# themattinthehatt/behavenet

Hardware: AMD Instinct MI355X
Metric: AE training frames/sec (128x128x1, batch 256) (higher is better)
Workload: dtype f32; 1 GPU; configs[1]: conv AE default arch, 1x128x128 f32 frames resident in HBM, 12 latents, batch 256 (chunks 200+56), fwd+bwd+Adam(amsgrad)

## Files before the change

### behavenet_amd/_hip.py

```python

import ctypes
import os

import numpy as np
import torch

_LIB_NAME = 'libbehavenet_hip.so'
_LIB_PATH = os.environ.get('BN_HIP_LIB') or os.path.join(
    os.path.dirname(os.path.abspath(__file__)), _LIB_NAME)
_lib = None

ACT_NONE, ACT_LRELU, ACT_SIGMOID = 0, 1, 2

PROF_NONE, PROF_CONV_FWD, PROF_CONV_BWD_D, PROF_CONV_BWD_W = 0, 1, 2, 3
PROF_CONVT_FWD, PROF_CONVT_BWD_D, PROF_CONVT_BWD_W, PROF_ADAM = 4, 5, 6, 7
PROF_LINEAR_FWD, PROF_LINEAR_BWD = 8, 9

_c_int, _c_float, _c_size_t, _c_void_p = ctypes.c_int, ctypes.c_float, ctypes.c_size_t, ctypes.c_void_p

_CONV_GEOM = [_c_int] * 12
_ACT_WS = [_c_int, _c_float, _c_void_p, _c_size_t, _c_void_p]

OP_CONV_FWD, OP_CONV_BWD_D, OP_CONV_BWD_W = 1, 2, 3
OP_CONVT_FWD, OP_CONVT_BWD_D, OP_CONVT_BWD_W = 4, 5, 6

SIGNATURES = {
    'bn_version': (_c_int, []),
    'bn_build_arch': (ctypes.c_char_p, []),
    'bn_error_string': (ctypes.c_char_p, [_c_int]),
    'bn_set_force_generic': (_c_int, [_c_int]),
    'bn_set_bigk1_block_bytes': (_c_size_t, [_c_size_t]),
    'bn_conv_ws_bytes': (_c_size_t, [_c_int] + _CONV_GEOM),
    'bn_conv_taps_bytes': (_c_size_t, [_c_int] + _CONV_GEOM),
    'bn_conv_taps_pad': (_c_int, [_c_int, _c_void_p, _c_void_p, _c_void_p, _c_void_p]),
    'bn_conv2d_fwd': (_c_int, [_c_void_p] * 5 + _CONV_GEOM + _ACT_WS),
    'bn_conv2d_fwd_u8_ws_bytes': (_c_size_t, _CONV_GEOM + [_c_int]),
    'bn_conv2d_fwd_u8': (_c_int, [_c_void_p] * 4 + _CONV_GEOM + _ACT_WS),
    'bn_conv2d_bwd_data': (_c_int, [_c_void_p] * 5 + _CONV_GEOM + _ACT_WS),
    'bn_conv2d_bwd_weight': (
        _c_int, [_c_void_p] * 4 + _CONV_GEOM + [_c_int, _c_void_p, _c_size_t, _c_void_p]),
    'bn_convT2d_fwd': (_c_int, [_c_void_p] * 5 + _CONV_GEOM + _ACT_WS),
    'bn_convT2d_bwd_data': (_c_int, [_c_void_p] * 5 + _CONV_GEOM + _ACT_WS),
    'bn_convT2d_bwd_weight': (
        _c_int, [_c_void_p] * 4 + _CONV_GEOM + [_c_int, _c_void_p, _c_size_t, _c_void_p]),
    'bn_batchnorm_ws_bytes': (_c_size_t, [_c_int, _c_int]),
    'bn_batchnorm_stats': (_c_int, [_c_void_p] * 3 + [_c_int] * 3 + [_c_void_p, _c_size_t, _c_void_p]),
    'bn_batchnorm_finalize': (_c_int, [_c_void_p] * 5 + [_c_int] + [_c_float] * 3 + [_c_void_p]),
    'bn_batchnorm_act_fwd': (_c_int, [_c_void_p] * 6 + [_c_int] * 4 + [_c_float, _c_void_p]),
    'bn_batchnorm_train_fwd_chunks': (
        _c_int, [_c_void_p] * 11 + [_c_int] * 3 + [_c_float, _c_int, _c_float, _c_void_p, _c_size_t,
                                                  _c_void_p]),
    'bn_batchnorm_act_bwd_chunks': (
        _c_int, [_c_void_p] * 10 + [_c_int, _c_void_p] + [_c_int] * 4 + [_c_float, _c_void_p, _c_size_t,
                                                                        _c_void_p]),
    'bn_batchnorm_act_bwd': (
        _c_int, [_c_void_p] * 9 + [_c_int] * 6 + [_c_float, _c_void_p, _c_size_t, _c_void_p]),
    'bn_batchnorm_moment': (_c_int, [_c_void_p] * 3 + [_c_int] * 3 + [_c_void_p, _c_size_t, _c_void_p]),
    'bn_batchnorm_bwd_reduce': (
        _c_int, [_c_void_p] * 7 + [_c_int] * 4 + [_c_float, _c_void_p, _c_size_t, _c_void_p]),
    'bn_batchnorm_bwd_apply': (
        _c_int, [_c_void_p] * 9 + [_c_int] * 3 + [_c_float, _c_int, _c_float, _c_void_p]),
    'bn_maxpool2d_fwd': (_c_int, [_c_void_p] * 3 + [_c_int] * 9 + [_c_void_p]),
    'bn_maxpool2d_bwd': (_c_int, [_c_void_p] * 3 + [_c_int] * 9 + [_c_void_p]),
    'bn_maxpool2d_act_fwd': (_c_int, [_c_void_p] * 3 + [_c_int] * 4 + [ctypes.c_float, _c_void_p]),
    'bn_conv2d_pool2_act_fwd': (_c_int, [_c_void_p] * 5 + _CONV_GEOM + [_c_int, _c_float, _c_void_p]),
    'bn_conv2d_pool2_act_ok': (_c_int, _CONV_GEOM),
    'bn_conv2d_pool2_bwd_weight_ws_bytes': (_c_size_t, _CONV_GEOM),
    'bn_conv2d_pool2_bwd_weight': (
        _c_int, [_c_void_p] * 6 + _CONV_GEOM + [_c_int, _c_float, _c_int, _c_void_p, _c_size_t, _c_void_p]),
    'bn_maxpool2d_act_bwd': (_c_int, [_c_void_p] * 4 + [_c_int] * 4 + [ctypes.c_float, _c_void_p]),
    'bn_maxunpool2d_fwd': (_c_int, [_c_void_p] * 3 + [_c_int] * 3 + [_c_void_p]),
    'bn_maxunpool2d_fwd_k2': (_c_int, [_c_void_p] * 3 + [_c_int] * 3 + [_c_void_p]),
    'bn_maxunpool2d_bwd': (_c_int, [_c_void_p] * 3 + [_c_int] * 3 + [_c_void_p]),
    'bn_act_fwd': (_c_int, [_c_void_p] * 2 + [_c_size_t, _c_int, _c_float, _c_void_p]),
    'bn_act_bwd': (_c_int, [_c_void_p] * 3 + [_c_size_t, _c_int, _c_float, _c_void_p]),
    'bn_linear_ws_bytes': (_c_size_t, [_c_int] * 3),
    'bn_linear_fwd': (_c_int, [_c_void_p] * 4 + [_c_int] * 3 + [_c_void_p, _c_size_t, _c_void_p]),
    'bn_linear_bwd': (
        _c_int, [_c_void_p] * 5 + [_c_int, _c_float, _c_void_p, _c_void_p, _c_int] +
        [_c_int] * 3 + [_c_void_p, _c_size_t, _c_void_p]),
    'bn_sqerr_frame_sums': (_c_int, [_c_void_p] * 4 + [_c_int, _c_size_t, _c_void_p]),
    'bn_sqerr_bwd': (_c_int, [_c_void_p] * 4 + [_c_size_t, _c_float, _c_void_p, _c_void_p]),
    'bn_convT2d_fwd_sqerr_parts': (_c_int, _CONV_GEOM),
    'bn_convT2d_fwd_sqerr_ws_bytes': (_c_size_t, _CONV_GEOM + [_c_int]),
    'bn_convT2d_fwd_sqerr': (
        _c_int, [_c_void_p] * 8 + _CONV_GEOM + [_c_int, _c_float, _c_void_p, _c_size_t, _c_void_p]),
    'bn_scale_frames': (_c_int, [_c_void_p] * 4 + [_c_int, _c_size_t, _c_void_p]),
    'bn_reduce_sum': (_c_int, [_c_void_p] * 2 + [_c_size_t, _c_float, _c_void_p]),
    'bn_reparam_fwd': (_c_int, [_c_void_p] * 4 + [_c_size_t, _c_void_p]),
    'bn_kl_rows': (_c_int, [_c_void_p] * 3 + [_c_int, _c_int, _c_void_p]),
    'bn_reparam_bwd': (_c_int, [_c_void_p] * 4 + [_c_size_t, _c_void_p]),
    'bn_kl_bwd': (_c_int, [_c_void_p] * 4 + [_c_size_t, _c_float, _c_void_p, _c_void_p]),
    'bn_decomposed_kl_fwd': (_c_int, [_c_void_p] * 7 + [_c_int, _c_int, _c_void_p]),
    'bn_decomposed_kl_bwd': (_c_int, [_c_void_p] * 9 + [_c_int, _c_int, _c_void_p]),
    'bn_psvae_head_fwd': (_c_int, [_c_void_p] * 14 + [_c_int] * 3 + [_c_void_p]),
    'bn_psvae_head_combine': (
        _c_int, [_c_void_p] * 4 + [_c_int] + [_c_float] * 3 + [_c_int] + [_c_void_p] * 3),
    'bn_psvae_head_bwd': (
        _c_int, [_c_void_p] * 3 + [_c_int] + [_c_void_p] * 10 + [_c_float] + [_c_void_p] * 5 +
        [_c_int] * 4 + [_c_void_p]),
    'bn_adam_amsgrad_step': (
        _c_int, [_c_void_p] * 5 + [_c_size_t] + [_c_float] * 5 + [_c_int, _c_void_p]),
    'bn_conv2d_first_bf16_ok': (_c_int, _CONV_GEOM),
    'bn_conv2d_bf16_ok': (_c_int, _CONV_GEOM),
    'bn_conv_pack_w_bf16_bytes': (_c_size_t, [_c_int] * 4),
    'bn_conv_pack_w_bf16': (_c_int, [_c_void_p] * 2 + [_c_int] * 4 + [_c_void_p]),
    'bn_conv2d_first_bf16': (
        _c_int, [_c_void_p, _c_int] + [_c_void_p] * 3 + _CONV_GEOM + [_c_int, _c_float, _c_void_p]),
    'bn_conv2d_fwd_bf16': (
        _c_int, [_c_void_p] * 4 + [_c_int] + _CONV_GEOM + [_c_int, _c_float, _c_void_p]),
    'bn_convT2d_bf16_ok': (_c_int, _CONV_GEOM),
    'bn_convT2d_last_bf16_ok': (_c_int, _CONV_GEOM),
    'bn_convT_pack_w_bf16_bytes': (_c_size_t, [_c_int] * 4),
    'bn_convT_pack_w_bf16': (_c_int, [_c_void_p] * 2 + [_c_int] * 4 + [_c_void_p]),
    'bn_to_nhwc_bf16': (_c_int, [_c_void_p] * 2 + [_c_int] * 4 + [_c_void_p]),
    'bn_convT2d_fwd_bf16': (
        _c_int, [_c_void_p] * 4 + [_c_int] + _CONV_GEOM + [_c_int, _c_float, _c_void_p]),
    'bn_convT2d_last_bf16': (
        _c_int, [_c_void_p] * 4 + _CONV_GEOM + [_c_int, _c_float, _c_void_p]),
    'bn_convT2d_last_bf16_sqerr_ws_bytes': (_c_size_t, _CONV_GEOM),
    'bn_convT2d_last_bf16_sqerr': (
        _c_int, [_c_void_p] * 4 + [_c_int] + [_c_void_p] * 2 + _CONV_GEOM +
        [_c_int, _c_float, _c_float, _c_void_p, _c_size_t, _c_void_p]),
    'bn_convT2d_last_bf16_u8': (
        _c_int, [_c_void_p] * 4 + _CONV_GEOM + [_c_int, _c_float, _c_void_p]),
    'bn_frame_sq_err_ws_bytes': (_c_size_t, [_c_int, _c_size_t]),
    'bn_frame_sq_err': (
        _c_int, [_c_void_p] * 2 + [_c_int] + [_c_void_p] * 2 + [_c_int, _c_size_t, _c_float, _c_void_p, _c_size_t,
                                                                 _c_void_p]),
    'bn_pixel_stats_ws_bytes': (_c_size_t, [_c_int, _c_size_t]),
    'bn_pixel_stats_accum': (
        _c_int, [_c_void_p] * 2 + [_c_int, _c_void_p, _c_int, _c_void_p, _c_int, _c_size_t, _c_void_p, _c_size_t,
                                   _c_void_p]),
    'bn_u8_to_unit_float': (_c_int, [_c_void_p] * 2 + [_c_size_t, _c_void_p]),
    'bn_unit_float_to_u8': (_c_int, [_c_void_p] * 2 + [_c_size_t, _c_void_p]),
    'bn_cond_encoder_input': (_c_int, [_c_void_p, _c_int, _c_void_p] + [_c_int] * 6 + [_c_void_p, _c_void_p]),
    'bn_frame_mosaic_u8': (_c_int, [_c_void_p] + [_c_int] * 10 + [_c_void_p] + [_c_int] * 3 + [_c_void_p, _c_void_p]),
    'bn_recon_panels_u8': (_c_int, [_c_void_p, _c_int, _c_void_p, _c_int, _c_void_p] + [_c_int] * 6
                           + [_c_void_p, _c_size_t, _c_void_p]),
    'bn_column_select_ws_bytes': (_c_size_t, [_c_int] * 3),
    'bn_column_count': (_c_int, [_c_void_p] + [_c_int] * 3 + [_c_void_p, _c_void_p, _c_size_t, _c_void_p]),
    'bn_column_select': (_c_int, [_c_void_p] + [_c_int] * 3 + [_c_void_p, _c_int, _c_void_p, _c_void_p, _c_size_t,
                                                                _c_void_p]),
    'bn_segment_label_sums_ws_bytes': (_c_size_t, [_c_int] * 3),
    'bn_segment_label_sums': (_c_int, [_c_void_p, _c_int] * 3 + [_c_void_p] + [_c_int] * 3
                              + [_c_void_p, _c_void_p, _c_size_t, _c_void_p]),
    'bn_prof_select': (_c_int, [_c_int] * 3),
    'bn_prof_select_nth': (_c_int, [_c_int] * 4),
    'bn_prof_read': (_c_int, [ctypes.POINTER(ctypes.c_double), ctypes.POINTER(ctypes.c_long)]),
    'bn_prof_read_main': (_c_int, [ctypes.POINTER(ctypes.c_double), ctypes.POINTER(ctypes.c_long)]),
    'bn_prof_set_bracket': (_c_int, [_c_int]),
    'bn_prof_kernel_name': (ctypes.c_char_p, []),
    'bn_prof_dispatch_overhead_us': (ctypes.c_double, [_c_int, _c_void_p]),
}


class HipLibraryError(RuntimeError):
    pass


def lib_path():
    return _LIB_PATH


def load(required=True):
    global _lib
    if _lib is not None:
        return _lib
    if not os.path.exists(_LIB_PATH):
        if required:
            raise HipLibraryError(
                '%s not found next to the package (%s). Build it with '
                '`python -c "import __graft_entry__ as g; g.build()"` or '
                '`make -C behavenet_amd/csrc`. There is no CPU fallback.' % (_LIB_NAME, _LIB_PATH))
        return None
    lib = ctypes.CDLL(_LIB_PATH)
    for name, (restype, argtypes) in SIGNATURES.items():
        fn = getattr(lib, name)
        fn.restype = restype
        fn.argtypes = argtypes
    _lib = lib
    return _lib


def _check(rc, what):
    if rc != 0:
        msg = load().bn_error_string(int(rc))
        raise HipLibraryError('%s failed: %s (code %d)' % (what, msg.decode() if msg else '?', rc))


def _ptr(t, name, dtype=torch.float32, allow_none=False):
    if t is None:
        if allow_none:
            return None
        raise HipLibraryError('%s: tensor is None' % name)
    if not t.is_cuda:
        raise HipLibraryError(
            '%s: expected a tensor on the GPU, got device %s (the HIP path has no CPU fallback)'
            % (name, t.device))
    if t.dtype != dtype:
        raise HipLibraryError('%s: expected dtype %s, got %s' % (name, dtype, t.dtype))
    if not t.is_contiguous():
        raise HipLibraryError('%s: tensor must be contiguous' % name)
    return t.data_ptr()


def _stream():
    return torch.cuda.current_stream().cuda_stream


_ws_cache = {}


def _arena(device, nbytes, tag=None):
    if torch.cuda.is_current_stream_capturing():
        return torch.empty(int(nbytes), dtype=torch.uint8, device=device).data_ptr()
    key = (device, torch.cuda.current_stream(device).cuda_stream) + ((tag,) if tag else ())
    buf = _ws_cache.get(key)
    if buf is None or buf.numel() < nbytes:
        with torch.cuda.stream(torch.cuda.current_stream(device)):
            buf = torch.empty(int(nbytes), dtype=torch.uint8, device=device)
        _ws_cache[key] = buf
    return buf.data_ptr()


def _workspace(op, geom, device):
    if torch.device(device).type != 'cuda':
        raise HipLibraryError(
            'expected tensors on the GPU, got device %s (the HIP path has no CPU fallback)' % device)
    nbytes = load().bn_conv_ws_bytes(op, *geom)
    if nbytes == 0:
        return None, 0
    return _arena(device, nbytes), nbytes


_taps_bytes = {}
_generic_epoch = 0


def conv_taps_bytes(op, geom):
    key = (_generic_epoch, op) + tuple(geom)
    v = _taps_bytes.get(key)
    if v is None:
        v = _taps_bytes[key] = int(load().bn_conv_taps_bytes(op, *geom))
    return v


def conv_taps_pad(jobs, device):
    n = len(jobs)
    if n == 0:
        return []
    sizes = [(conv_taps_bytes(op, geom) // 4 + 63) // 64 * 64 for op, geom, _ in jobs]
    if min(sizes) == 0:
        raise HipLibraryError('conv_taps_pad: a layer whose op does not pad its taps')
    buf = torch.empty(sum(sizes), dtype=torch.float32, device=device)
    out, o = [], 0
    for sz in sizes:
        out.append(buf[o:o + sz])
        o += sz
    wp = (ctypes.c_void_p * n)(*[_ptr(w, 'w') for _, _, w in jobs])
    w5p = (ctypes.c_void_p * n)(*[t.data_ptr() for t in out])
    flat = []
    for op, geom, _ in jobs:
        flat.append(op)
        flat.extend(int(v) for v in geom)
    geoms = (ctypes.c_int * (13 * n))(*flat)
    _check(load().bn_conv_taps_pad(n, wp, w5p, geoms, _stream()), 'bn_conv_taps_pad')
    return out


def conv2d_fwd(x, w, b, geom, act, slope, w5=None):
    N, C, H, W, K, R, S, st, pt, pl, P, Q = geom
    y = torch.empty((N, K, P, Q), dtype=torch.float32, device=x.device)
    ws, nb = _workspace(OP_CONV_FWD, geom, x.device)
    _check(load().bn_conv2d_fwd(
        _ptr(x, 'x'), _ptr(w, 'w'), _ptr(w5, 'w5', allow_none=True), _ptr(b, 'b', allow_none=True), _ptr(y, 'y'),
        *geom, act, slope, ws, nb, _stream()), 'bn_conv2d_fwd')
    return y


def conv2d_fwd_u8(x_u8, w, b, geom, act, slope):
    N, C, H, W, K, R, S, st, pt, pl, P, Q = geom
    y = torch.empty((N, K, P, Q), dtype=torch.float32, device=x_u8.device)
    lib = load()
    nbytes = lib.bn_conv2d_fwd_u8_ws_bytes(*geom, act)
    ws = None
    if nbytes:
        ws = _arena(x_u8.device, nbytes, 'fwd_u8')
    _check(lib.bn_conv2d_fwd_u8(
        _ptr(x_u8, 'x', dtype=torch.uint8), _ptr(w, 'w'), _ptr(b, 'b', allow_none=True),
        _ptr(y, 'y'), *geom, act, slope, ws, nbytes, _stream()), 'bn_conv2d_fwd_u8')
    return y


def conv2d_bwd_data(dy, w, geom, dact_src, dact, slope, w5=None):
    N, C, H, W = geom[:4]
    dx = torch.empty((N, C, H, W), dtype=torch.float32, device=dy.device)
    ws, nb = _workspace(OP_CONV_BWD_D, geom, dy.device)
    _check(load().bn_conv2d_bwd_data(
        _ptr(dy, 'dy'), _ptr(w, 'w'), _ptr(w5, 'w5', allow_none=True), _ptr(dx, 'dx'),
        _ptr(dact_src, 'dact_src', allow_none=True), *geom, dact, slope, ws, nb, _stream()), 'bn_conv2d_bwd_data')
    return dx


def conv2d_bwd_weight(x, dy, dw, db, geom, accumulate):
    ws, nb = _workspace(OP_CONV_BWD_W, geom, x.device)
    _check(load().bn_conv2d_bwd_weight(
        _ptr(x, 'x'), _ptr(dy, 'dy'), _ptr(dw, 'dw'), _ptr(db, 'db', allow_none=True), *geom,
# ... 361 lines not shown


def batchnorm_sync_train_fwd(x, gamma, beta, running_mean, running_var, momentum, eps, act, slope,
                             all_reduce):
    n, c = x.shape[0], x.shape[1]
    hw = x.numel() // max(n * c, 1) if n else int(x.shape[2] * x.shape[3])
    dev = x.device
    s1 = torch.zeros((c + 1,), dtype=torch.float32, device=dev)
    if n:
        ws, nb = _bn_ws(n, c, dev)
        _check(load().bn_batchnorm_moment(_ptr(x, 'x'), None, _ptr(s1, 'sums'), n, c, hw, ws, nb,
                                          _stream()), 'bn_batchnorm_moment')
        s1[c] = float(n)
    all_reduce(s1)
    count = s1[c] * hw
    mean = (s1[:c] / count).contiguous()
    s2 = torch.zeros((c,), dtype=torch.float32, device=dev)
    if n:
        _check(load().bn_batchnorm_moment(_ptr(x, 'x'), _ptr(mean, 'mean'), _ptr(s2, 'sums'), n, c,
                                          hw, ws, nb, _stream()), 'bn_batchnorm_moment')
    all_reduce(s2)
    var = (s2 / count).contiguous()
    cnt = float(count.item())
    unbias = cnt / (cnt - 1.0) if cnt > 1 else 1.0
    invstd = torch.empty_like(mean)
    _check(load().bn_batchnorm_finalize(
        _ptr(mean, 'mean'), _ptr(var, 'var'), _ptr(invstd, 'invstd'),
        _ptr(running_mean, 'running_mean', allow_none=True),
        _ptr(running_var, 'running_var', allow_none=True), c, eps, momentum, unbias, _stream()),
        'bn_batchnorm_finalize')
    y = torch.empty_like(x)
    if n:
        _check(load().bn_batchnorm_act_fwd(
            _ptr(x, 'x'), _ptr(mean, 'mean'), _ptr(invstd, 'invstd'),
            _ptr(gamma, 'gamma', allow_none=True), _ptr(beta, 'beta', allow_none=True),
            _ptr(y, 'y'), n, c, hw, act, slope, _stream()), 'bn_batchnorm_act_fwd')
    return y, mean, invstd, cnt


def batchnorm_sync_bwd(x, y, dy, mean, invstd, gamma, count, act, slope, all_reduce):
    n, c = x.shape[0], x.shape[1]
    hw = x.numel() // max(n * c, 1) if n else 1
    local = torch.zeros((2, c), dtype=torch.float32, device=x.device)
    if n:
        ws, nb = _bn_ws(n, c, x.device)
        _check(load().bn_batchnorm_bwd_reduce(
            _ptr(x, 'x'), _ptr(y, 'y'), _ptr(dy, 'dy'), _ptr(mean, 'mean'),
            _ptr(invstd, 'invstd'), _ptr(local[0], 'sum_dz'), _ptr(local[1], 'sum_dzx'), n, c, hw,
            act, slope, ws, nb, _stream()), 'bn_batchnorm_bwd_reduce')
    total = all_reduce(local.clone())
    dx = torch.empty_like(x)
    if n:
        _check(load().bn_batchnorm_bwd_apply(
            _ptr(x, 'x'), _ptr(y, 'y'), _ptr(dy, 'dy'), _ptr(mean, 'mean'),
            _ptr(invstd, 'invstd'), _ptr(gamma, 'gamma', allow_none=True),
            _ptr(total[0], 'sum_dz'), _ptr(total[1], 'sum_dzx'), _ptr(dx, 'dx'), n, c, hw,
            1.0 / float(count), act, slope, _stream()), 'bn_batchnorm_bwd_apply')
    return dx, local[0], local[1]


def act_fwd(x, act, slope):
    y = torch.empty_like(x)
    _check(load().bn_act_fwd(_ptr(x, 'x'), _ptr(y, 'y'), x.numel(), act, slope, _stream()),
           'bn_act_fwd')
    return y


def act_bwd(dy, y, act, slope, out=None):
    if out is None:
        out = torch.empty_like(dy)
    _check(load().bn_act_bwd(
        _ptr(dy, 'dy'), _ptr(y, 'y'), _ptr(out, 'dpre'), dy.numel(), act, slope, _stream()),
        'bn_act_bwd')
    return out


def _linear_ws(M, K, N, device):
    nbytes = load().bn_linear_ws_bytes(M, K, N)
    if nbytes == 0:
        return None, 0
    return _arena(device, nbytes, 'linear'), nbytes


def linear_fwd(x, w, b):
    M, K = x.shape
    N = w.shape[0]
    y = torch.empty((M, N), dtype=torch.float32, device=x.device)
    ws, nb = _linear_ws(M, K, N, x.device)
    _check(load().bn_linear_fwd(
        _ptr(x, 'x'), _ptr(w, 'w'), _ptr(b, 'b', allow_none=True), _ptr(y, 'y'), M, K, N,
        ws, nb, _stream()), 'bn_linear_fwd')
    return y


def linear_bwd(x, w, dy, need_dx, dact_src, dact, slope, dw, db, accumulate):
    M, N = dy.shape
    K = w.shape[1]
    dx = torch.empty((M, K), dtype=torch.float32, device=dy.device) if need_dx else None
    ws, nb = _linear_ws(M, K, N, dy.device) if need_dx else (None, 0)
    _check(load().bn_linear_bwd(
        _ptr(x, 'x', allow_none=True), _ptr(w, 'w'), _ptr(dy, 'dy'),
        _ptr(dx, 'dx', allow_none=True), _ptr(dact_src, 'dact_src', allow_none=True), dact, slope,
        _ptr(dw, 'dw', allow_none=True), _ptr(db, 'db', allow_none=True), int(accumulate),
        M, K, N, ws, nb, _stream()), 'bn_linear_bwd')
    return dx


def sqerr_frame_sums(pred, target, mask):
    N = pred.shape[0]
    D = pred.numel() // N
    out = torch.empty((N,), dtype=torch.float32, device=pred.device)
    _check(load().bn_sqerr_frame_sums(
        _ptr(pred, 'pred'), _ptr(target, 'target'), _ptr(mask, 'mask', allow_none=True),
        _ptr(out, 'frame_sums'), N, D, _stream()), 'bn_sqerr_frame_sums')
    return out


def sqerr_bwd(pred, target, mask, scale, gscale, out=None):
    dpred = torch.empty_like(pred) if out is None else out
    _check(load().bn_sqerr_bwd(
        _ptr(pred, 'pred'), _ptr(target, 'target'), _ptr(mask, 'mask', allow_none=True),
        _ptr(dpred, 'dpred'), pred.numel(), float(scale), _ptr(gscale, 'gscale', allow_none=True),
        _stream()), 'bn_sqerr_bwd')
    return dpred


def convT2d_fwd_sqerr(x, w, b, target, mask, geom, act, slope, want_xhat):
    N, Ci, Hi, Wi, Co, R, S, st, ct, cl, Ho, Wo = geom
    lib = load()
    P = lib.bn_convT2d_fwd_sqerr_parts(*geom)
    if P <= 0:
        raise HipLibraryError('bn_convT2d_fwd_sqerr_parts: bad geometry %s' % (geom,))
    xhat = torch.empty((N, Co, Ho, Wo), dtype=torch.float32, device=x.device) if want_xhat \
        else None
    dpre = torch.empty((N, Co, Ho, Wo), dtype=torch.float32, device=x.device)
    part = torch.empty((N, P), dtype=torch.float32, device=x.device)
    nbytes = lib.bn_convT2d_fwd_sqerr_ws_bytes(*geom, int(want_xhat))
    ws = None
    if nbytes:
        ws = _arena(x.device, nbytes, 'fwd_sqerr')
    _check(lib.bn_convT2d_fwd_sqerr(
        _ptr(x, 'x'), _ptr(w, 'w'), _ptr(b, 'b', allow_none=True), _ptr(target, 'target'),
        _ptr(mask, 'mask', allow_none=True), _ptr(xhat, 'xhat', allow_none=True),
        _ptr(dpre, 'dpre'), _ptr(part, 'part'), *geom, act, slope, ws, nbytes, _stream()),
        'bn_convT2d_fwd_sqerr')
    return xhat, dpre, part


def scale_frames(t, frame_scale, group_scale=None, group_of_frame=None):
    N = t.shape[0]
    _check(load().bn_scale_frames(
        _ptr(t, 't'), _ptr(frame_scale, 'frame_scale'),
        _ptr(group_scale, 'group_scale', allow_none=True),
        _ptr(group_of_frame, 'group_of_frame', dtype=torch.int32, allow_none=True),
        N, t.numel() // N, _stream()), 'bn_scale_frames')
    return t


def reduce_sum(t, scale=1.0, out=None):
    if out is None:
        out = torch.empty((), dtype=torch.float32, device=t.device)
    _check(load().bn_reduce_sum(_ptr(t, 'in'), _ptr(out, 'out'), t.numel(), float(scale),
                                _stream()), 'bn_reduce_sum')
    return out


def reparam_fwd(mu, logvar, eps):
    z = torch.empty_like(mu)
    _check(load().bn_reparam_fwd(
        _ptr(mu, 'mu'), _ptr(logvar, 'logvar'), _ptr(eps, 'eps'), _ptr(z, 'z'), mu.numel(),
        _stream()), 'bn_reparam_fwd')
    return z


def kl_rows(mu, logvar):
    N, D = mu.shape
    out = torch.empty((N,), dtype=torch.float32, device=mu.device)
    _check(load().bn_kl_rows(_ptr(mu, 'mu'), _ptr(logvar, 'logvar'), _ptr(out, 'kl_rows'), N, D,
                             _stream()), 'bn_kl_rows')
    return out


DECOMPOSED_KL_MAX_D = 64


def _check_dkl_width(D):
    if D > DECOMPOSED_KL_MAX_D:
        raise ValueError('decomposed KL: %d latent dimensions, the kernels serve at most %d'
                         % (D, DECOMPOSED_KL_MAX_D))


def decomposed_kl_fwd(z, mu, logvar, out3=None):
    N, D = z.shape
    _check_dkl_width(D)
    if out3 is None:
        out3 = torch.empty((3,), dtype=torch.float32, device=z.device)
    log_qz = torch.empty((N,), dtype=torch.float32, device=z.device)
    lse = torch.empty((N, D), dtype=torch.float32, device=z.device)
    terms = torch.empty((3 * N,), dtype=torch.float32, device=z.device)
    _check(load().bn_decomposed_kl_fwd(
        _ptr(z, 'z'), _ptr(mu, 'mu'), _ptr(logvar, 'logvar'), _ptr(out3, 'out3'),
        _ptr(log_qz, 'log_qz'), _ptr(lse, 'lse'), _ptr(terms, 'terms'), N, D, _stream()),
        'bn_decomposed_kl_fwd')
    return out3, log_qz, lse


def decomposed_kl_bwd(z, mu, logvar, log_qz, lse, g3, out=None):
    N, D = z.shape
    _check_dkl_width(D)
    dz, dmu, dlogvar = out if out is not None else (
        torch.empty_like(z), torch.empty_like(z), torch.empty_like(z))
    _check(load().bn_decomposed_kl_bwd(
        _ptr(z, 'z'), _ptr(mu, 'mu'), _ptr(logvar, 'logvar'), _ptr(log_qz, 'log_qz'),
        _ptr(lse, 'lse'), _ptr(g3, 'g3'), _ptr(dz, 'dz'), _ptr(dmu, 'dmu'),
        _ptr(dlogvar, 'dlogvar'), N, D, _stream()), 'bn_decomposed_kl_bwd')
    return dz, dmu, dlogvar


def psvae_head_fwd(y, w, logvar, eps, Dw, Db, labels, lmask):
    N, L = y.shape
    U = logvar.shape[1] - L
    dev = y.device
    z = torch.empty((N, L + U), dtype=torch.float32, device=dev)
    z_u = torch.empty((N, U), dtype=torch.float32, device=dev)
    lv_u = torch.empty((N, U), dtype=torch.float32, device=dev)
    yhat = torch.empty((N, L), dtype=torch.float32, device=dev)
    rows = torch.empty((2, N), dtype=torch.float32, device=dev)
    _check(load().bn_psvae_head_fwd(
        _ptr(y, 'y'), _ptr(w, 'w', allow_none=True), _ptr(logvar, 'logvar'), _ptr(eps, 'eps'),
        _ptr(Dw, 'Dw'), _ptr(Db, 'Db', allow_none=True), _ptr(labels, 'labels'),
        _ptr(lmask, 'lmask', allow_none=True), _ptr(z, 'z'), _ptr(z_u, 'z_u'), _ptr(lv_u, 'lv_u'),
        _ptr(yhat, 'yhat'), _ptr(rows[0], 'row_sq'), _ptr(rows[1], 'row_kl'), N, L, U, _stream()),
        'bn_psvae_head_fwd')
    return z, z_u, lv_u, yhat, rows[0], rows[1]


def psvae_head_combine(row_sq, row_kl, dkl3, bounds_dev, n_chunks, alpha, kl, beta, L):
    T = torch.empty((n_chunks,), dtype=torch.float32, device=row_sq.device)
    cols5 = torch.empty((n_chunks, 5), dtype=torch.float32, device=row_sq.device)
    _check(load().bn_psvae_head_combine(
        _ptr(row_sq, 'row_sq'), _ptr(row_kl, 'row_kl'), _ptr(dkl3, 'dkl3'),
        _ptr(bounds_dev, 'bounds', dtype=torch.int32), int(n_chunks), float(alpha), float(kl),
        float(beta), int(L), _ptr(T, 'T'), _ptr(cols5, 'cols5'), _stream()), 'bn_psvae_head_combine')
    return T, cols5


# ... 411 lines not shown
```

### behavenet_amd/csrc/bn_launch.h

```cpp
#pragma once
#include "bn_common.h"

struct GemmArgs {
    const float* A; long sai, sak;
    const float* B; long sbk, sbj;
    float* C; long sci, scj;
    int M, N, K;
    const float* bias_j;
    const float* dact_src;
    int dact; float slope;
    int accumulate;
    float* part;
    int kslice;
};

int bn_launch_down_generic(const float* big, const float* w, const float* bias, float* out,
                           const float* dact_src, const BnGeom& g, int act, int dact, float slope,
                           hipStream_t st);
int bn_launch_up_generic(const float* small, const float* w, const float* bias, float* out,
                         const float* dact_src, const BnGeom& g, int act, int dact, float slope,
                         hipStream_t st);
int bn_launch_wgrad_generic(const float* small, const float* big, float* dw, const BnGeom& g,
                            int accumulate, hipStream_t st);
size_t bn_channel_sum_ws_bytes(int N, int C, int npix);
int bn_launch_channel_sum(const float* t, float* db, int N, int C, int npix, int accumulate,
                          void* ws, size_t ws_bytes, hipStream_t st);

int bn_launch_gemm(const GemmArgs& a, hipStream_t st, void* ws = nullptr, size_t ws_bytes = 0);
size_t bn_gemm_ws_bytes(int M, int N, int K);
int bn_launch_col_sum(const float* dy, float* db, int M, int N, int accumulate, hipStream_t st);
int bn_launch_linear_jobs(const GemmArgs* g0, const GemmArgs* g1, const float* dy, float* db, int M,
                          int N, int accumulate, void* ws, size_t ws_bytes, hipStream_t st);
size_t bn_linear_jobs_ws_bytes(int M, int N, int K);

int bn_launch_act_fwd(const float* x, float* y, size_t n, int act, float slope, hipStream_t st);
int bn_launch_act_bwd(const float* dy, const float* y, float* dpre, size_t n, int act, float slope,
                      hipStream_t st);
int bn_launch_sqerr_frame_sums(const float* pred, const float* target, const float* mask,
                               float* frame_sums, int N, size_t D, hipStream_t st);
int bn_launch_sqerr_bwd(const float* pred, const float* target, const float* mask, float* dpred,
                        size_t n, float scale, const float* gscale, hipStream_t st);
int bn_launch_scale_frames(float* t, const float* frame_scale, const float* group_scale,
                           const int* group_of_frame, int N, size_t D, hipStream_t st);
int bn_launch_reduce_sum(const float* in, float* out, size_t n, float scale, hipStream_t st);
int bn_launch_reparam_fwd(const float* mu, const float* logvar, const float* eps, float* z,
                          size_t n, hipStream_t st);
int bn_launch_kl_rows(const float* mu, const float* logvar, float* kl_rows, int N, int D,
                      hipStream_t st);
int bn_launch_reparam_bwd(const float* dz, const float* z, const float* mu, float* dlogvar,
                          size_t n, hipStream_t st);
int bn_launch_kl_bwd(const float* mu, const float* logvar, float* dmu, float* dlogvar, size_t n,
                     float scale, const float* gscale, hipStream_t st);
int bn_launch_adam(float* p, const float* g, float* m, float* v, float* vmax, size_t n, float lr,
                   float b1, float b2, float eps, float wd, int step, hipStream_t st);
int bn_launch_u8_to_unit_float(const unsigned char* in, float* out, size_t n, hipStream_t st);

bool bn_frame_sq_err_ok(int N, size_t D);
size_t bn_frame_sq_err_ws_bytes_impl(int N, size_t D);
int bn_launch_frame_sq_err(const float* xhat, const void* target, int target_is_u8, const float* mask, float* out,
                           int N, size_t D, float scale, void* ws, hipStream_t st);
int bn_launch_frame_err_finish(const float* part, float* out, int N, unsigned P, float scale, hipStream_t st);

bool bn_unit_float_to_u8_ok(size_t n);
int bn_launch_unit_float_to_u8(const float* in, unsigned char* out, size_t n, hipStream_t st);

bool bn_pixel_stats_ok(int N, size_t D);
size_t bn_pixel_stats_ws_bytes_impl(int N, size_t D);
int bn_launch_pixel_stats(const float* xhat, const void* target, int target_is_u8, const float* mask, int mask_frames,
                          double* acc, int N, size_t D, void* ws, hipStream_t st);

bool bn_cond_input_ok(int N, int C, int H, int W, int L);
int bn_launch_cond_input(const void* frames, int frames_is_u8, const float* coords, int ld, int N, int C, int H, int W,
                         int L, float* out, hipStream_t st);

bool bn_frame_mosaic_ok(int P, int C, int H, int W, int ch, int y_min, int x_min, int Hc, int Wc, int T, int R, int Cc);
int bn_launch_frame_mosaic(const void* frames, int frames_u8, int P, int C, int H, int W, int ch, int y_min, int x_min,
                           int Hc, int Wc, const int* src, int T, int R, int Cc, unsigned char* out, hipStream_t st);

bool bn_recon_panels_ok(int N, int C, int H, int W, size_t out_frame_stride);
int bn_launch_recon_panels(const void* orig, int orig_u8, const void* recon, int recon_u8, const float* mask,
                           int mask_per_frame, int N, int C, int H, int W, int show_orig, unsigned char* out,
                           size_t out_frame_stride, hipStream_t st);

bool bn_column_select_ok(int n, int d, int ld, int r);
size_t bn_column_count_ws_bytes_impl(int n, int d);
size_t bn_column_select_ws_bytes_impl(int n, int d, int r);
int bn_launch_column_count(const float* x, int n, int d, int ld, long long* n_valid, void* ws, hipStream_t st);
int bn_launch_column_select(const float* x, int n, int d, int ld, const long long* ranks, int r, float* out, void* ws,
                            hipStream_t st);

bool bn_segment_label_sums_ok(int n, int S, int L);
size_t bn_segment_label_sums_ws_bytes_impl(int n, int S, int L);
int bn_launch_segment_label_sums(const float* pred, int ld_pred, const float* truth, int ld_truth, const float* mask,
                                 int ld_mask, const long long* offsets, int S, int L, int n, double* out, void* ws,
                                 hipStream_t st);

size_t bn_batchnorm_ws_bytes_impl(int N, int C);
int bn_launch_bn_stats(const float* x, float* mean, float* var, int N, int C, int HW, void* ws,
                       hipStream_t st);
int bn_launch_bn_finalize(const float* mean, const float* var, float* invstd, float* running_mean,
                          float* running_var, int C, float eps, float momentum, float unbias,
                          hipStream_t st);
int bn_launch_bn_act_fwd(const float* x, const float* mean, const float* invstd,
                         const float* gamma, const float* beta, float* y, int N, int C, int HW,
                         int act, float slope, hipStream_t st);
int bn_launch_bn_act_bwd(const float* x, const float* y, const float* dy, const float* mean,
                         const float* invstd, const float* gamma, float* dx, float* dgamma,
                         float* dbeta, int accumulate, int batch_stats, int N, int C, int HW,
                         int act, float slope, void* ws, hipStream_t st);

int bn_launch_bn_moment(const float* x, const float* center, float* sums, int N, int C, int HW,
                        void* ws, hipStream_t st);
int bn_launch_bn_bwd_reduce(const float* x, const float* y, const float* dy, const float* mean,
                            const float* invstd, float* sum_dz, float* sum_dzx, int N, int C,
                            int HW, int act, float slope, void* ws, hipStream_t st);
int bn_launch_bn_train_fwd_chunks(const float* x, const float* gamma, const float* beta,
                                  float* running_mean, float* running_var, long long* num_batches,
                                  float* y, float* mean, float* invstd, const int* bounds,
                                  const float* factors, int n_chunks, int C, int HW, float eps, int act,
                                  float slope, void* ws, hipStream_t st);
int bn_launch_bn_act_bwd_chunks(const float* x, const float* y, const float* dy, const float* mean,
                                const float* invstd, const float* gamma, const float* beta, float* dx,
                                float* dgamma, float* dbeta, int accumulate, const int* bounds,
                                int n_chunks, int C, int HW, int act, float slope, void* ws,
                                hipStream_t st);
int bn_launch_bn_bwd_apply(const float* x, const float* y, const float* dy, const float* mean,
                           const float* invstd, const float* gamma, const float* sum_dz,
// ... 85 lines not shown
```

### behavenet_amd/csrc/bn_reduce.h

```cpp
#pragma once
#include "bn_common.h"

__global__ __launch_bounds__(1024) void k_sum_partials(const float* __restrict__ part,
                                                       float* __restrict__ out, int total,
                                                       int splits, int accumulate, int ab_elems,
                                                       int ntap, int row_len, int row_stride);

__global__ __launch_bounds__(256) void k_sum_partials_pair(
    const float* __restrict__ part_a, float* __restrict__ out_a, int total_a, int ab_elems, int ntap,
    const float* __restrict__ part_b, float* __restrict__ out_b, int total_b, int splits,
    int accumulate, int blocks_a);

static inline int bn_launch_sum_partials_pair(const float* part_a, float* out_a, int total_a,
                                              int ab_elems, int ntap, const float* part_b,
                                              float* out_b, int total_b, int splits, int accumulate,
                                              hipStream_t st) {
    const int blocks_a = (total_a + 63) / 64, blocks_b = (total_b + 63) / 64;
    hipLaunchKernelGGL(k_sum_partials_pair, dim3(blocks_a + blocks_b), dim3(256), 0, st, part_a, out_a,
                       total_a, ab_elems, ntap, part_b, out_b, total_b, splits, accumulate, blocks_a);
    hipError_t e = hipGetLastError();
    return e == hipSuccess ? 0 : (int)e;
}

static inline int bn_launch_sum_partials(const float* part, float* out, int total, int splits,
                                         int accumulate, int ab_elems, int ntap, hipStream_t st,
                                         int row_len = 0, int row_stride = 0) {
    const int threads = (splits >= 128 && total <= 16384) ? 1024 : 256;
    hipLaunchKernelGGL(k_sum_partials, dim3((total + 63) / 64), dim3(threads), 0, st, part, out, total,
                       splits, accumulate, ab_elems, ntap, row_len, row_stride);
    hipError_t e = hipGetLastError();
    return e == hipSuccess ? 0 : (int)e;
}
```

### behavenet_amd/csrc/capi.hip

```cpp
#include <math.h>
#include <stdio.h>
#include <stdlib.h>
#include <string.h>
#include <hip/hip_ext.h>
#include "bn_common.h"
#include "bn_launch.h"
#include "bn_fast.h"

namespace {
struct ProfState {
    int family = BN_PROF_NONE;
    int C = 0, K = 0;
    static const int kMaxSlots = 2048;
    hipEvent_t ev[4 * kMaxSlots];
    bool taken[kMaxSlots], bracketed[kMaxSlots];
    int created = 0;
    int used = 0;
    double total_ms = 0.0, main_ms = 0.0;
    long launches = 0, main_launches = 0;
    bool bracket = true;
    int nth = -1, seen = 0;
    char kernel_name[96] = "";
} g_prof;

// ... 1342 lines not shown
        if (bi[1] <= 0 || bounds[2 * i] < 0) return BN_E_BADARG;
        if (!ws || ws_bytes < bn_batchnorm_ws_bytes_impl(bi[1], C)) return BN_E_WORKSPACE;
        const size_t o = (size_t)bounds[2 * i] * C * HW;
        const float fi = factors ? factors[i] : 0.f;
        const int rc = bn_launch_bn_train_fwd_chunks(x + o, gamma, beta, running_mean, running_var,
                                                     num_batches_tracked, y + o, mean + (size_t)i * C,
                                                     invstd + (size_t)i * C, bi, &fi, 1, C, HW, eps, act,
                                                     slope, ws, st);
        if (rc) return rc;
    }
    return 0;
}

extern "C" int bn_batchnorm_act_bwd_chunks(const float* x, const float* y, const float* dy,
                                           const float* mean, const float* invstd,
                                           const float* gamma, const float* beta, float* dx,
                                           float* dgamma, float* dbeta, int accumulate,
                                           const int* bounds, int n_chunks, int C, int HW, int act,
                                           float slope, void* ws, size_t ws_bytes, bn_stream_t stream) {
    if (!x || !dy || !mean || !invstd || !dx || !bounds || n_chunks <= 0 || C <= 0 || HW <= 0)
        return BN_E_BADARG;
    if (!y && act != BN_ACT_NONE && act != BN_ACT_LRELU) return BN_E_BADARG;
    hipStream_t st = (hipStream_t)stream;
    {
        int nmax = 0;
        for (int i = 0; i < n_chunks; ++i) nmax = bounds[2 * i + 1] - bounds[2 * i] > nmax ? bounds[2 * i + 1] - bounds[2 * i] : nmax;
        if (nmax > 0 && ws && ws_bytes >= bn_batchnorm_ws_bytes_impl(nmax, C)) {
            const int rc = bn_launch_bn_act_bwd_chunks(x, y, dy, mean, invstd, gamma, beta, dx, dgamma, dbeta,
                                                       accumulate, bounds, n_chunks, C, HW, act, slope, ws, st);
            if (rc != BN_E_SHAPE) return rc;
        }
    }
    for (int i = 0; i < n_chunks; ++i) {
        const int bi[2] = {0, bounds[2 * i + 1] - bounds[2 * i]};
        if (bi[1] <= 0 || bounds[2 * i] < 0) return BN_E_BADARG;
        if (!ws || ws_bytes < bn_batchnorm_ws_bytes_impl(bi[1], C)) return BN_E_WORKSPACE;
        const size_t o = (size_t)bounds[2 * i] * C * HW;
        const int rc = bn_launch_bn_act_bwd_chunks(x + o, y ? y + o : nullptr, dy + o, mean + (size_t)i * C,
                                                   invstd + (size_t)i * C, gamma, beta, dx + o, dgamma, dbeta,
                                                   (accumulate || i > 0) ? 1 : 0, bi, 1, C, HW, act, slope, ws,
                                                   st);
        if (rc) return rc;
    }
    return 0;
}

extern "C" int bn_batchnorm_moment(const float* x, const float* center, float* sums, int N, int C,
                                   int HW, void* ws, size_t ws_bytes, bn_stream_t stream) {
    if (!x || !sums || N <= 0 || C <= 0 || HW <= 0) return BN_E_BADARG;
    if (!ws || ws_bytes < bn_batchnorm_ws_bytes_impl(N, C)) return BN_E_WORKSPACE;
    return bn_launch_bn_moment(x, center, sums, N, C, HW, ws, (hipStream_t)stream);
}

extern "C" int bn_batchnorm_bwd_reduce(const float* x, const float* y, const float* dy,
                                       const float* mean, const float* invstd, float* sum_dz,
                                       float* sum_dzx, int N, int C, int HW, int act, float slope,
                                       void* ws, size_t ws_bytes, bn_stream_t stream) {
    if (!x || !y || !dy || !mean || !invstd || !sum_dz || !sum_dzx || N <= 0 || C <= 0 || HW <= 0)
        return BN_E_BADARG;
    if (!ws || ws_bytes < bn_batchnorm_ws_bytes_impl(N, C)) return BN_E_WORKSPACE;
    return bn_launch_bn_bwd_reduce(x, y, dy, mean, invstd, sum_dz, sum_dzx, N, C, HW, act, slope, ws,
                                   (hipStream_t)stream);
}

extern "C" int bn_batchnorm_bwd_apply(const float* x, const float* y, const float* dy,
                                      const float* mean, const float* invstd, const float* gamma,
                                      const float* sum_dz, const float* sum_dzx, float* dx, int N,
                                      int C, int HW, float inv_count, int act, float slope,
                                      bn_stream_t stream) {
    if (!x || !y || !dy || !mean || !invstd || !sum_dz || !sum_dzx || !dx || N <= 0 || C <= 0 ||
        HW <= 0)
        return BN_E_BADARG;
    return bn_launch_bn_bwd_apply(x, y, dy, mean, invstd, gamma, sum_dz, sum_dzx, dx, N, C, HW,
                                  inv_count, act, slope, (hipStream_t)stream);
}

extern "C" size_t bn_linear_ws_bytes(int M, int K, int N) {
    if (M <= 0 || K <= 0 || N <= 0) return 0;
    const size_t f = bn_gemm_ws_bytes(M, N, K), d = bn_gemm_ws_bytes(M, K, N);
    return f > d ? f : d;
}

extern "C" int bn_linear_fwd(const float* x, const float* w, const float* b, float* y, int M,
                             int K, int N, void* ws, size_t ws_bytes, bn_stream_t stream) {
    if (!x || !w || !y || M <= 0 || K <= 0 || N <= 0) return BN_E_BADARG;
    GemmArgs a;
    a.A = x; a.sai = K; a.sak = 1;
    a.B = w; a.sbk = 1; a.sbj = K;
    a.C = y; a.sci = N; a.scj = 1;
    a.M = M; a.N = N; a.K = K;
    a.bias_j = b; a.dact_src = nullptr; a.dact = BN_ACT_NONE; a.slope = 0.f; a.accumulate = 0;
    BnProfScope prof(BN_PROF_LINEAR_FWD, K, N, "k_linear_jobs", (hipStream_t)stream);
    return bn_launch_linear_jobs(&a, nullptr, nullptr, nullptr, 0, 0, 0, ws, ws_bytes, (hipStream_t)stream);
}

extern "C" int bn_linear_bwd(const float* x, const float* w, const float* dy, float* dx,
                             const float* dact_src, int dact, float slope, float* dw, float* db,
                             int accumulate, int M, int K, int N, void* ws, size_t ws_bytes,
                             bn_stream_t stream) {
    if (!dy || M <= 0 || K <= 0 || N <= 0) return BN_E_BADARG;
    hipStream_t st = (hipStream_t)stream;
    BnProfScope prof(BN_PROF_LINEAR_BWD, K, N, "k_linear_jobs (dx, dW, db)", st);
    GemmArgs gx, gw;
    if (dx) {
        if (!w) return BN_E_BADARG;
        GemmArgs& a = gx;
        a.A = dy; a.sai = N; a.sak = 1;
        a.B = w; a.sbk = K; a.sbj = 1;
        a.C = dx; a.sci = K; a.scj = 1;
        a.M = M; a.N = K; a.K = N;
        a.bias_j = nullptr; a.dact_src = dact_src; a.dact = dact; a.slope = slope;
        a.accumulate = 0; a.part = nullptr; a.kslice = 0;
    }
    if (dw) {
        if (!x) return BN_E_BADARG;
        GemmArgs& a = gw;
        a.A = dy; a.sai = 1; a.sak = N;
        a.B = x; a.sbk = K; a.sbj = 1;
        a.C = dw; a.sci = K; a.scj = 1;
        a.M = N; a.N = K; a.K = M;
        a.bias_j = nullptr; a.dact_src = nullptr; a.dact = BN_ACT_NONE; a.slope = 0.f;
        a.accumulate = accumulate; a.part = nullptr; a.kslice = 0;
    }
    return bn_launch_linear_jobs(dx ? &gx : nullptr, dw ? &gw : nullptr, dy, db, M, N, accumulate, ws,
                                 ws_bytes, st);
}

extern "C" int bn_sqerr_frame_sums(const float* pred, const float* target, const float* mask,
                                   float* frame_sums, int N, size_t D, bn_stream_t stream) {
    if (!pred || !target || !frame_sums || N <= 0 || D == 0) return BN_E_BADARG;
    return bn_launch_sqerr_frame_sums(pred, target, mask, frame_sums, N, D, (hipStream_t)stream);
}

extern "C" int bn_sqerr_bwd(const float* pred, const float* target, const float* mask,
                            float* dpred, size_t n, float scale, const float* gscale,
                            bn_stream_t stream) {
    if (!pred || !target || !dpred) return BN_E_BADARG;
    if (n == 0) return 0;
    return bn_launch_sqerr_bwd(pred, target, mask, dpred, n, scale, gscale, (hipStream_t)stream);
}

static bool fused_sqerr_fast(const BnGeom& g) {
    return !force_generic() && !bn_qgemm_supported(g) && !bn_s5win_supported(g) && !bn_s5_up_plan(g).supported &&
           bn_edge_up_plan(g).supported;
}

extern "C" int bn_convT2d_fwd_sqerr_parts(int N, int Ci, int Hi, int Wi, int Co, int R, int S,
                                          int stride, int crop_t, int crop_l, int Ho, int Wo) {
    const BnGeom g = convT_geom(N, Ci, Hi, Wi, Co, R, S, stride, crop_t, crop_l, Ho, Wo);
    if (!bn_geom_ok(g)) return 0;
    return fused_sqerr_fast(g) ? bn_edge_up_parts_per_frame(g) : 1;
}

extern "C" size_t bn_convT2d_fwd_sqerr_ws_bytes(int N, int Ci, int Hi, int Wi, int Co, int R,
                                                int S, int stride, int crop_t, int crop_l, int Ho,
                                                int Wo, int with_xhat) {
    const BnGeom g = convT_geom(N, Ci, Hi, Wi, Co, R, S, stride, crop_t, crop_l, Ho, Wo);
    if (!bn_geom_ok(g) || fused_sqerr_fast(g)) return 0;
    size_t conv = bn_conv_ws_bytes(BN_OP_CONVT_FWD, N, Ci, Hi, Wi, Co, R, S, stride, crop_t, crop_l,
                                   Ho, Wo);
    conv = (conv + 255) & ~(size_t)255;
    return conv + (with_xhat ? 0 : (size_t)N * Co * Ho * Wo * sizeof(float));
}

extern "C" int bn_convT2d_fwd_sqerr(const float* x, const float* w, const float* b,
                                    const float* target, const float* mask, float* xhat,
                                    float* dpre, float* part, int N, int Ci, int Hi, int Wi,
                                    int Co, int R, int S, int stride, int crop_t, int crop_l,
                                    int Ho, int Wo, int act, float slope, void* ws,
                                    size_t ws_bytes, bn_stream_t stream) {
    if (!x || !w || !target || !dpre || !part) return BN_E_BADARG;
    const BnGeom g = convT_geom(N, Ci, Hi, Wi, Co, R, S, stride, crop_t, crop_l, Ho, Wo);
    if (!bn_geom_ok(g)) return BN_E_BADARG;
    hipStream_t st = (hipStream_t)stream;
    if (fused_sqerr_fast(g)) {
        BnProfScope prof(BN_PROF_CONVT_FWD, g.Cs, g.Cb, bn_edge_up_kernel_name(g, true), st);
        return bn_launch_edge_up(x, w, b, xhat, g, act, slope, st, target, mask, dpre, part);
    }
    const size_t need = bn_convT2d_fwd_sqerr_ws_bytes(N, Ci, Hi, Wi, Co, R, S, stride, crop_t,
                                                      crop_l, Ho, Wo, xhat != nullptr);
    if (need && (!ws || ws_bytes < need)) return BN_E_WORKSPACE;
    const size_t n_out = (size_t)N * Co * Ho * Wo;
    const size_t conv_ws = need - (xhat ? 0 : n_out * sizeof(float));
    float* xh = xhat ? xhat : (float*)((char*)ws + conv_ws);
    int rc = run_up(BN_PROF_CONVT_FWD, x, w, nullptr, b, xh, nullptr, g, act, BN_ACT_NONE, slope, ws,
                    conv_ws, st);
    if (rc) return rc;
    rc = bn_launch_sqerr_frame_sums(xh, target, mask, part, N, (size_t)Co * Ho * Wo, st);
    if (rc) return rc;
    rc = bn_launch_sqerr_bwd(xh, target, mask, dpre, n_out, 1.f, nullptr, st);
    if (rc) return rc;
    if (act != BN_ACT_NONE) rc = bn_launch_act_bwd(dpre, xh, dpre, n_out, act, slope, st);
    return rc;
}

extern "C" int bn_scale_frames(float* t, const float* frame_scale, const float* group_scale,
                               const int* group_of_frame, int N, size_t D, bn_stream_t stream) {
    if (!t || !frame_scale || N <= 0 || D == 0) return BN_E_BADARG;
    if ((group_scale == nullptr) != (group_of_frame == nullptr)) return BN_E_BADARG;
    return bn_launch_scale_frames(t, frame_scale, group_scale, group_of_frame, N, D,
                                  (hipStream_t)stream);
}

extern "C" int bn_reduce_sum(const float* in, float* out, size_t n, float scale,
                             bn_stream_t stream) {
    if (!in || !out) return BN_E_BADARG;
    return bn_launch_reduce_sum(in, out, n, scale, (hipStream_t)stream);
}

extern "C" int bn_reparam_fwd(const float* mu, const float* logvar, const float* eps, float* z,
                              size_t n, bn_stream_t stream) {
    if (!mu || !logvar || !eps || !z) return BN_E_BADARG;
    if (n == 0) return 0;
    return bn_launch_reparam_fwd(mu, logvar, eps, z, n, (hipStream_t)stream);
}

extern "C" int bn_kl_rows(const float* mu, const float* logvar, float* kl_rows, int N, int D,
                          bn_stream_t stream) {
    if (!mu || !logvar || !kl_rows || N <= 0 || D <= 0) return BN_E_BADARG;
    return bn_launch_kl_rows(mu, logvar, kl_rows, N, D, (hipStream_t)stream);
}

extern "C" int bn_reparam_bwd(const float* dz, const float* z, const float* mu, float* dlogvar,
                              size_t n, bn_stream_t stream) {
    if (!dz || !z || !mu || !dlogvar) return BN_E_BADARG;
    if (n == 0) return 0;
    return bn_launch_reparam_bwd(dz, z, mu, dlogvar, n, (hipStream_t)stream);
}

extern "C" int bn_kl_bwd(const float* mu, const float* logvar, float* dmu, float* dlogvar,
                         size_t n, float scale, const float* gscale, bn_stream_t stream) {
    if (!mu || !logvar || !dmu || !dlogvar) return BN_E_BADARG;
    if (n == 0) return 0;
    return bn_launch_kl_bwd(mu, logvar, dmu, dlogvar, n, scale, gscale, (hipStream_t)stream);
}

extern "C" int bn_decomposed_kl_fwd(const float* z, const float* mu, const float* logvar,
                                    float* out3, float* log_qz, float* lse, float* terms, int N,
                                    int D, bn_stream_t stream) {
    if (!z || !mu || !logvar || !out3 || !log_qz || !lse || !terms || N <= 0 || D <= 0)
        return BN_E_BADARG;
    return bn_launch_dkl_fwd(z, mu, logvar, out3, log_qz, lse, terms, N, D, (hipStream_t)stream);
}

extern "C" int bn_decomposed_kl_bwd(const float* z, const float* mu, const float* logvar,
                                    const float* log_qz, const float* lse, const float* g3,
                                    float* dz, float* dmu, float* dlogvar, int N, int D,
                                    bn_stream_t stream) {
    if (!z || !mu || !logvar || !log_qz || !lse || !g3 || !dz || !dmu || !dlogvar || N <= 0 ||
        D <= 0)
        return BN_E_BADARG;
    return bn_launch_dkl_bwd(z, mu, logvar, log_qz, lse, g3, dz, dmu, dlogvar, N, D,
                             (hipStream_t)stream);
}

extern "C" int bn_adam_amsgrad_step(float* p, const float* g, float* m, float* v, float* vmax,
                                    size_t n, float lr, float beta1, float beta2, float eps,
                                    float weight_decay, int step, bn_stream_t stream) {
    if (!p || !g || !m || !v || !vmax || step < 1) return BN_E_BADARG;
    if (n == 0) return 0;
    BnProfScope prof(BN_PROF_ADAM, 0, 0, "k_adam_amsgrad", (hipStream_t)stream);
    return bn_launch_adam(p, g, m, v, vmax, n, lr, beta1, beta2, eps, weight_decay, step,
                          (hipStream_t)stream);
}

extern "C" int bn_u8_to_unit_float(const unsigned char* in, float* out, size_t n,
                                   bn_stream_t stream) {
    if (!in || !out) return BN_E_BADARG;
    if (n == 0) return 0;
    return bn_launch_u8_to_unit_float(in, out, n, (hipStream_t)stream);
}

static BnBf16Geom bf16_geom(int N, int C, int H, int W, int K, int R, int S, int stride, int pad_t, int pad_l, int P,
                            int Q) {
    return BnBf16Geom{N, C, H, W, K, R, S, stride, pad_t, pad_l, P, Q};
}
static bool bf16_geom_valid(const BnBf16Geom& g) {
    if (!(g.N > 0 && g.C > 0 && g.H > 0 && g.W > 0 && g.K > 0 && g.R > 0 && g.S > 0 && g.stride > 0 && g.pt >= 0 &&
          g.pl >= 0 && g.P > 0 && g.Q > 0))
        return false;
    return (long)(g.P - 1) * g.stride - g.pt < g.H && (long)(g.Q - 1) * g.stride - g.pl < g.W;
}
static bool aligned16(const void* p) { return ((uintptr_t)p & 15) == 0; }

extern "C" int bn_conv2d_bf16_ok(int N, int C, int H, int W, int K, int R, int S, int stride, int pad_t, int pad_l,
                                 int P, int Q) {
    const BnBf16Geom g = bf16_geom(N, C, H, W, K, R, S, stride, pad_t, pad_l, P, Q);
    return (bf16_geom_valid(g) && bn_bf16_conv_ok(g)) ? 1 : 0;
}
extern "C" int bn_conv2d_first_bf16_ok(int N, int C, int H, int W, int K, int R, int S, int stride, int pad_t,
                                       int pad_l, int P, int Q) {
    const BnBf16Geom g = bf16_geom(N, C, H, W, K, R, S, stride, pad_t, pad_l, P, Q);
// ... 228 lines not shown
```

### behavenet_amd/csrc/conv_edge.hip

```cpp
#include <hip/hip_ext.h>
#include <stdlib.h>
#include "bn_common.h"
#include "bn_fast.h"
#include "bn_reduce.h"

typedef float floatx16 __attribute__((ext_vector_type(16)));

#define ED_THREADS 256
#define ED_OOB 0x7fffffff

__device__ __forceinline__ float ed_ld(__amdgpu_buffer_rsrc_t r, int byte_off) {
    return __builtin_bit_cast(float, __builtin_amdgcn_raw_buffer_load_b32(r, byte_off, 0, 0));
}

#define WC_ROWS 4
#define WC_W 64
#define WC_TPX (WC_ROWS * WC_W)
#define WC_SP (WC_TPX + 2)
#define WC_IH (2 * WC_ROWS + 3)
#define WC_RW (2 * WC_W + 4)
#define WC_KS (32 * WC_TPX / ED_THREADS)

#define WC_DECODE_GRID()                                                                    \
    int bch, bx, G;                                                                         \
// ... 436 lines not shown
        p.variant = 1;
        p.d = wgrad_c1_grid(g);
        p.ws_bytes = ((size_t)g.Cb * p.d * g.Cs * 25 + (size_t)p.d * 32) * sizeof(float);
        p.kernel_name = wgrad_c1e_ok(g) ? "k_wgrad_c1e" : "k_wgrad_c1<1>";
        return p;
    }
    if (g.Cs > 32) return p;
    if (g.Ws != WC_W || (g.Hs % WC_ROWS) != 0 || g.Hb != 2 * g.Hs || g.Wb != 2 * g.Ws) {
        if (g.pt > 4 || g.pl > 4 || (g.CsS > 0 && g.CsS != g.Cs)) return p;
        p.supported = true;
        p.variant = 1;
        p.d = wgrad_c1_grid(g);
        p.ws_bytes = ((size_t)g.Cb * p.d * g.Cs * 25 + (size_t)p.d * 32) * sizeof(float);
        p.kernel_name = "k_wgrad_c1<2>";
        return p;
    }
    p.supported = true;
    p.d = wgrad_c1_grid(g);
    p.ws_bytes = ((size_t)g.Cb * p.d * g.Cs * 25 + (size_t)p.d * 32) * sizeof(float);
    p.kernel_name = (g.pt == 1 && g.pl == 1) ? "k_wgrad_c1d" : "k_wgrad_c1<2>";
    return p;
}

int bn_launch_edge_wgrad(const BnFastPlan& plan, const float* small, const float* big, float* dw,
                         const BnGeom& g, int accumulate, void* ws, hipStream_t st, float* db,
                         int bias_side, bool* bias_done) {
    const int spf = wgrad_c1_rblocks(g) * wgrad_c1_cblocks(g), n_stages = g.N * spf;
    float* bias_part = (db && bias_side == 1)
        ? (float*)ws + (size_t)g.Cb * plan.d * g.Cs * 25 : nullptr;
    if (g.CsS > 0 && g.CsS != g.Cs && !(g.pt == 1 && g.pl == 1)) return BN_E_SHAPE;
    const bool vec = (g.Ws & 3) == 0 && (((uintptr_t)small) & 15u) == 0 && g.CsS == 0;
    const int pair = (g.Cb > 1 && (plan.d & 7) == 0) ? 1 : 0;
    const dim3 wgrid = pair ? dim3(plan.d * g.Cb) : dim3(plan.d, g.Cb);
    if (g.stride == 1 && wgrad_c1e_ok(g) && vec) {
        static bool attr_set = false;
        if (!attr_set) {
            const void* fns[4] = {(const void*)k_wgrad_c1e<true, false>, (const void*)k_wgrad_c1e<false, false>,
                                  (const void*)k_wgrad_c1e<true, true>, (const void*)k_wgrad_c1e<false, true>};
            for (const void* fn : fns) {
                hipError_t e1 = hipFuncSetAttribute(fn, hipFuncAttributeMaxDynamicSharedMemorySize, WE_LDS);
                if (e1 != hipSuccess) return (int)e1;
            }
            attr_set = true;
        }
#define WE_LAUNCH(B, M)                                                                                     \
        BN_LAUNCH_MAIN((k_wgrad_c1e<B, M>), wgrid, dim3(ED_THREADS), WE_LDS, st, small, big, (float*)ws,   \
                           bias_part, g, n_stages, spf, wgrad_c1_cblocks(g), pair)
        if (g.Cs <= 16) { if (bias_part) WE_LAUNCH(true, true); else WE_LAUNCH(false, true); }
        else { if (bias_part) WE_LAUNCH(true, false); else WE_LAUNCH(false, false); }
#undef WE_LAUNCH
    } else if (g.stride == 1) {
        if (vec)
            BN_LAUNCH_MAIN((k_wgrad_c1<1, true>), wgrid, dim3(ED_THREADS), 0, st, small, big,
                               (float*)ws, bias_part, g, n_stages, spf, wgrad_c1_cblocks(g), pair);
        else
            BN_LAUNCH_MAIN((k_wgrad_c1<1, false>), wgrid, dim3(ED_THREADS), 0, st, small, big,
                               (float*)ws, bias_part, g, n_stages, spf, wgrad_c1_cblocks(g), pair);
    } else if (g.pt == 1 && g.pl == 1 && plan.variant != 1) {
        static bool attr_set = false;
        if (!attr_set) {
            hipError_t e1 = hipFuncSetAttribute((const void*)k_wgrad_c1d<true>,
                                                hipFuncAttributeMaxDynamicSharedMemorySize, WD_LDS);
            hipError_t e2 = hipFuncSetAttribute((const void*)k_wgrad_c1d<false>,
                                                hipFuncAttributeMaxDynamicSharedMemorySize, WD_LDS);
            if (e1 != hipSuccess) return (int)e1;
            if (e2 != hipSuccess) return (int)e2;
            attr_set = true;
        }
        if (bias_part)
            BN_LAUNCH_MAIN(k_wgrad_c1d<true>, wgrid, dim3(ED_THREADS), WD_LDS, st, small,
                               big, (float*)ws, bias_part, g, n_stages, g.Hs / WC_ROWS, pair);
        else
            BN_LAUNCH_MAIN(k_wgrad_c1d<false>, wgrid, dim3(ED_THREADS), WD_LDS, st, small,
                               big, (float*)ws, bias_part, g, n_stages, g.Hs / WC_ROWS, pair);
    } else if (vec) {
        BN_LAUNCH_MAIN((k_wgrad_c1<2, true>), wgrid, dim3(ED_THREADS), 0, st, small, big,
                           (float*)ws, bias_part, g, n_stages, spf, wgrad_c1_cblocks(g), pair);
    } else {
        BN_LAUNCH_MAIN((k_wgrad_c1<2, false>), wgrid, dim3(ED_THREADS), 0, st, small, big,
                           (float*)ws, bias_part, g, n_stages, spf, wgrad_c1_cblocks(g), pair);
    }
    BN_LAUNCH_CHECK();
    if (bias_part) {
        const int rc = bn_launch_sum_partials(bias_part, db, g.Cs, plan.d, accumulate, 0, 0, st);
        if (rc) return rc;
        if (bias_done) *bias_done = true;
    }
    for (int b = 0; b < g.Cb; ++b) {
        const int rc = bn_launch_sum_partials(
            (const float*)ws + (size_t)b * plan.d * g.Cs * 25, dw + b * 25, g.Cs * 25, plan.d,
            accumulate, 0, 0, st, 25, g.Cb * 25);
        if (rc) return rc;
    }
    return 0;
}

#define DC_W 64
#define DC_ROWS 2
#define DC_IH (2 * DC_ROWS + 3)
#define DC_X0 4
#define DC_RW (2 * DC_W + 8)
#define DC_C4 (DC_RW / 4)
#define DC_NLD ((DC_IH * DC_C4 + 63) / 64)
#define DC_TS (DC_W + 4)
#define DC_SLAB (32 * DC_TS)
#ifndef DC_HALF
#define DC_HALF 1
#endif
#if DC_HALF
#define DC_MAX_WAVES_PER_CU 16
#define DC_WPE 4
#else
#define DC_MAX_WAVES_PER_CU 12
#define DC_WPE 3
#endif
#define DC_HTS 36

#ifndef DC_ST_AUX
#define DC_ST_AUX 16
#endif

typedef float floatx2p __attribute__((ext_vector_type(2)));
__device__ __forceinline__ void ed_lrelu4(float (&v)[4], float slope) {
    const floatx2p s2 = {slope, slope};
    floatx2p lo = {v[0], v[1]}, hi = {v[2], v[3]}, mlo, mhi;
    asm("v_pk_mul_f32 %0, %1, %2" : "=v"(mlo) : "v"(lo), "v"(s2));
    asm("v_pk_mul_f32 %0, %1, %2" : "=v"(mhi) : "v"(hi), "v"(s2));
    asm("v_max_f32 %0, %1, %2" : "=v"(v[0]) : "v"(lo.x), "v"(mlo.x));
    asm("v_max_f32 %0, %1, %2" : "=v"(v[1]) : "v"(lo.y), "v"(mlo.y));
    asm("v_max_f32 %0, %1, %2" : "=v"(v[2]) : "v"(hi.x), "v"(mhi.x));
    asm("v_max_f32 %0, %1, %2" : "=v"(v[3]) : "v"(hi.y), "v"(mhi.y));
}

#ifdef E0_SMALLOUT
#define E0_OUT_OFFSET(o) ((o) & 0xffff0)
#else
#define E0_OUT_OFFSET(o) (o)
#endif

typedef int intx4 __attribute__((ext_vector_type(4)));
typedef float floatx4e __attribute__((ext_vector_type(4)));
typedef unsigned int uintx4e __attribute__((ext_vector_type(4)));

template <int ACT, bool MASK, bool GENW = false>
__global__ __launch_bounds__(64) __attribute__((amdgpu_waves_per_eu(DC_WPE, DC_WPE))) void k_down_c1(
    const float* __restrict__ big, const float* __restrict__ w, const float* __restrict__ bias,
    float* __restrict__ out, const float* __restrict__ dact_src, BnGeom g, float slope,
    int units) {
    __shared__ __attribute__((aligned(16))) float bl[DC_IH * DC_RW];
    __shared__ __attribute__((aligned(16))) float tw[DC_HALF ? 32 * DC_HTS : DC_SLAB];
    const int lane = threadIdx.x;
    const int li = lane & 31, kk = lane >> 5;
    const int ncb = GENW ? (g.Ws + DC_W - 1) / DC_W : 1;
    const int rpf = GENW ? (g.Hs + DC_ROWS - 1) / DC_ROWS : g.Hs / DC_ROWS;
    const int upf = rpf * ncb;
    const int HWb = g.Hb * g.Wb, PQ = g.Hs * g.Ws;
#ifdef E0_TRACE
    unsigned long long* trc = e0_trace + (size_t)blockIdx.x * 8;
#define E0_MARK(slot) do { if (threadIdx.x == 0) trc[slot] = __builtin_amdgcn_s_memrealtime(); } while (0)
    E0_MARK(0);
    if (threadIdx.x == 0) trc[7] = __builtin_amdgcn_s_getreg((4 << 0) | (0 << 6) | (31 << 11));
#else
#define E0_MARK(slot)
#endif

    const __amdgpu_buffer_rsrc_t rb = __builtin_amdgcn_make_buffer_rsrc(
        (void*)big, 0, (int)((size_t)g.N * HWb * 4), 0x00020000);

    int ld_y[DC_NLD], ld_off[DC_NLD];
#pragma unroll
    for (int k = 0; k < DC_NLD; ++k) {
// ... 1774 lines not shown
```

### behavenet_amd/csrc/conv_generic.hip

```cpp
#include "bn_common.h"
#include "bn_launch.h"

#define GEN_THREADS 256
#define GEN_MT 8
#define GEN_MAXS 16

__global__ __launch_bounds__(GEN_THREADS) void k_down_generic(
    const float* __restrict__ big, const float* __restrict__ w, const float* __restrict__ bias,
    float* __restrict__ out, const float* __restrict__ dact_src, BnGeom g, int act, int dact,
    float slope) {
    const int pix = blockIdx.x * GEN_THREADS + threadIdx.x;
    const int npix = g.Hs * g.Ws;
    const int m0 = blockIdx.y * GEN_MT;
    const int n = blockIdx.z;
    if (pix >= npix) return;
    const int p = pix / g.Ws, q = pix - p * g.Ws;
    const int RS = g.R * g.S;
    float acc[GEN_MT];
#pragma unroll
    for (int j = 0; j < GEN_MT; ++j) acc[j] = 0.f;

    const int h0 = p * g.stride - g.pt, w0 = q * g.stride - g.pl;
    for (int c = 0; c < g.Cb; ++c) {
        const float* bp = big + ((size_t)n * g.Cb + c) * g.Hb * g.Wb;
// ... 167 lines not shown
int bn_launch_wgrad_generic(const float* small, const float* big, float* dw, const BnGeom& g,
                            int accumulate, hipStream_t st) {
    if (g.R > GEN_MAXS || g.S > GEN_MAXS) return BN_E_SHAPE;
    dim3 grid(g.Cb, g.Cs, g.R);
    hipLaunchKernelGGL(k_wgrad_generic, grid, dim3(GEN_THREADS), 0, st, small, big, dw, g,
                       accumulate);
    BN_LAUNCH_CHECK();
    return 0;
}

__global__ __launch_bounds__(GEN_THREADS) void k_channel_sum_part(
    const float* __restrict__ t, float* __restrict__ part, int N, int C, int npix, int S) {
    __shared__ float red[4];
    const int c = blockIdx.x, sp = blockIdx.y;
    const int n_beg = (int)((long)sp * N / S), n_end = (int)((long)(sp + 1) * N / S);
    float acc = 0.f;
    const bool vec = (npix & 3) == 0 && ((((uintptr_t)t) & 15u) == 0);
    const int per = npix >> 2;
    if (vec && per < GEN_THREADS && (GEN_THREADS % per) == 0) {
        const int fpp = GEN_THREADS / per, q = threadIdx.x % per;
        for (int n = n_beg + threadIdx.x / per; n < n_end; n += fpp) {
            const float4 v = reinterpret_cast<const float4*>(t + ((size_t)n * C + c) * npix)[q];
            acc += (v.x + v.y) + (v.z + v.w);
        }
    } else
    for (int n = n_beg; n < n_end; ++n) {
        const float* tp = t + ((size_t)n * C + c) * npix;
        if (vec) {
            const float4* t4 = reinterpret_cast<const float4*>(tp);
            for (int i = threadIdx.x; i < (npix >> 2); i += GEN_THREADS) {
                const float4 v = t4[i];
                acc += (v.x + v.y) + (v.z + v.w);
            }
        } else {
            for (int i = threadIdx.x; i < npix; i += GEN_THREADS) acc += tp[i];
        }
    }
    const float s = bn_block_reduce_256(acc, red);
    if (threadIdx.x == 0) part[(size_t)c * S + sp] = s;
}

__global__ __launch_bounds__(64) void k_channel_sum_final(const float* __restrict__ part, float* __restrict__ db,
                                                          int C, int S, int accumulate) {
    const int c = blockIdx.x;
    float v = 0.f;
    for (int s = threadIdx.x; s < S; s += 64) v += part[(size_t)c * S + s];
#pragma unroll
    for (int off = 32; off > 0; off >>= 1) v += __shfl_xor(v, off, 64);
    if (threadIdx.x == 0) db[c] = accumulate ? db[c] + v : v;
}

static int channel_sum_splits(int N, int C, int npix) {
    if ((long)N * npix < 8192) return 1;
    int s = 1024 / C;
    if (s > 256) s = 256;
    if (s > N) s = N;
    return s < 1 ? 1 : s;
}

size_t bn_channel_sum_ws_bytes(int N, int C, int npix) {
    const int s = channel_sum_splits(N, C, npix);
    return s > 1 ? (size_t)C * s * sizeof(float) : 0;
}

int bn_launch_channel_sum(const float* t, float* db, int N, int C, int npix, int accumulate,
                          void* ws, size_t ws_bytes, hipStream_t st) {
    const int S = channel_sum_splits(N, C, npix);
    if (S > 1 && ws && ws_bytes >= (size_t)C * S * sizeof(float)) {
        hipLaunchKernelGGL(k_channel_sum_part, dim3(C, S), dim3(GEN_THREADS), 0, st, t, (float*)ws,
                           N, C, npix, S);
        BN_LAUNCH_CHECK();
        hipLaunchKernelGGL(k_channel_sum_final, dim3(C), dim3(64), 0, st,
                           (const float*)ws, db, C, S, accumulate);
        BN_LAUNCH_CHECK();
        return 0;
    }
    hipLaunchKernelGGL(k_channel_sum, dim3(C), dim3(GEN_THREADS), 0, st, t, db, N, C, npix,
                       accumulate);
    BN_LAUNCH_CHECK();
    return 0;
}

#include "bn_reduce.h"
__global__ __launch_bounds__(1024) void k_sum_partials(const float* __restrict__ part,
                                                       float* __restrict__ out, int total,
                                                       int splits, int accumulate, int ab_elems,
                                                       int ntap, int row_len, int row_stride) {
    __shared__ float red[16][64];
    const int il = threadIdx.x & 63, zl = threadIdx.x >> 6;
    const int nz = blockDim.x >> 6;
    const int i = blockIdx.x * 64 + il;
    float s0 = 0.f, s1 = 0.f, s2 = 0.f, s3 = 0.f;
    if (i < total) {
        int z = zl;
        for (; z + 3 * nz < splits; z += 4 * nz) {
            s0 += part[(size_t)z * total + i];
            s1 += part[(size_t)(z + nz) * total + i];
            s2 += part[(size_t)(z + 2 * nz) * total + i];
            s3 += part[(size_t)(z + 3 * nz) * total + i];
        }
        for (; z < splits; z += nz) s0 += part[(size_t)z * total + i];
    }
    red[zl][il] = (s0 + s1) + (s2 + s3);
    __syncthreads();
    if (nz == 16 && zl < 4)
        red[zl][il] = (red[zl][il] + red[zl + 4][il]) + (red[zl + 8][il] + red[zl + 12][il]);
    if (nz == 16) __syncthreads();
    if (zl == 0 && i < total) {
        const float v = (red[0][il] + red[1][il]) + (red[2][il] + red[3][il]);
        size_t o = i;
        if (ab_elems > 0) {
            const int tap = i / ab_elems;
            o = (size_t)(i - tap * ab_elems) * ntap + tap;
        } else if (row_len > 0) {
            const int row = i / row_len;
            o = (size_t)row * row_stride + (i - row * row_len);
        }
        out[o] = accumulate ? out[o] + v : v;
    }
}

__global__ __launch_bounds__(256) void k_sum_partials_pair(
    const float* __restrict__ part_a, float* __restrict__ out_a, int total_a, int ab_elems, int ntap,
    const float* __restrict__ part_b, float* __restrict__ out_b, int total_b, int splits,
    int accumulate, int blocks_a) {
    __shared__ float red[4][64];
    const bool job_b = (int)blockIdx.x >= blocks_a;
    const float* part = job_b ? part_b : part_a;
    float* out = job_b ? out_b : out_a;
    const int total = job_b ? total_b : total_a;
    const int il = threadIdx.x & 63, zl = threadIdx.x >> 6;
    const int i = (job_b ? (int)blockIdx.x - blocks_a : (int)blockIdx.x) * 64 + il;
    float s0 = 0.f, s1 = 0.f, s2 = 0.f, s3 = 0.f;
    if (i < total) {
        int z = zl;
        for (; z + 12 < splits; z += 16) {
            s0 += part[(size_t)z * total + i];
            s1 += part[(size_t)(z + 4) * total + i];
            s2 += part[(size_t)(z + 8) * total + i];
            s3 += part[(size_t)(z + 12) * total + i];
        }
        for (; z < splits; z += 4) s0 += part[(size_t)z * total + i];
    }
    red[zl][il] = (s0 + s1) + (s2 + s3);
    __syncthreads();
    if (zl == 0 && i < total) {
        const float v = (red[0][il] + red[1][il]) + (red[2][il] + red[3][il]);
        size_t o = i;
        if (!job_b && ab_elems > 0) {
            const int tap = i / ab_elems;
            o = (size_t)(i - tap * ab_elems) * ntap + tap;
        }
        out[o] = accumulate ? out[o] + v : v;
    }
}
```

### behavenet_amd/csrc/elementwise.hip

```cpp
#include "bn_common.h"
#include "bn_launch.h"

#define EW_THREADS 256
#define EW_MAX_BLOCKS 2048

static inline int ew_blocks(size_t nvec) {
    size_t b = (nvec + EW_THREADS - 1) / EW_THREADS;
    if (b < 1) b = 1;
    if (b > EW_MAX_BLOCKS) b = EW_MAX_BLOCKS;
    return (int)b;
}

static inline bool aligned16(const void* p) { return (((uintptr_t)p) & 15u) == 0; }

__global__ __launch_bounds__(EW_THREADS) void k_act_bwd(
    const float* __restrict__ dy, const float* __restrict__ y, float* __restrict__ dpre, size_t n,
    int vec, int act, float slope) {
    const size_t tid = (size_t)blockIdx.x * EW_THREADS + threadIdx.x;
    const size_t nthreads = (size_t)gridDim.x * EW_THREADS;
    if (vec) {
        const size_t n4 = n >> 2;
        const float4* dy4 = reinterpret_cast<const float4*>(dy);
        const float4* y4 = reinterpret_cast<const float4*>(y);
        float4* o4 = reinterpret_cast<float4*>(dpre);
// ... 1 lines not shown
            const float4 a = dy4[i], b = y4[i];
            float4 o;
            o.x = a.x * bn_act_grad_from_output(b.x, act, slope);
            o.y = a.y * bn_act_grad_from_output(b.y, act, slope);
            o.z = a.z * bn_act_grad_from_output(b.z, act, slope);
            o.w = a.w * bn_act_grad_from_output(b.w, act, slope);
            o4[i] = o;
        }
        for (size_t i = (n4 << 2) + tid; i < n; i += nthreads)
            dpre[i] = dy[i] * bn_act_grad_from_output(y[i], act, slope);
    } else {
        for (size_t i = tid; i < n; i += nthreads)
            dpre[i] = dy[i] * bn_act_grad_from_output(y[i], act, slope);
    }
}

__global__ __launch_bounds__(EW_THREADS) void k_sqerr_frame_sums(
    const float* __restrict__ pred, const float* __restrict__ target,
    const float* __restrict__ mask, float* __restrict__ frame_sums, size_t D, int vec) {
    __shared__ float red[EW_THREADS / BN_WAVE];
    const size_t base = (size_t)blockIdx.x * D;
    const float* p = pred + base;
    const float* t = target + base;
    const float* m = mask ? mask + base : nullptr;
    float acc = 0.f;
    if (vec) {
        const size_t D4 = D >> 2;
        const float4* p4 = reinterpret_cast<const float4*>(p);
        const float4* t4 = reinterpret_cast<const float4*>(t);
        const float4* m4 = reinterpret_cast<const float4*>(m);
        for (size_t i = threadIdx.x; i < D4; i += EW_THREADS) {
            const float4 a = p4[i], b = t4[i];
            float dx = a.x - b.x, dy = a.y - b.y, dz = a.z - b.z, dw = a.w - b.w;
            dx *= dx; dy *= dy; dz *= dz; dw *= dw;
            if (m) { const float4 k = m4[i]; dx *= k.x; dy *= k.y; dz *= k.z; dw *= k.w; }
            acc += (dx + dy) + (dz + dw);
        }
        for (size_t i = (D4 << 2) + threadIdx.x; i < D; i += EW_THREADS) {
            float d = p[i] - t[i]; d *= d; if (m) d *= m[i]; acc += d;
        }
    } else {
        for (size_t i = threadIdx.x; i < D; i += EW_THREADS) {
            float d = p[i] - t[i]; d *= d; if (m) d *= m[i]; acc += d;
        }
    }
#pragma unroll
    for (int off = 32; off > 0; off >>= 1) acc += __shfl_down(acc, off, 64);
    if ((threadIdx.x & 63) == 0) red[threadIdx.x >> 6] = acc;
    __syncthreads();
    if (threadIdx.x == 0) frame_sums[blockIdx.x] = (red[0] + red[1]) + (red[2] + red[3]);
}

__global__ __launch_bounds__(EW_THREADS) void k_sqerr_bwd(
    const float* __restrict__ pred, const float* __restrict__ target,
    const float* __restrict__ mask, float* __restrict__ dpred, size_t n, float scale,
    const float* __restrict__ gscale, int vec) {
    const float sc = 2.f * scale * (gscale ? gscale[0] : 1.f);
    const size_t tid = (size_t)blockIdx.x * EW_THREADS + threadIdx.x;
    const size_t nthreads = (size_t)gridDim.x * EW_THREADS;
    if (vec) {
        const size_t n4 = n >> 2;
        const float4* p4 = reinterpret_cast<const float4*>(pred);
        const float4* t4 = reinterpret_cast<const float4*>(target);
        const float4* m4 = reinterpret_cast<const float4*>(mask);
        float4* o4 = reinterpret_cast<float4*>(dpred);
        for (size_t i = tid; i < n4; i += nthreads) {
            const float4 a = p4[i], b = t4[i];
            float4 o;
            o.x = sc * (a.x - b.x); o.y = sc * (a.y - b.y);
            o.z = sc * (a.z - b.z); o.w = sc * (a.w - b.w);
            if (mask) { const float4 k = m4[i]; o.x *= k.x; o.y *= k.y; o.z *= k.z; o.w *= k.w; }
            o4[i] = o;
        }
        for (size_t i = (n4 << 2) + tid; i < n; i += nthreads) {
            float o = sc * (pred[i] - target[i]); if (mask) o *= mask[i]; dpred[i] = o;
        }
    } else {
        for (size_t i = tid; i < n; i += nthreads) {
            float o = sc * (pred[i] - target[i]); if (mask) o *= mask[i]; dpred[i] = o;
        }
    }
}

__global__ __launch_bounds__(EW_THREADS) void k_reduce_sum(
    const float* __restrict__ in, float* __restrict__ out, size_t n, float scale) {
    __shared__ float red[EW_THREADS / BN_WAVE];
    float acc = 0.f;
    for (size_t i = threadIdx.x; i < n; i += EW_THREADS) acc += in[i];
#pragma unroll
    for (int off = 32; off > 0; off >>= 1) acc += __shfl_down(acc, off, 64);
    if ((threadIdx.x & 63) == 0) red[threadIdx.x >> 6] = acc;
    __syncthreads();
    if (threadIdx.x == 0) out[0] = ((red[0] + red[1]) + (red[2] + red[3])) * scale;
}

__global__ __launch_bounds__(EW_THREADS) void k_reparam_fwd(
    const float* __restrict__ mu, const float* __restrict__ logvar, const float* __restrict__ eps,
    float* __restrict__ z, size_t n) {
    const size_t nthreads = (size_t)gridDim.x * EW_THREADS;
    for (size_t i = (size_t)blockIdx.x * EW_THREADS + threadIdx.x; i < n; i += nthreads)
        z[i] = fmaf(eps[i], expf(logvar[i]), mu[i]);
}

__global__ __launch_bounds__(EW_THREADS) void k_kl_rows(
    const float* __restrict__ mu, const float* __restrict__ logvar, float* __restrict__ kl_rows,
    int N, int D) {
    const int row = blockIdx.x * (EW_THREADS / BN_WAVE) + (threadIdx.x >> 6);
    if (row >= N) return;
    const int lane = threadIdx.x & 63;
    float acc = 0.f;
    for (int d = lane; d < D; d += BN_WAVE) {
        const float lv = logvar[(size_t)row * D + d], m = mu[(size_t)row * D + d];
        acc += expf(lv) - lv + m * m - 1.f;
    }
#pragma unroll
    for (int off = 32; off > 0; off >>= 1) acc += __shfl_down(acc, off, 64);
    if (lane == 0) kl_rows[row] = 0.5f * acc;
}

__global__ __launch_bounds__(EW_THREADS) void k_reparam_bwd(
    const float* __restrict__ dz, const float* __restrict__ z, const float* __restrict__ mu,
    float* __restrict__ dlogvar, size_t n) {
    const size_t nthreads = (size_t)gridDim.x * EW_THREADS;
    for (size_t i = (size_t)blockIdx.x * EW_THREADS + threadIdx.x; i < n; i += nthreads)
        dlogvar[i] = dz[i] * (z[i] - mu[i]);
}

__global__ __launch_bounds__(EW_THREADS) void k_kl_bwd(
    const float* __restrict__ mu, const float* __restrict__ logvar, float* __restrict__ dmu,
    float* __restrict__ dlogvar, size_t n, float scale, const float* __restrict__ gscale) {
    const float s = scale * (gscale ? gscale[0] : 1.f);
    const size_t nthreads = (size_t)gridDim.x * EW_THREADS;
    for (size_t i = (size_t)blockIdx.x * EW_THREADS + threadIdx.x; i < n; i += nthreads) {
        dmu[i] = s * mu[i];
        dlogvar[i] = s * 0.5f * (expf(logvar[i]) - 1.f);
    }
}

typedef unsigned int adam_u4 __attribute__((ext_vector_type(4)));
__global__ __launch_bounds__(EW_THREADS) void k_adam_amsgrad(
    float* __restrict__ p, const float* __restrict__ g, float* __restrict__ m,
    float* __restrict__ v, float* __restrict__ vmax, size_t n, float step_size, float b1,
    float b2, float bc2_sqrt, float eps, float wd, int vec) {
    const size_t tid = (size_t)blockIdx.x * EW_THREADS + threadIdx.x;
    const size_t nthreads = (size_t)gridDim.x * EW_THREADS;
    const float omb1 = 1.f - b1, omb2 = 1.f - b2;
#define ADAM_ONE(P, G, M, V, X)                                  \
    {                                                            \
        float gg = (G);                                          \
        if (wd != 0.f) gg = fmaf(wd, (P), gg);                   \
        (M) = (M) + omb1 * (gg - (M));                           \
        (V) = fmaf(omb2 * gg, gg, (V) * b2);                     \
        (X) = fmaxf((X), (V));                                   \
        const float denom = sqrtf(X) / bc2_sqrt + eps;           \
        (P) = (P) - step_size * ((M) / denom);                   \
    }
#define ADAM_ST(VAL, PTR)                                                                       \
    __builtin_amdgcn_raw_buffer_store_b128(                                                     \
        __builtin_bit_cast(adam_u4, VAL),                                                       \
        __builtin_amdgcn_make_buffer_rsrc((void*)(PTR), 0, (int)(n * 4), 0x00020000), o, 0, 16);
    if (vec) {
        const size_t n4 = n >> 2;
        float4* p4 = reinterpret_cast<float4*>(p);
        const float4* g4 = reinterpret_cast<const float4*>(g);
        float4* m4 = reinterpret_cast<float4*>(m);
        float4* v4 = reinterpret_cast<float4*>(v);
        float4* x4 = reinterpret_cast<float4*>(vmax);
        for (size_t i = tid; i < n4; i += nthreads) {
            float4 P = p4[i], M = m4[i], V = v4[i], X = x4[i];
            const float4 G = g4[i];
            ADAM_ONE(P.x, G.x, M.x, V.x, X.x)
            ADAM_ONE(P.y, G.y, M.y, V.y, X.y)
            ADAM_ONE(P.z, G.z, M.z, V.z, X.z)
            ADAM_ONE(P.w, G.w, M.w, V.w, X.w)
            if (vec == 2) {
                const int o = (int)(i << 4);
// ... 26 lines not shown
        for (size_t i = (n4 << 2) + tid; i < n; i += nthreads) out[i] = in[i] / 255.f;
    } else {
        for (size_t i = tid; i < n; i += nthreads) out[i] = in[i] / 255.f;
    }
}

int bn_launch_act_bwd(const float* dy, const float* y, float* dpre, size_t n, int act, float slope,
                      hipStream_t st) {
    const int vec = aligned16(dy) && aligned16(y) && aligned16(dpre);
    hipLaunchKernelGGL(k_act_bwd, dim3(ew_blocks(vec ? n / 4 + 1 : n)), dim3(EW_THREADS), 0, st, dy,
                       y, dpre, n, vec, act, slope);
    BN_LAUNCH_CHECK();
    return 0;
}

__global__ __launch_bounds__(EW_THREADS) void k_act_fwd(const float* __restrict__ x,
                                                        float* __restrict__ y, size_t n, int act,
                                                        float slope) {
    const size_t nthreads = (size_t)gridDim.x * EW_THREADS;
    for (size_t i = (size_t)blockIdx.x * EW_THREADS + threadIdx.x; i < n; i += nthreads)
        y[i] = bn_apply_act(x[i], act, slope);
}

int bn_launch_act_fwd(const float* x, float* y, size_t n, int act, float slope, hipStream_t st) {
    hipLaunchKernelGGL(k_act_fwd, dim3(ew_blocks(n)), dim3(EW_THREADS), 0, st, x, y, n, act, slope);
    BN_LAUNCH_CHECK();
    return 0;
}

int bn_launch_sqerr_frame_sums(const float* pred, const float* target, const float* mask,
                               float* frame_sums, int N, size_t D, hipStream_t st) {
    const int vec = aligned16(pred) && aligned16(target) && (!mask || aligned16(mask)) &&
                    (D % 4 == 0);
    hipLaunchKernelGGL(k_sqerr_frame_sums, dim3(N), dim3(EW_THREADS), 0, st, pred, target, mask,
                       frame_sums, D, vec);
    BN_LAUNCH_CHECK();
    return 0;
}

int bn_launch_sqerr_bwd(const float* pred, const float* target, const float* mask, float* dpred,
                        size_t n, float scale, const float* gscale, hipStream_t st) {
    const int vec = aligned16(pred) && aligned16(target) && aligned16(dpred) &&
                    (!mask || aligned16(mask));
    hipLaunchKernelGGL(k_sqerr_bwd, dim3(ew_blocks(vec ? n / 4 + 1 : n)), dim3(EW_THREADS), 0, st,
                       pred, target, mask, dpred, n, scale, gscale, vec);
    BN_LAUNCH_CHECK();
    return 0;
}

__global__ __launch_bounds__(EW_THREADS) void k_scale_frames(
    float* __restrict__ t, const float* __restrict__ frame_scale,
    const float* __restrict__ group_scale, const int* __restrict__ group_of_frame, size_t D,
    int vec) {
    const int n = blockIdx.y;
    float sc = frame_scale[n];
    if (group_scale) sc *= group_scale[group_of_frame[n]];
    float* row = t + (size_t)n * D;
    const size_t tid = (size_t)blockIdx.x * EW_THREADS + threadIdx.x;
    const size_t nthreads = (size_t)gridDim.x * EW_THREADS;
    if (vec) {
        float4* r4 = reinterpret_cast<float4*>(row);
        for (size_t i = tid; i < (D >> 2); i += nthreads) {
            float4 v = r4[i];
            v.x *= sc; v.y *= sc; v.z *= sc; v.w *= sc;
            r4[i] = v;
        }
    } else {
        for (size_t i = tid; i < D; i += nthreads) row[i] *= sc;
    }
}

int bn_launch_scale_frames(float* t, const float* frame_scale, const float* group_scale,
                           const int* group_of_frame, int N, size_t D, hipStream_t st) {
    const int vec = aligned16(t) && (D % 4 == 0);
    const size_t per = vec ? D / 4 : D;
    int bx = (int)((per + EW_THREADS - 1) / EW_THREADS);
    if (bx > 64) bx = 64;
    hipLaunchKernelGGL(k_scale_frames, dim3(bx, N), dim3(EW_THREADS), 0, st, t, frame_scale,
                       group_scale, group_of_frame, D, vec);
    BN_LAUNCH_CHECK();
    return 0;
}

int bn_launch_reduce_sum(const float* in, float* out, size_t n, float scale, hipStream_t st) {
    hipLaunchKernelGGL(k_reduce_sum, dim3(1), dim3(EW_THREADS), 0, st, in, out, n, scale);
    BN_LAUNCH_CHECK();
    return 0;
}

int bn_launch_reparam_fwd(const float* mu, const float* logvar, const float* eps, float* z,
                          size_t n, hipStream_t st) {
    hipLaunchKernelGGL(k_reparam_fwd, dim3(ew_blocks(n)), dim3(EW_THREADS), 0, st, mu, logvar, eps,
                       z, n);
    BN_LAUNCH_CHECK();
    return 0;
}

int bn_launch_kl_rows(const float* mu, const float* logvar, float* kl_rows, int N, int D,
                      hipStream_t st) {
    const int rows_per_block = EW_THREADS / BN_WAVE;
    hipLaunchKernelGGL(k_kl_rows, dim3((N + rows_per_block - 1) / rows_per_block),
                       dim3(EW_THREADS), 0, st, mu, logvar, kl_rows, N, D);
    BN_LAUNCH_CHECK();
    return 0;
}

int bn_launch_reparam_bwd(const float* dz, const float* z, const float* mu, float* dlogvar,
                          size_t n, hipStream_t st) {
    hipLaunchKernelGGL(k_reparam_bwd, dim3(ew_blocks(n)), dim3(EW_THREADS), 0, st, dz, z, mu,
                       dlogvar, n);
    BN_LAUNCH_CHECK();
    return 0;
}

int bn_launch_kl_bwd(const float* mu, const float* logvar, float* dmu, float* dlogvar, size_t n,
                     float scale, const float* gscale, hipStream_t st) {
    hipLaunchKernelGGL(k_kl_bwd, dim3(ew_blocks(n)), dim3(EW_THREADS), 0, st, mu, logvar, dmu,
                       dlogvar, n, scale, gscale);
    BN_LAUNCH_CHECK();
    return 0;
}

int bn_launch_adam(float* p, const float* g, float* m, float* v, float* vmax, size_t n, float lr,
                   float b1, float b2, float eps, float wd, int step, hipStream_t st) {
    const double bc1 = 1.0 - pow((double)b1, (double)step);
    const double bc2 = 1.0 - pow((double)b2, (double)step);
    const float step_size = (float)((double)lr / bc1);
    const float bc2_sqrt = (float)sqrt(bc2);
    int vec = aligned16(p) && aligned16(g) && aligned16(m) && aligned16(v) && aligned16(vmax);
    if (vec && n * 4 < 0x7fffffffull) vec = 2;
    BN_LAUNCH_MAIN(k_adam_amsgrad, dim3(ew_blocks(vec ? n / 4 + 1 : n)), dim3(EW_THREADS), 0,
                       st, p, g, m, v, vmax, n, step_size, b1, b2, bc2_sqrt, eps, wd, vec);
    BN_LAUNCH_CHECK();
    return 0;
}

int bn_launch_u8_to_unit_float(const unsigned char* in, float* out, size_t n, hipStream_t st) {
    const int vec = ((((uintptr_t)in) & 3u) == 0) && aligned16(out);
    hipLaunchKernelGGL(k_u8_to_unit_float, dim3(ew_blocks(vec ? n / 4 + 1 : n)), dim3(EW_THREADS),
                       0, st, in, out, n, vec);
    BN_LAUNCH_CHECK();
    return 0;
}
```

### behavenet_amd/csrc/gemm.hip

```cpp
#include <string.h>
#include "bn_common.h"
#include "bn_launch.h"

typedef float floatx16 __attribute__((ext_vector_type(16)));


__device__ __forceinline__ void gemm_tile(const GemmArgs& a, const int bx, const int by, const int bz,
                                          const int nw, const int ws, float* red,
                                          const bool live = true) {
    const int lane = threadIdx.x & 63;
    const int i0 = by * 32, j0 = bx * 32;
    const int li = lane & 31, lk = lane >> 5;

    const int zbeg = bz * a.kslice;
    const int zend = min(a.K, zbeg + a.kslice);
    int kper = (zend - zbeg + nw - 1) / nw;
    kper = (kper + 7) & ~7;
    const int kbeg = zbeg + ws * kper;
    const int kend = min(zend, kbeg + kper);

    const int ia = i0 + li, jb = j0 + li;
    const bool a_ok = ia < a.M, b_ok = jb < a.N;
    const float* ap = a.A + (long)(a_ok ? ia : 0) * a.sai;
    const float* bp = a.B + (long)(b_ok ? jb : 0) * a.sbj;

    floatx16 acc;
#pragma unroll
    for (int t = 0; t < 16; ++t) acc[t] = 0.f;

    const bool vec = (a.sak == 1) && (a.sbk == 1) && ((kbeg & 7) == 0) && ((kend & 3) == 0) && kend - kbeg >= 4 &&
                     ((a.sai & 3) == 0) && ((a.sbj & 3) == 0) &&
                     ((((uintptr_t)a.A) | ((uintptr_t)a.B)) & 15u) == 0;
    if (vec) {
        for (int k0 = kbeg; k0 < kend; k0 += 32) {
            float4 av4[4], bv4[4];
#pragma unroll
            for (int h = 0; h < 4; ++h) {
                const int k = min(k0 + 8 * h + 4 * lk, kend - 4);
                av4[h] = *reinterpret_cast<const float4*>(ap + k);
                bv4[h] = *reinterpret_cast<const float4*>(bp + k);
            }
#pragma unroll
            for (int h = 0; h < 4; ++h) {
                const bool ok = (k0 + 8 * h + 4 * lk) < kend;
                if (k0 + 8 * h >= kend) break;
                const float ax[4] = {av4[h].x, av4[h].y, av4[h].z, av4[h].w};
                const float bx4[4] = {bv4[h].x, bv4[h].y, bv4[h].z, bv4[h].w};
#pragma unroll
                for (int u = 0; u < 4; ++u)
                    acc = __builtin_amdgcn_mfma_f32_32x32x2f32((a_ok && ok) ? ax[u] : 0.f,
                                                               (b_ok && ok) ? bx4[u] : 0.f, acc, 0,
                                                               0, 0);
            }
        }
    }
    const bool veca = !vec && (a.sak == 1) && ((kbeg & 7) == 0) && ((kend & 3) == 0) && kend - kbeg >= 4 &&
                      ((a.sai & 3) == 0) && (((uintptr_t)a.A) & 15u) == 0;
    if (veca) {
        for (int k0 = kbeg; k0 < kend; k0 += 32) {
            float4 av4[4];
            float bs[4][4];
#pragma unroll
            for (int h = 0; h < 4; ++h) {
                const int k = min(k0 + 8 * h + 4 * lk, kend - 4);
                av4[h] = *reinterpret_cast<const float4*>(ap + k);
#pragma unroll
                for (int u = 0; u < 4; ++u) bs[h][u] = bp[(long)(k + u) * a.sbk];
            }
#pragma unroll
            for (int h = 0; h < 4; ++h) {
                const bool ok = (k0 + 8 * h + 4 * lk) < kend;
                if (k0 + 8 * h >= kend) break;
                const float ax[4] = {av4[h].x, av4[h].y, av4[h].z, av4[h].w};
#pragma unroll
                for (int u = 0; u < 4; ++u)
                    acc = __builtin_amdgcn_mfma_f32_32x32x2f32((a_ok && ok) ? ax[u] : 0.f,
                                                               (b_ok && ok) ? bs[h][u] : 0.f, acc, 0,
                                                               0, 0);
            }
        }
    }
    const int klast = max(kend - 1, kbeg);
    for (int k0 = kbeg + lk; k0 < ((vec || veca) ? 0 : kend + lk); k0 += 32) {
        float av[16], bv[16];
#pragma unroll
        for (int u = 0; u < 16; ++u) {
            const int k = min(k0 + 2 * u, klast);
            av[u] = ap[(long)k * a.sak];
            bv[u] = bp[(long)k * a.sbk];
        }
#pragma unroll
        for (int u = 0; u < 16; ++u) {
            const bool ok = (k0 + 2 * u) < kend;
            acc = __builtin_amdgcn_mfma_f32_32x32x2f32((a_ok && ok) ? av[u] : 0.f,
                                                       (b_ok && ok) ? bv[u] : 0.f, acc, 0, 0, 0);
        }
    }

    if (nw > 1) {
#pragma unroll
        for (int t = 0; t < 16; ++t) red[(ws * 16 + t) * 64 + lane] = acc[t];
        __syncthreads();
        if (ws != 0) return;
#pragma unroll
        for (int t = 0; t < 16; ++t) {
            float s = red[t * 64 + lane];
            for (int w2 = 1; w2 < nw; ++w2) s += red[(w2 * 16 + t) * 64 + lane];
            acc[t] = s;
        }
    }

    const int j = j0 + (lane & 31);
    if (j >= a.N || !live) return;
    if (a.part) {
#pragma unroll
        for (int t = 0; t < 16; ++t) {
            const int i = i0 + (t & 3) + 8 * (t >> 2) + 4 * (lane >> 5);
            if (i < a.M) a.part[((size_t)bz * a.M + i) * a.N + j] = acc[t];
        }
        return;
    }
    const float bj = a.bias_j ? a.bias_j[j] : 0.f;
#pragma unroll
    for (int t = 0; t < 16; ++t) {
        const int i = i0 + (t & 3) + 8 * (t >> 2) + 4 * (lane >> 5);
        if (i >= a.M) continue;
        const long off = (long)i * a.sci + (long)j * a.scj;
        float v = acc[t] + bj;
        if (a.dact_src) v *= bn_act_grad_from_output(a.dact_src[off], a.dact, a.slope);
        a.C[off] = a.accumulate ? a.C[off] + v : v;
    }
}

template <int SPLITK>
__global__ __launch_bounds__(64 * SPLITK) void k_gemm_mfma(GemmArgs a) {
    __shared__ float red[SPLITK > 1 ? SPLITK * 16 * 64 : 1];
    gemm_tile(a, blockIdx.x, blockIdx.y, blockIdx.z, SPLITK, threadIdx.x >> 6, red);
}

__global__ void k_gemm_combine(GemmArgs a, int slices);
#define GJ_WAVES 4
struct GemmJob { GemmArgs a; int tiles_x, tiles, slices, nw, blocks; };
struct LinearJobs {
    GemmJob g[2];
    const float* dy; float* db; int M, N, accumulate, db_blocks;
};

__global__ __launch_bounds__(64 * GJ_WAVES) void k_linear_jobs(LinearJobs p) {
    __shared__ float red[GJ_WAVES * 16 * 64];
    int b = blockIdx.x;
    const int wave = threadIdx.x >> 6;
#pragma unroll
    for (int q = 0; q < 2; ++q) {
        const GemmJob& job = p.g[q];
        if (b < job.blocks) {
            const int upb = GJ_WAVES / job.nw;
            const int units = job.tiles * job.slices;
            const int unit_w = b * upb + wave / job.nw;
            const bool live = unit_w < units;
            const int unit = live ? unit_w : units - 1;
            const int tile = unit / job.slices, slice = unit - tile * job.slices;
            gemm_tile(job.a, tile % job.tiles_x, tile / job.tiles_x, slice, job.nw, wave % job.nw,
                      red + (wave / job.nw) * job.nw * 1024, live);
            return;
        }
        b -= job.blocks;
    }
    const int col = b * 64 + (threadIdx.x & 63);
    float acc = 0.f;
    if (col < p.N) {
        for (int m0 = wave; m0 < p.M; m0 += 16 * GJ_WAVES) {
            float v[16];
#pragma unroll
            for (int u = 0; u < 16; ++u) {
                const int m = m0 + u * GJ_WAVES;
                v[u] = p.dy[(size_t)(m < p.M ? m : wave) * p.N + col];
            }
#pragma unroll
            for (int u = 0; u < 16; ++u)
                if (m0 + u * GJ_WAVES < p.M) acc += v[u];
        }
    }
    red[threadIdx.x] = acc;
    __syncthreads();
    if (wave == 0 && col < p.N) {
        float v = red[threadIdx.x];
        for (int w2 = 1; w2 < GJ_WAVES; ++w2) v += red[w2 * 64 + threadIdx.x];
        p.db[col] = p.accumulate ? p.db[col] + v : v;
    }
}

static int gemm_slices(int M, int N, int K) {
    const int tiles = ((N + 31) / 32) * ((M + 31) / 32);
    if (K < 1024 || tiles > 32) return 1;
    int s = K / 128;
    int cap = 16;
    while (cap < 128 && tiles * cap < 512 && K / (2 * cap) >= 256) cap *= 2;
    if (s > cap) s = cap;
    return s < 1 ? 1 : s;
}

static void gemm_job(GemmJob* j, const GemmArgs& a, float* part) {
    j->a = a;
    j->tiles_x = (a.N + 31) / 32;
    j->tiles = j->tiles_x * ((a.M + 31) / 32);
    j->slices = part ? gemm_slices(a.M, a.N, a.K) : 1;
    j->a.part = j->slices > 1 ? part : nullptr;
    j->a.kslice = ((a.K + j->slices - 1) / j->slices + 15) & ~15;
    const int kw = j->a.kslice / 32;
    j->nw = kw >= 4 ? 4 : kw >= 2 ? 2 : 1;
    const int upb = GJ_WAVES / j->nw, units = j->tiles * j->slices;
    j->blocks = (units + upb - 1) / upb;
}

size_t bn_linear_jobs_ws_bytes(int M, int N, int K) {
    const int s = gemm_slices(M, N, K);
    return s > 1 ? (size_t)s * M * N * sizeof(float) : 0;
}

int bn_launch_linear_jobs(const GemmArgs* g0, const GemmArgs* g1, const float* dy, float* db, int M,
                          int N, int accumulate, void* ws, size_t ws_bytes, hipStream_t st) {
    LinearJobs p;
    memset(&p, 0, sizeof(p));
    int blocks = 0;
    const GemmArgs* gs[2] = {g0, g1};
    char* wp = (char*)ws;
    for (int q = 0; q < 2; ++q)
        if (gs[q]) {
            const size_t need = bn_linear_jobs_ws_bytes(gs[q]->M, gs[q]->N, gs[q]->K);
            float* part = nullptr;
            if (need && wp && ws_bytes >= need) { part = (float*)wp; wp += need; ws_bytes -= need; }
            gemm_job(&p.g[q], *gs[q], part);
            blocks += p.g[q].blocks;
        }
    if (db) {
        p.dy = dy; p.db = db; p.M = M; p.N = N; p.accumulate = accumulate;
        p.db_blocks = (N + 63) / 64;
        blocks += p.db_blocks;
    }
    if (blocks == 0) return 0;
    BN_LAUNCH_MAIN(k_linear_jobs, dim3(blocks), dim3(64 * GJ_WAVES), 0, st, p);
    for (int q = 0; q < 2; ++q)
        if (gs[q] && p.g[q].slices > 1)
            hipLaunchKernelGGL(k_gemm_combine, dim3((gs[q]->M * gs[q]->N + 255) / 256), dim3(256), 0, st,
                               p.g[q].a, p.g[q].slices);
    BN_LAUNCH_CHECK();
    return 0;
}

#define GT_M 64
#define GT_N 128
#define GT_K 32
#define GT_LD 33
template <int TA, int TB>
__global__ __launch_bounds__(256) void k_gemm_tiled(GemmArgs a) {
    __shared__ float As[GT_M * GT_LD];
    __shared__ float Bs[GT_N * GT_LD];
    const int tid = threadIdx.x, lane = tid & 63;
    const int wv = __builtin_amdgcn_readfirstlane(tid >> 6);
    const int li = lane & 31, lk = lane >> 5;
    const int i0 = blockIdx.y * GT_M, j0 = blockIdx.x * GT_N;
    const int kbeg = blockIdx.z * a.kslice;
    const int kend = min(a.K, kbeg + a.kslice);

    const int ar = TA ? (tid & 7) * 8 : tid >> 2, ak = TA ? tid >> 3 : (tid & 3) * 8;
    const int br = TB ? (tid & 7) * 8 : tid >> 2, bk = TB ? tid >> 3 : (tid & 3) * 8;
    float ra[8], rb[2][8];
    auto fetch = [&](const int k0) __attribute__((always_inline)) {
        {
            const int i = i0 + ar, k = k0 + ak;
            const bool ok = TA ? (k < kend && i < a.M) : (i < a.M && k < kend);
            float4 v0 = make_float4(0.f, 0.f, 0.f, 0.f), v1 = v0;
            if (ok) {
                const float* p = a.A + (long)i * a.sai + (long)k * a.sak;
                v0 = *reinterpret_cast<const float4*>(p);
                v1 = *reinterpret_cast<const float4*>(p + 4);
            }
            ra[0] = v0.x; ra[1] = v0.y; ra[2] = v0.z; ra[3] = v0.w;
            ra[4] = v1.x; ra[5] = v1.y; ra[6] = v1.z; ra[7] = v1.w;
        }
#pragma unroll
        for (int h = 0; h < 2; ++h) {
            const int j = j0 + 64 * h + br, k = k0 + bk;
            const bool ok = j < a.N && k < kend;
            float4 v0 = make_float4(0.f, 0.f, 0.f, 0.f), v1 = v0;
            if (ok) {
                const float* p = a.B + (long)k * a.sbk + (long)j * a.sbj;
                v0 = *reinterpret_cast<const float4*>(p);
                v1 = *reinterpret_cast<const float4*>(p + 4);
            }
            rb[h][0] = v0.x; rb[h][1] = v0.y; rb[h][2] = v0.z; rb[h][3] = v0.w;
            rb[h][4] = v1.x; rb[h][5] = v1.y; rb[h][6] = v1.z; rb[h][7] = v1.w;
        }
    };

    floatx16 acc[2];
#pragma unroll
    for (int h = 0; h < 2; ++h)
#pragma unroll
        for (int t = 0; t < 16; ++t) acc[h][t] = 0.f;
    const float* ap = As + ((wv >> 1) * 32 + li) * GT_LD + lk;
    const float* bp = Bs + ((wv & 1) * 32 + li) * GT_LD + lk;

    if (kbeg < kend) fetch(kbeg);
    for (int k0 = kbeg; k0 < kend; k0 += GT_K) {
        __syncthreads();
#pragma unroll
        for (int e = 0; e < 8; ++e) {
            if (TA) As[(ar + e) * GT_LD + ak] = ra[e];
            else    As[ar * GT_LD + ak + e] = ra[e];
        }
#pragma unroll
        for (int h = 0; h < 2; ++h)
#pragma unroll
            for (int e = 0; e < 8; ++e) {
                if (TB) Bs[(64 * h + br + e) * GT_LD + bk] = rb[h][e];
                else    Bs[(64 * h + br) * GT_LD + bk + e] = rb[h][e];
            }
        __syncthreads();
#pragma unroll
        for (int t = 0; t < GT_K / 2; ++t) {
            const float av = ap[2 * t];
#pragma unroll
            for (int h = 0; h < 2; ++h)
                acc[h] = __builtin_amdgcn_mfma_f32_32x32x2f32(av, bp[64 * h * GT_LD + 2 * t], acc[h], 0, 0, 0);
            if (t == 1) {
                __builtin_amdgcn_sched_barrier(0);
                if (k0 + GT_K < kend) fetch(k0 + GT_K);
                __builtin_amdgcn_sched_barrier(0);
            }
        }
    }

#pragma unroll
    for (int h = 0; h < 2; ++h) {
        const int j = j0 + 64 * h + (wv & 1) * 32 + li;
        if (j >= a.N) continue;
        const float bj = (a.bias_j && !a.part) ? a.bias_j[j] : 0.f;
#pragma unroll
        for (int t = 0; t < 16; ++t) {
            const int i = i0 + (wv >> 1) * 32 + (t & 3) + 8 * (t >> 2) + 4 * lk;
            if (i >= a.M) continue;
            if (a.part) {
                a.part[((size_t)blockIdx.z * a.M + i) * a.N + j] = acc[h][t];
                continue;
            }
            const long off = (long)i * a.sci + (long)j * a.scj;
            float v = acc[h][t] + bj;
            if (a.dact_src) v *= bn_act_grad_from_output(a.dact_src[off], a.dact, a.slope);
            a.C[off] = a.accumulate ? a.C[off] + v : v;
        }
    }
}

__global__ __launch_bounds__(256) void k_gemm_combine(GemmArgs a, int slices) {
    const int idx = blockIdx.x * 256 + threadIdx.x;
    if (idx >= a.M * a.N) return;
    const int i = idx / a.N, j = idx - i * a.N;
    float v = 0.f;
    const size_t zs = (size_t)a.M * a.N;
    const float* p0 = a.part + (size_t)i * a.N + j;
    for (int z0 = 0; z0 < slices; z0 += 16) {
        float t[16];
#pragma unroll
        for (int u = 0; u < 16; ++u) t[u] = p0[(size_t)(z0 + u < slices ? z0 + u : z0) * zs];
#pragma unroll
        for (int u = 0; u < 16; ++u)
            if (z0 + u < slices) v += t[u];
    }
    if (a.bias_j) v += a.bias_j[j];
    const long off = (long)i * a.sci + (long)j * a.scj;
    if (a.dact_src) v *= bn_act_grad_from_output(a.dact_src[off], a.dact, a.slope);
    a.C[off] = a.accumulate ? a.C[off] + v : v;
}

__global__ __launch_bounds__(64) void k_col_sum(const float* __restrict__ dy,
                                                float* __restrict__ db, int M, int N,
                                                int accumulate) {
    const int n = blockIdx.x;
    float acc = 0.f;
    for (int m = threadIdx.x; m < M; m += 64) acc += dy[(size_t)m * N + n];
#pragma unroll
    for (int off = 32; off > 0; off >>= 1) acc += __shfl_down(acc, off, 64);
    if (threadIdx.x == 0) db[n] = accumulate ? db[n] + acc : acc;
}

static int gemm_tiled_slices(int M, int N, int K) {
    const int tiles = ((N + GT_N - 1) / GT_N) * ((M + GT_M - 1) / GT_M);
    if (tiles >= 256 || K < 512) return 1;
    int s = 512 / tiles;
    if (s > K / 128) s = K / 128;
    if (s > 64) s = 64;
    return s < 1 ? 1 : s;
}

size_t bn_gemm_ws_bytes(int M, int N, int K) {
    const int s = gemm_slices(M, N, K);
    size_t need = s > 1 ? (size_t)s * M * N * sizeof(float) : 0;
    if (M >= 64 && N >= 64 && K >= 64) {
        const size_t t = (size_t)gemm_tiled_slices(M, N, K) * M * N * sizeof(float);
        if (gemm_tiled_slices(M, N, K) > 1 && t > need) need = t;
    }
    return need;
}

static bool gemm_tiled_ok(const GemmArgs& a, int* ta, int* tb) {
    if (a.M < 64 || a.N < 64 || a.K < 64 || (size_t)a.M * a.N < 64 * 1024) return false;
    if ((((uintptr_t)a.A) | ((uintptr_t)a.B)) & 15u) return false;
    if (a.sak == 1) { *ta = 0; if ((a.K & 7) || (a.sai & 3)) return false; }
    else if (a.sai == 1) { *ta = 1; if ((a.M & 7) || (a.sak & 3)) return false; }
    else return false;
    if (a.sbk == 1) { *tb = 0; if ((a.K & 7) || (a.sbj & 3)) return false; }
    else if (a.sbj == 1) { *tb = 1; if ((a.N & 7) || (a.sbk & 3)) return false; }
    else return false;
    return true;
}
int bn_launch_gemm(const GemmArgs& a0, hipStream_t st, void* ws, size_t ws_bytes) {
    GemmArgs a = a0;
    int ta = 0, tb = 0;
    if (gemm_tiled_ok(a, &ta, &tb)) {
        int slices = gemm_tiled_slices(a.M, a.N, a.K);
        if (slices > 1 && (!ws || ws_bytes < (size_t)slices * a.M * a.N * sizeof(float))) slices = 1;
        a.kslice = ((a.K + slices - 1) / slices + GT_K - 1) / GT_K * GT_K;
        a.part = slices > 1 ? (float*)ws : nullptr;
        dim3 grid((a.N + GT_N - 1) / GT_N, (a.M + GT_M - 1) / GT_M, slices);
        if (grid.y < 65536) {
            if (ta == 0 && tb == 0) hipLaunchKernelGGL((k_gemm_tiled<0, 0>), grid, dim3(256), 0, st, a);
            else if (ta == 0) hipLaunchKernelGGL((k_gemm_tiled<0, 1>), grid, dim3(256), 0, st, a);
            else if (tb == 0) hipLaunchKernelGGL((k_gemm_tiled<1, 0>), grid, dim3(256), 0, st, a);
            else hipLaunchKernelGGL((k_gemm_tiled<1, 1>), grid, dim3(256), 0, st, a);
            if (slices > 1)
                hipLaunchKernelGGL(k_gemm_combine, dim3((a.M * a.N + 255) / 256), dim3(256), 0, st, a, slices);
            BN_LAUNCH_CHECK();
            return 0;
        }
    }
    a = a0;
    int slices = gemm_slices(a.M, a.N, a.K);
    if (slices > 1 && (!ws || ws_bytes < (size_t)slices * a.M * a.N * sizeof(float))) slices = 1;
    a.kslice = ((a.K + slices - 1) / slices + 15) & ~15;
    a.part = slices > 1 ? (float*)ws : nullptr;
    dim3 grid((a.N + 31) / 32, (a.M + 31) / 32, slices);
    if (a.K >= 512) {
        hipLaunchKernelGGL(k_gemm_mfma<8>, grid, dim3(512), 0, st, a);
    } else if (a.K >= 128) {
        hipLaunchKernelGGL(k_gemm_mfma<4>, grid, dim3(256), 0, st, a);
    } else {
        hipLaunchKernelGGL(k_gemm_mfma<1>, grid, dim3(64), 0, st, a);
    }
    if (slices > 1)
        hipLaunchKernelGGL(k_gemm_combine, dim3((a.M * a.N + 255) / 256), dim3(256), 0, st, a,
                           slices);
    BN_LAUNCH_CHECK();
    return 0;
}

int bn_launch_col_sum(const float* dy, float* db, int M, int N, int accumulate, hipStream_t st) {
    hipLaunchKernelGGL(k_col_sum, dim3(N), dim3(64), 0, st, dy, db, M, N, accumulate);
    BN_LAUNCH_CHECK();
    return 0;
}
```

### behavenet_amd/hip_functions.py

```python

import collections.abc
import contextlib
import os
import threading
import warnings

import torch

from behavenet_amd import _hip

LRELU_SLOPE = 0.05

_direct_grads = False


class accumulate_into_param_grads(object):

    def __enter__(self):
        global _direct_grads
        self._prev = _direct_grads
        _direct_grads = True

    def __exit__(self, *exc):
        global _direct_grads
# ... 302 lines not shown

def _fwd(layer, x, w, b, w5=None):
    g = layer.geom(x.shape[0])
    if layer.kind == 'conv':
        if x.dtype == torch.uint8:
            return _hip.conv2d_fwd_u8(x, w, b, g, layer.act, LRELU_SLOPE)
        return _hip.conv2d_fwd(x, w, b, g, layer.act, LRELU_SLOPE, w5=w5)
    return _hip.convT2d_fwd(x, w, b, g, layer.act, LRELU_SLOPE, w5=w5)


_FWD_OP = {'conv': _hip.OP_CONV_FWD, 'convT': _hip.OP_CONVT_FWD}
_BWD_OP = {'conv': _hip.OP_CONV_BWD_D, 'convT': _hip.OP_CONVT_BWD_D}


def _stack_taps(plan, n, params, first=0):
    jobs, idx = [], []
    for i in range(first, len(plan)):
        layer = plan[i]
        g = layer.geom(n)
        for op in (_FWD_OP[layer.kind], _BWD_OP[layer.kind]):
            if _hip.conv_taps_bytes(op, g):
                jobs.append((op, g, params[2 * i].detach()))
                idx.append(i)
                break
    if not jobs:
        return None
    taps = [None] * len(plan)
    for i, w5 in zip(idx, _hip.conv_taps_pad(jobs, params[0].device)):
        taps[i] = w5
    return taps


def first_layer_forward(plan, x, params):
    return _fwd(plan[0], x.contiguous(), params[0].detach(), params[1].detach())


_sign_tap = None


def _note_signs(plan, i, h):
    if _sign_tap is not None and plan[i].act == _hip.ACT_LRELU:
        _sign_tap.setdefault(id(plan), [[] for _ in plan])[i].append((h.detach() > 0).cpu())


class ConvStackFn(torch.autograd.Function):

    @staticmethod
    def forward(ctx, plan, x, h1, *params):
        if x.shape[1:] != (plan[0].cin, plan[0].hin, plan[0].win):
            raise ValueError('conv stack expects input (N,%d,%d,%d), got %s' % (
                plan[0].cin, plan[0].hin, plan[0].win, tuple(x.shape)))
        x = x.contiguous()
        acts = [x]
        h = x
        skip_first = h1 is not None and not x.requires_grad
        taps = _stack_taps(plan, x.shape[0], params, first=1 if skip_first else 0) if x.is_cuda else None
        for i, layer in enumerate(plan):
            if i == 0 and h1 is not None:
                h = h1
            else:
                h = _fwd(layer, h, params[2 * i].detach(), params[2 * i + 1].detach(),
                         w5=taps[i] if taps else None)
            acts.append(h)
        for i in range(len(plan)):
            _note_signs(plan, i, acts[i + 1])
        ctx.plan = plan
        ctx.taps = taps
        ctx.need_dx = x.requires_grad
        ctx.param_refs = params
        _note_use(params, any(ctx.needs_input_grad[3:]))
        ctx.save_for_backward(*acts, *params[0::2])
        return h

    @staticmethod
    def backward(ctx, dout):
        plan = ctx.plan
        dout = dout.contiguous()
        top = plan[-1]
        if top.act != _hip.ACT_NONE:
            dpre = _hip.act_bwd(dout, ctx.saved_tensors[len(plan)], top.act, LRELU_SLOPE)
        else:
            dpre = dout
        dx, grads = _stack_backward(ctx, dpre, first_param=3)
        return (None, dx, None) + tuple(grads)


def _stack_backward(ctx, dpre, first_param):
    plan = ctx.plan
    n_layers = len(plan)
    saved = ctx.saved_tensors
    acts, weights = saved[:n_layers + 1], saved[n_layers + 1:2 * n_layers + 1]
    n = dpre.shape[0]
    grads = [None] * (2 * n_layers)
    taps = getattr(ctx, 'taps', None)
    for i in range(n_layers - 1, -1, -1):
        layer = plan[i]
        g = layer.geom(n)
        w = weights[i]
        x_in = acts[i]
        if x_in.dtype == torch.uint8:
            x_in = _hip.u8_to_unit_float(x_in) \
                if ctx.needs_input_grad[first_param + 2 * i] else None
        need_w = ctx.needs_input_grad[first_param + 2 * i]
        need_b = ctx.needs_input_grad[first_param + 1 + 2 * i]
        if need_w:
            gw = _grad_buffer(ctx.param_refs[2 * i])
            gb = _grad_buffer(ctx.param_refs[2 * i + 1]) if need_b else None
            direct = gw is not None and (gb is not None or not need_b)
            if direct:
                dw, db = gw, gb
            else:
                dw = torch.empty_like(w)
                db = torch.empty((layer.cout,), dtype=w.dtype, device=w.device) if need_b \
                    else None
            wgrad = _hip.conv2d_bwd_weight if layer.kind == 'conv' else _hip.convT2d_bwd_weight
            side = _side_stream(w.device) if (direct and _use_side_stream) else None
            if side is not None:
                main = torch.cuda.current_stream(w.device)
                ev = torch.cuda.Event()
                ev.record(main)
                with torch.cuda.stream(side):
                    side.wait_event(ev)
                    wgrad(x_in, dpre, dw, db, g, True)
                dpre.record_stream(side)
                x_in.record_stream(side)
                _report_ready(ctx.param_refs[2 * i:2 * i + 2])
            else:
                wgrad(x_in, dpre, dw, db, g, direct)
                if direct:
                    _report_ready(ctx.param_refs[2 * i:2 * i + 2])
            if not direct:
                grads[2 * i], grads[2 * i + 1] = dw, db
        if i > 0 or ctx.need_dx:
            dact_src = acts[i] if i > 0 else None
            dact = plan[i - 1].act if i > 0 else _hip.ACT_NONE
            w5 = taps[i] if taps else None
            if layer.kind == 'conv':
                dpre = _hip.conv2d_bwd_data(dpre, w, g, dact_src, dact, LRELU_SLOPE, w5=w5)
            else:
                dpre = _hip.convT2d_bwd_data(dpre, w, g, dact_src, dact, LRELU_SLOPE, w5=w5)
    return (dpre if ctx.need_dx else None), grads


def conv_stack(plan, x, params, h1=None):
    return ConvStackFn.apply(plan, x, h1, *params)


ENCODE_DTYPES = ('f32', 'bf16')
_encode_tls = threading.local()


def encode_dtype():
    return getattr(_encode_tls, 'dtype', 'f32')


@contextlib.contextmanager
def encode_precision(dtype):
    if dtype not in ENCODE_DTYPES:
        raise ValueError("encode_precision: dtype must be one of %s, got %r" % (ENCODE_DTYPES, dtype))
    prev = encode_dtype()
    _encode_tls.dtype = dtype
    try:
        yield
    finally:
        _encode_tls.dtype = prev


def warn_bf16_unserved(owner, reason):
    if getattr(owner, '_bf16_warned', False):
        return
    owner._bf16_warned = True
    warnings.warn('bf16 encoding was requested but this model runs its fp32 encoder: %s' % reason)


def stack_unserved_reason_bf16(plan):
    if len(plan) < 2:
        return 'a stack of one layer has no matrix-core layer'
    for i, layer in enumerate(plan):
        if layer.kind != 'conv' or layer.act not in (_hip.ACT_NONE, _hip.ACT_LRELU):
            return 'layer %d (%r) is not a convolution with a LeakyReLU / no activation' % (i, layer)
        if not _hip.conv2d_bf16_ok(layer.geom(1), first=(i == 0)):
            return 'layer %d (%r) is not served by the bf16 kernels' % (i, layer)
    return None


def stack_served_bf16(plan):
    return stack_unserved_reason_bf16(plan) is None


def conv_stack_bf16(plan, x, params):
    if torch.is_grad_enabled() and (x.requires_grad or any(p.requires_grad for p in params)):
        raise RuntimeError('conv_stack_bf16 is inference only: call it under torch.no_grad()')
    if x.shape[1:] != (plan[0].cin, plan[0].hin, plan[0].win):
        raise ValueError('conv stack expects input (N,%d,%d,%d), got %s' % (
            plan[0].cin, plan[0].hin, plan[0].win, tuple(x.shape)))
    reason = stack_unserved_reason_bf16(plan)
    if reason is not None:
        raise RuntimeError('conv_stack_bf16: %s' % reason)
    x = x.contiguous()
    n = x.shape[0]
    sizes = [_hip.conv_pack_w_bf16_bytes(params[2 * i].shape) for i in range(1, len(plan))]
    packed = torch.empty(sum(sizes), dtype=torch.uint8, device=x.device)
    wps, o = [None], 0
    for i, sz in zip(range(1, len(plan)), sizes):
        wps.append(_hip.conv_pack_w_bf16(params[2 * i].detach(), packed[o:o + sz]))
        o += sz
    h = _hip.conv2d_first_bf16(x, params[0].detach(), params[1].detach(), plan[0].geom(n), plan[0].act,
                               LRELU_SLOPE)
    for i in range(1, len(plan)):
        h = _hip.conv2d_fwd_bf16(h, wps[i], params[2 * i + 1].detach(), plan[i].geom(n), plan[i].act,
                                 LRELU_SLOPE, out_f32=(i == len(plan) - 1))
    return h


DECODE_DTYPES = ('f32', 'bf16')
_decode_tls = threading.local()


def decode_dtype():
    return getattr(_decode_tls, 'dtype', 'f32')


@contextlib.contextmanager
def decode_precision(dtype):
    if dtype not in DECODE_DTYPES:
        raise ValueError("decode_precision: dtype must be one of %s, got %r" % (DECODE_DTYPES, dtype))
    prev = decode_dtype()
# ... 77 lines not shown
def frame_err_request():
    return getattr(_frame_err_tls, 'req', None)


@contextlib.contextmanager
def scoring_frames(target, mask, scale):
    if frame_u8_request() is not None:
        raise RuntimeError('scoring_frames: a quantising request is open; a decoder call serves one of the two')
    prev = frame_err_request()
    req = _frame_err_tls.req = FrameErrRequest(target, mask, scale)
    try:
        yield req
    finally:
        _frame_err_tls.req = prev


_frame_u8_tls = threading.local()


class FrameU8Request(object):

    def __init__(self):
        self.frames = None


def frame_u8_request():
    return getattr(_frame_u8_tls, 'req', None)


@contextlib.contextmanager
def quantising_frames():
    if frame_err_request() is not None:
        raise RuntimeError('quantising_frames: a scoring request is open; a decoder call serves one of the two')
    prev = frame_u8_request()
    req = _frame_u8_tls.req = FrameU8Request()
    try:
        yield req
    finally:
        _frame_u8_tls.req = prev


_frame_scale_cache = {}


def _frame_scales(n, bounds, scales, device):
    key = (torch.device(device), int(n), tuple(bounds), tuple(float(s) for s in scales))
    hit = _frame_scale_cache.get(key)
    if hit is None:
        fs = torch.zeros(n, dtype=torch.float32)
        ci = torch.zeros(n, dtype=torch.int32)
        for c, ((beg, end), sc) in enumerate(zip(bounds, scales)):
            fs[beg:end] = float(sc)
            ci[beg:end] = c
        hit = (fs.to(device), ci.to(device))
        if len(_frame_scale_cache) > 64:
            _frame_scale_cache.clear()
        _frame_scale_cache[key] = hit
    return hit


class ConvStackSqErrFn(torch.autograd.Function):

    @staticmethod
    def forward(ctx, plan, x, target, mask, bounds, scales, want_xhat, *params):
        if plan[-1].kind != 'convT':
            raise ValueError('the fused pixel loss follows a transposed convolution')
        x = x.contiguous()
        target = target.contiguous()
        mask = mask.contiguous() if mask is not None else None
        acts = [x]
        h = x
        taps = _stack_taps(plan, x.shape[0], params) if x.is_cuda else None
        for i, layer in enumerate(plan[:-1]):
            h = _fwd(layer, h, params[2 * i].detach(), params[2 * i + 1].detach(), w5=taps[i] if taps else None)
            acts.append(h)
        top = plan[-1]
        n = h.shape[0]
        xhat, dpre, part = _hip.convT2d_fwd_sqerr(
            h, params[-2].detach(), params[-1].detach(), target, mask, top.geom(n), top.act,
            LRELU_SLOPE, bool(want_xhat))
        for i in range(len(plan) - 1):
            _note_signs(plan, i, acts[i + 1])
        out = torch.empty((len(bounds),), dtype=torch.float32, device=x.device)
        for c, ((beg, end), sc) in enumerate(zip(bounds, scales)):
            _hip.reduce_sum(part[beg:end], float(sc), out=out[c:c + 1])
        ctx.plan = plan
        ctx.taps = taps
        ctx.need_dx = x.requires_grad
        ctx.param_refs = params
        ctx.bounds, ctx.scales = list(bounds), [float(sc) for sc in scales]
        ctx.consumed = False
        _note_use(params, any(ctx.needs_input_grad[7:]))
        ctx.save_for_backward(*acts, dpre, *params[0::2])
        if xhat is not None:
            ctx.mark_non_differentiable(xhat)
        return out, xhat

    @staticmethod
    def backward(ctx, g, _g_xhat):
        if ctx.consumed:
            raise RuntimeError('ConvStackSqErrFn: backward twice (dL/dpre is scaled in place)')
        ctx.consumed = True
        n_layers = len(ctx.plan)
        dpre = ctx.saved_tensors[n_layers]
        fs, ci = _frame_scales(dpre.shape[0], ctx.bounds, ctx.scales, dpre.device)
        _hip.scale_frames(dpre, fs, g.contiguous(), ci)
        dx, grads = _stack_backward(ctx, dpre, first_param=7)
        return (None, dx, None, None, None, None, None) + tuple(grads)


def conv_stack_sq_err(plan, x, params, target, mask, bounds, scales, want_xhat=False):
    return ConvStackSqErrFn.apply(plan, x, target, mask, tuple(bounds), tuple(scales),
                                  bool(want_xhat), *params)


class FusedPixelLoss(object):

    def __init__(self, x_hat, chunk_terms, kind, bounds):
        self.x_hat = x_hat
        self.chunk_terms = chunk_terms
        self.kind = kind
        self.bounds = list(bounds)


_DEVICE_CONSTANTS = {}


def device_constant(values, device):
    key = (tuple(float(v) for v in values), str(device))
    t = _DEVICE_CONSTANTS.get(key)
    if t is None:
        if len(_DEVICE_CONSTANTS) > 256:
            _DEVICE_CONSTANTS.clear()
        t = torch.tensor(key[0], dtype=torch.float32, device=device)
        _DEVICE_CONSTANTS[key] = t
    return t


def pixel_loss_scales(kind, bounds, per_frame, chunk_sizes=None):
    sizes = chunk_sizes if chunk_sizes is not None else [end - beg for beg, end in bounds]
    if kind == 'mse':
        return [1.0 / (n * per_frame) for n in sizes]
    if kind == 'll':
        return [-0.5 / n for n in sizes]
    raise ValueError('unknown pixel loss kind "%s"' % kind)


_bn_bounds = None


class bn_chunks(object):
    def __init__(self, bounds):
        self.bounds = [(int(b), int(e)) for b, e in bounds if e > b]

    def __enter__(self):
        global _bn_bounds
        self._prev, _bn_bounds = _bn_bounds, (self.bounds if len(self.bounds) > 1 else None)
        return self

    def __exit__(self, *exc):
        global _bn_bounds
        _bn_bounds = self._prev
        return False


def _batches_tracked(module, added=1):
    t = module.num_batches_tracked
    mirror = getattr(module, '_bn_count_mirror', None)
# ... 84 lines not shown
        ctx.param_refs = (gamma, beta)
        ctx.from_x = ctx.chunks is not None and act in (_hip.ACT_NONE, _hip.ACT_LRELU)
        ctx.beta = b
        if ctx.from_x:
            ctx.save_for_backward(x, mean, invstd, g)
        else:
            ctx.save_for_backward(x, y, mean, invstd, g)
        return y

    @staticmethod
    def backward(ctx, dy):
        if ctx.from_x:
            x, mean, invstd, g = ctx.saved_tensors
            y = None
        else:
            x, y, mean, invstd, g = ctx.saved_tensors
        gamma, beta = ctx.param_refs
        need_g = gamma is not None and ctx.needs_input_grad[1]
        need_b = beta is not None and ctx.needs_input_grad[2]
        gg = _grad_buffer(gamma) if need_g else None
        gb = _grad_buffer(beta) if need_b else None
        direct = (need_g or need_b) and (gg is not None or not need_g) and \
            (gb is not None or not need_b)
        if getattr(ctx, 'sync_count', None) is not None:
            from behavenet_amd.fitting import distributed as bdist
            dx, sum_dz, sum_dzx = _hip.batchnorm_sync_bwd(
                x, y, dy.contiguous(), mean, invstd, g, ctx.sync_count, ctx.act, LRELU_SLOPE,
                bdist.all_reduce_)
            if direct:
                if need_g:
                    gg.add_(sum_dzx)
                if need_b:
                    gb.add_(sum_dz)
                return (dx if ctx.needs_input_grad[0] else None), None, None, None, None
            return (dx if ctx.needs_input_grad[0] else None), \
                (sum_dzx if need_g else None), (sum_dz if need_b else None), None, None
        chunks = getattr(ctx, 'chunks', None)
        if chunks is not None:
            dy = dy.contiguous()
            if direct:
                dgamma, dbeta = gg, gb
            else:
                dgamma = torch.zeros_like(mean[0]) if need_g else None
                dbeta = torch.zeros_like(mean[0]) if need_b else None
            dx = _hip.batchnorm_bwd_chunks(x, y, dy, mean, invstd, g, dgamma, dbeta, True, ctx.act,
                                           LRELU_SLOPE, chunks, beta=ctx.beta)
            if direct:
                dgamma = dbeta = None
            return (dx if ctx.needs_input_grad[0] else None), dgamma, dbeta, None, None
        if direct:
            dgamma, dbeta = gg, gb
        else:
            dgamma = torch.empty_like(mean) if need_g else None
            dbeta = torch.empty_like(mean) if need_b else None
        dx = _hip.batchnorm_bwd(x, y, dy.contiguous(), mean, invstd, g, dgamma, dbeta, direct,
                                ctx.batch_stats, ctx.act, LRELU_SLOPE)
        if direct:
            dgamma = dbeta = None
        return (dx if ctx.needs_input_grad[0] else None), dgamma, dbeta, None, None


def conv_stack_bn(plan, x, params, bn_modules):
    h = x
    run_plan, run_params = [], []
    for i, layer in enumerate(plan):
        run_params += [params[2 * i], params[2 * i + 1]]
        if bn_modules[i] is None:
            run_plan.append(layer)
            continue
        run_plan.append(layer.with_act(_hip.ACT_NONE))
        h = ConvStackFn.apply(run_plan, h, None, *run_params)
        bn = bn_modules[i]
        h = BatchNormActFn.apply(h, bn.weight, bn.bias, bn, layer.act)
        _note_signs(plan, i, h)
        run_plan, run_params = [], []
    if run_plan:
        h = ConvStackFn.apply(run_plan, h, None, *run_params)
    return h


class LinearFn(torch.autograd.Function):

    @staticmethod
    def forward(ctx, x, w, b):
        x = x.contiguous()
        ctx.save_for_backward(x, w)
        ctx.has_bias = b is not None
        ctx.param_refs = (w, b)
        _note_use((w, b), ctx.needs_input_grad[1])
        return _hip.linear_fwd(x, w.detach().contiguous(),
                               b.detach() if b is not None else None)

    @staticmethod
    def backward(ctx, dy):
        x, w = ctx.saved_tensors
        dy = dy.contiguous()
        need_dx, need_dw = ctx.needs_input_grad[0], ctx.needs_input_grad[1]
        need_db = ctx.has_bias and ctx.needs_input_grad[2]
        gw = _grad_buffer(ctx.param_refs[0]) if need_dw else None
        gb = _grad_buffer(ctx.param_refs[1]) if need_db else None
        direct = need_dw and gw is not None and (gb is not None or not need_db)
        if direct:
            dw, db = gw, gb
        else:
            dw = torch.empty_like(w) if need_dw else None
            db = torch.empty((w.shape[0],), dtype=w.dtype, device=w.device) if need_db else None
        wc = w.contiguous()
        if direct and _use_side_stream:
            dx = _hip.linear_bwd(x, wc, dy, need_dx, None, _hip.ACT_NONE, 0.0, None, None, False) \
                if need_dx else None
            side = _side_stream(w.device)
            ev = torch.cuda.Event()
            ev.record(torch.cuda.current_stream(w.device))
            with torch.cuda.stream(side):
                side.wait_event(ev)
                _hip.linear_bwd(x, wc, dy, False, None, _hip.ACT_NONE, 0.0, dw, db, True)
            dy.record_stream(side)
            x.record_stream(side)
            _report_ready(ctx.param_refs)
            return dx, None, None
        dx = _hip.linear_bwd(x, wc, dy, need_dx, None, _hip.ACT_NONE, 0.0, dw, db, direct)
        if direct:
            _report_ready(ctx.param_refs)
            return dx, None, None
        return dx, dw, db


def linear(x, w, b=None):
    return LinearFn.apply(x, w, b)


class SqErrFn(torch.autograd.Function):

    @staticmethod
    def forward(ctx, a, b, mask, scale):
        a, b = a.contiguous(), b.contiguous()
        mask = mask.contiguous() if mask is not None else None
        ctx.save_for_backward(a, b, mask)
        ctx.scale = float(scale)
        sums = _hip.sqerr_frame_sums(a, b, mask)
        return _hip.reduce_sum(sums, scale)

    @staticmethod
    def backward(ctx, g):
        a, b, mask = ctx.saved_tensors
        g = g.contiguous()
        da = db = None
        if ctx.needs_input_grad[0]:
            da = _hip.sqerr_bwd(a, b, mask, ctx.scale, g)
        if ctx.needs_input_grad[1]:
            db = _hip.sqerr_bwd(b, a, mask, ctx.scale, g)
        return da, db, None, None


def sq_err(a, b, mask, scale):
    return SqErrFn.apply(a, b, mask, scale)


class ChunkedSqErrFn(torch.autograd.Function):

    @staticmethod
    def forward(ctx, a, b, mask, bounds, scales):
        a, b = a.contiguous(), b.contiguous()
        mask = mask.contiguous() if mask is not None else None
        ctx.save_for_backward(a, b, mask)
        ctx.bounds, ctx.scales = list(bounds), [float(s) for s in scales]
        sums = _hip.sqerr_frame_sums(a, b, mask)
        out = torch.empty((len(ctx.bounds),), dtype=torch.float32, device=a.device)
        for i, ((beg, end), s) in enumerate(zip(ctx.bounds, ctx.scales)):
            _hip.reduce_sum(sums[beg:end], s, out=out[i:i + 1])
        return out

    @staticmethod
    def backward(ctx, g):
        a, b, mask = ctx.saved_tensors
        g = g.contiguous()
        grads = []
        for need, p, t in ((ctx.needs_input_grad[0], a, b), (ctx.needs_input_grad[1], b, a)):
            if not need:
                grads.append(None)
                continue
            d = torch.empty_like(p)
            for i, ((beg, end), s) in enumerate(zip(ctx.bounds, ctx.scales)):
                _hip.sqerr_bwd(p[beg:end], t[beg:end], mask[beg:end] if mask is not None else None,
                               s, g[i:i + 1], out=d[beg:end])
            grads.append(d)
        return grads[0], grads[1], None, None, None


def chunked_sq_err(a, b, mask, bounds, scales):
    return ChunkedSqErrFn.apply(a, b, mask, bounds, scales)


class ReparamFn(torch.autograd.Function):

    @staticmethod
    def forward(ctx, mu, logvar, eps):
        mu, logvar, eps = mu.contiguous(), logvar.contiguous(), eps.contiguous()
        z = _hip.reparam_fwd(mu, logvar, eps)
        ctx.save_for_backward(mu, z)
        return z

    @staticmethod
    def backward(ctx, dz):
        mu, z = ctx.saved_tensors
        dz = dz.contiguous()
        dlogvar = _hip.reparam_bwd(dz, z, mu) if ctx.needs_input_grad[1] else None
        return (dz if ctx.needs_input_grad[0] else None), dlogvar, None


def reparameterize_with_eps(mu, logvar, eps):
    return ReparamFn.apply(mu, logvar, eps)


class KLFn(torch.autograd.Function):

    @staticmethod
    def forward(ctx, mu, logvar):
        mu, logvar = mu.contiguous(), logvar.contiguous()
        ctx.save_for_backward(mu, logvar)
        rows = _hip.kl_rows(mu, logvar)
        return _hip.reduce_sum(rows, 1.0 / mu.shape[0])

    @staticmethod
    def backward(ctx, g):
        mu, logvar = ctx.saved_tensors
        dmu, dlogvar = _hip.kl_bwd(mu, logvar, 1.0 / mu.shape[0], g.contiguous())
        return dmu, dlogvar


class ActFn(torch.autograd.Function):

    @staticmethod
    def forward(ctx, x, act):
        y = _hip.act_fwd(x.contiguous(), act, LRELU_SLOPE)
        ctx.act = act
        ctx.save_for_backward(y)
        return y

    @staticmethod
    def backward(ctx, dy):
        (y,) = ctx.saved_tensors
        return _hip.act_bwd(dy.contiguous(), y, ctx.act, LRELU_SLOPE), None


def activation(x, act):
    return ActFn.apply(x, act)


class MaxPoolFn(torch.autograd.Function):

    @staticmethod
    def forward(ctx, x, k, stride, pad, out_hw):
# ... 366 lines not shown
```

### behavenet_amd/models/aes.py

```python

import os

import numpy as np
import torch
from torch import nn

import behavenet_amd.fitting.losses as losses
from behavenet_amd import _hip
from behavenet_amd.fitting import distributed as bdist
from behavenet_amd.models.base import BaseModule, BaseModel
from behavenet_amd.hip_functions import (
    ChunkScalars, ConvLayerPlan, FusedPixelLoss, Readback, activation, backward_chunks, bn_chunks,
    capturing, finish_loss, conv_stack_bf16, encode_dtype, stack_unserved_reason_bf16, warn_bf16_unserved,
    convT_stack_bf16, decode_dtype, decode_precision, frame_err_request, frame_u8_request,
    stack_unserved_reason_bf16_dec, warn_bf16_unserved_dec,
    chunked_sq_err, conv_stack, conv_stack_bn, conv_stack_sq_err, first_layer_forward,
    join_side_streams, linear, begin_chunks, chunk_stream, max_pool, max_pool_act, max_unpool, conv_pool_act,
    pixel_loss_scales, reserve_device_pools, _note_signs)

__all__ = [
    'ConvAEEncoder', 'ConvAEDecoder', 'LinearAEEncoder', 'LinearAEDecoder', 'AE', 'ConditionalAE',
    'AEMSP',
    'load_pretrained_ae', 'encoder_input']

# ... 77 lines not shown
            args, pads = self._get_conv2d_args(i, gnum)
            if hp.get('fit_sess_io_layers', False) and i == 0:
                name = 'conv%i_sess_io_layers' % gnum
                self.encoder.add_module(name, nn.ModuleList([
                    _mark_footprint(nn.Conv2d(**args)) for _ in range(hp['n_datasets'])]))
            else:
                name = 'conv%i' % gnum
                self.encoder.add_module(name, _mark_footprint(nn.Conv2d(**args)))
            if hp['ae_batch_norm']:
                self.encoder.add_module('batchnorm%i' % gnum, nn.BatchNorm2d(
                    hp['ae_encoding_n_channels'][i],
                    momentum=hp.get('ae_batch_norm_momentum', 0.1),
                    track_running_stats=hp.get('track_running_stats', True)))
            pool = None
            if i < n_layers - 1 and hp['ae_encoding_layer_type'][i + 1] == 'maxpool':
                pargs = self._get_maxpool2d_args(i)
                self.encoder.add_module('maxpool%i' % gnum, _mark_footprint(nn.MaxPool2d(**pargs)))
                pool = (pargs['kernel_size'], pargs['stride'], pargs['padding'],
                        (hp['ae_encoding_y_dim'][i + 1], hp['ae_encoding_x_dim'][i + 1]))
            self._pool_after.append(pool)
            self.encoder.add_module('relu%i' % gnum, nn.LeakyReLU(0.05))

            if i == 0:
                hin, win = hp['ae_input_dim'][1], hp['ae_input_dim'][2]
            else:
                hin, win = hp['ae_encoding_y_dim'][i - 1], hp['ae_encoding_x_dim'][i - 1]
            k = args['kernel_size']
            self._plan.append(ConvLayerPlan(
                'conv', args['in_channels'], hin, win, args['out_channels'],
                hp['ae_encoding_y_dim'][i], hp['ae_encoding_x_dim'][i], k, k, args['stride'],
                pads[0], pads[1], _hip.ACT_LRELU))
            self._layer_names.append(name)
            gnum += 1

        last = hp['ae_encoding_n_channels'][-1] * hp['ae_encoding_y_dim'][-1] * \
            hp['ae_encoding_x_dim'][-1]
        self.FF = _mark_footprint(nn.Linear(last, hp['n_ae_latents']))
        if hp.get('variational', False):
            self.logvar = _mark_footprint(nn.Linear(last, hp['n_ae_latents']))

    def _get_conv2d_args(self, layer, global_layer):
        hp = self.hparams
        if layer == 0:
            extra = 0
            if hp['model_class'] == 'cond-ae' and hp.get('conditional_encoder', False):
                extra = int(hp['n_labels'] / 2)
            in_channels = hp['ae_input_dim'][0] + extra
        else:
            in_channels = hp['ae_encoding_n_channels'][layer - 1]
        x0, x1 = hp['ae_encoding_x_padding'][layer]
        y0, y1 = hp['ae_encoding_y_padding'][layer]
        if x0 == x1 and y0 == y1:
            padding = (y0, x0)
        else:
            self.encoder.add_module('zero_pad%i' % global_layer, nn.ZeroPad2d((x0, x1, y0, y1)))
            padding = 0
        args = {
            'in_channels': in_channels,
            'out_channels': hp['ae_encoding_n_channels'][layer],
            'kernel_size': hp['ae_encoding_kernel_size'][layer],
            'stride': hp['ae_encoding_stride_size'][layer],
            'padding': padding}
        return args, (y0, x0)

    def _get_maxpool2d_args(self, layer):
        hp = self.hparams
        return {
            'kernel_size': int(hp['ae_encoding_kernel_size'][layer + 1]),
            'stride': int(hp['ae_encoding_stride_size'][layer + 1]),
            'padding': (hp['ae_encoding_y_padding'][layer + 1][0],
                        hp['ae_encoding_x_padding'][layer + 1][0]),
            'return_indices': True,
            'ceil_mode': hp['ae_padding_type'] != 'valid'}

    def _stack_params(self, dataset):
        params = []
        for name in self._layer_names:
            mod = getattr(self.encoder, name)
            if isinstance(mod, nn.ModuleList):
                mod = mod[dataset]
            params += [mod.weight, mod.bias]
        return params

    def _features(self, x, dataset=None):
        hp = self.hparams
        self._pool_state = ([], [])
        if encode_dtype() == 'bf16' and self._bf16_eligible(x):
            h = conv_stack_bf16(self._plan, x, self._stack_params(dataset))
            return h.view(h.size(0), -1)
        if any(p is not None for p in self._pool_after):
            return self._features_pooled(x, dataset)
        if hp['ae_batch_norm']:
            h = conv_stack_bn(self._plan, x, self._stack_params(dataset),
                              _bn_modules(self.encoder, self._layer_names))
        else:
            h = conv_stack(self._plan, x, self._stack_params(dataset),
                           h1=self._first_layer_slice(x, dataset))
        return h.view(h.size(0), -1)

    def _bf16_eligible(self, x):
        if self.training or torch.is_grad_enabled():
            reason = 'the encoder is in training mode or gradients are enabled'
        elif any(p is not None for p in self._pool_after):
            reason = 'max-pooling architectures are not served'
        elif self.hparams['ae_batch_norm']:
            reason = 'batch-norm architectures are not served'
        elif self._plan and self._plan[0].cin != self.hparams['ae_input_dim'][0]:
            reason = 'extra input channels (conditional_encoder) are not served'
        elif not x.is_cuda or x.dtype not in (torch.float32, torch.uint8):
            reason = 'the frames are not fp32 / uint8 device tensors'
        else:
            reason = stack_unserved_reason_bf16(self._plan)
        if reason is None:
            return True
        warn_bf16_unserved(self, reason)
        return False

    def _features_pooled(self, x, dataset):
        params = self._stack_params(dataset)
        bns = _bn_modules(self.encoder, self._layer_names)
        pool_idx, sizes = [], []
        h = x
        for j, layer in enumerate(self._plan):
            pool = self._pool_after[j]
            one = [layer.with_act(_hip.ACT_NONE) if pool is not None else layer]
            fused = None
            if pool is not None and bns[j] is None:
                fused = conv_pool_act(one[0], h, params[2 * j:2 * j + 2], *pool, _hip.ACT_LRELU)
            if fused is not None:
                sizes.append(torch.Size((h.size(0), layer.cout, layer.hout, layer.wout)))
                h, idx = fused
                pool_idx.append(idx)
                _note_signs(self._plan, j, h)
                continue
            if bns[j] is not None:
                h = conv_stack_bn(one, h, params[2 * j:2 * j + 2], [bns[j]])
            else:
                h = conv_stack(one, h, params[2 * j:2 * j + 2])
            if pool is not None:
                k, stride, pad, out_hw = pool
                sizes.append(h.size())
                h, idx = max_pool_act(h, k, stride, pad, out_hw, _hip.ACT_LRELU)
                pool_idx.append(idx)
            _note_signs(self._plan, j, h)
        self._pool_state = (pool_idx, sizes)
        return h.reshape(h.size(0), -1)

    def _pool_out(self):
        state = getattr(self, '_pool_state', ([], []))
        self._pool_state = ([], [])
        return state

    def prepare_first_layer(self, x_all, dataset=None):
        self._h1_cache = None
        if self.hparams['ae_batch_norm'] or not x_all.is_cuda or not x_all.is_contiguous() \
                or tuple(x_all.shape[1:]) != (self._plan[0].cin, self._plan[0].hin,
                                              self._plan[0].win):
            return
        with torch.no_grad():
            h1 = first_layer_forward(self._plan, x_all, self._stack_params(dataset))
        self._h1_cache = (x_all, h1, dataset)

    def release_first_layer(self):
        self._h1_cache = None

    def _first_layer_slice(self, x, dataset):
        cache = getattr(self, '_h1_cache', None)
        if cache is None:
            return None
        x_all, h1, ds = cache
        frame_bytes = x_all[0].numel() * x_all.element_size()
        delta = x.data_ptr() - x_all.data_ptr()
        if ds != dataset or not x.is_contiguous() or x.shape[1:] != x_all.shape[1:] or \
                delta < 0 or delta % frame_bytes != 0:
            return None
        beg = delta // frame_bytes
        if beg + x.shape[0] > x_all.shape[0]:
            return None
        return h1[beg:beg + x.shape[0]]

    def forward(self, x, dataset=None):
        x1 = self._features(x, dataset)
        pool_idx, sizes = self._pool_out()
        if self.hparams.get('variational', False):
            return (linear(x1, self.FF.weight, self.FF.bias),
                    linear(x1, self.logvar.weight, self.logvar.bias), pool_idx, sizes)
        return linear(x1, self.FF.weight, self.FF.bias), pool_idx, sizes


class ConvAEDecoder(BaseModule):

    def __init__(self, hparams):
        super().__init__()
        self.hparams = hparams
        self.decoder = None
        self.build_model()

    def __str__(self):
        out = 'Decoder architecture:\n'
        out += '    {:02d}: {}\n'.format(0, self.FF)
        for i, module in enumerate(self.decoder):
            out += '    {:02d}: {}\n'.format(i + 1, module)
        return out

    def build_model(self):
        hp = self.hparams
        start = hp['ae_decoding_starting_dim']
        self.FF = _mark_footprint(nn.Linear(hp['hidden_layer_size'], start[0] * start[1] * start[2]))
        self.decoder = nn.ModuleList()
        self.conv_t_pads = {}
        self._layer_names = []
        self._plan = []
        self._unpool_before = []
        n_layers = len(hp['ae_decoding_n_channels'])
        gnum = 0
        for i in range(n_layers):
            if hp['ae_decoding_layer_type'][i] != 'convtranspose':
                continue
            self._unpool_before.append(i > 0 and hp['ae_decoding_layer_type'][i - 1] == 'unpool')
            if i > 0 and hp['ae_decoding_layer_type'][i - 1] == 'unpool':
                k = int(hp['ae_decoding_kernel_size'][i - 1])
                s = int(hp['ae_decoding_stride_size'][i - 1])
                self.decoder.add_module('maxunpool%i' % gnum, _mark_footprint(nn.MaxUnpool2d(
                    kernel_size=(k, k), stride=(s, s),
                    padding=(hp['ae_decoding_y_padding'][i - 1][0],
                             hp['ae_decoding_x_padding'][i - 1][0]))))
            args, crop, out_hw = self._get_convtranspose2d_args(i, gnum)
            is_last = i == n_layers - 1 and not hp['ae_decoding_last_FF_layer']
            if hp.get('fit_sess_io_layers', False) and is_last:
                name = 'convtranspose%i_sess_io_layers' % gnum
                self.decoder.add_module(name, nn.ModuleList([
                    _mark_footprint(nn.ConvTranspose2d(**args))
                    for _ in range(hp['n_datasets'])]))
                self.conv_t_pads[name] = self.conv_t_pads['convtranspose%i' % gnum]
            else:
                name = 'convtranspose%i' % gnum
                self.decoder.add_module(name, _mark_footprint(nn.ConvTranspose2d(**args)))
            if is_last:
                self.decoder.add_module('sigmoid%i' % gnum, nn.Sigmoid())
                act = _hip.ACT_SIGMOID
            else:
                if hp['ae_batch_norm']:
                    self.decoder.add_module('batchnorm%i' % gnum, nn.BatchNorm2d(
                        hp['ae_decoding_n_channels'][i],
                        momentum=hp.get('ae_batch_norm_momentum', 0.1),
                        track_running_stats=hp.get('track_running_stats', True)))
                self.decoder.add_module('relu%i' % gnum, nn.LeakyReLU(0.05))
                act = _hip.ACT_LRELU

            if i == 0:
                hin, win = start[1], start[2]
            else:
                hin, win = hp['ae_decoding_y_dim'][i - 1], hp['ae_decoding_x_dim'][i - 1]
            k = args['kernel_size'][0]
            self._plan.append(ConvLayerPlan(
                'convT', args['in_channels'], hin, win, args['out_channels'], out_hw[0], out_hw[1],
                k, k, args['stride'][0], crop[0], crop[1], act))
            self._layer_names.append(name)
            gnum += 1

        if hp['ae_decoding_last_FF_layer']:
            if hp.get('fit_sess_io_layers', False):
                raise NotImplementedError
            self.decoder.add_module('last_ff%i' % gnum, _mark_footprint(nn.Linear(
                hp['ae_decoding_x_dim'][-1] * hp['ae_decoding_y_dim'][-1] *
                hp['ae_decoding_n_channels'][-1],
                hp['ae_input_dim'][0] * hp['ae_input_dim'][1] * hp['ae_input_dim'][2])))
            self.decoder.add_module('sigmoid%i' % gnum, nn.Sigmoid())
            self._last_ff_name = 'last_ff%i' % gnum

# ... 599 lines not shown
```

### include/behavenet_hip.h

```cpp
#ifndef BEHAVENET_HIP_H
#define BEHAVENET_HIP_H

#include <stddef.h>

#ifdef __cplusplus
extern "C" {
#endif

#define BN_E_BADARG   (-1)
#define BN_E_SHAPE    (-2)
#define BN_E_WORKSPACE (-3)

#define BN_ACT_NONE    0
#define BN_ACT_LRELU   1
#define BN_ACT_SIGMOID 2

typedef void* bn_stream_t;

int         bn_version(void);
const char* bn_build_arch(void);
const char* bn_error_string(int code);

#define BN_OP_CONV_FWD    1
#define BN_OP_CONV_BWD_D  2
// ... 25 lines not shown
                         int accumulate, void* ws, size_t ws_bytes, bn_stream_t stream);

int bn_convT2d_fwd(const float* x, const float* w, const float* w5, const float* b, float* y,
                   int N, int Ci, int Hi, int Wi, int Co, int R, int S, int stride,
                   int crop_t, int crop_l, int Ho, int Wo,
                   int act, float slope, void* ws, size_t ws_bytes, bn_stream_t stream);

int bn_convT2d_bwd_data(const float* dy, const float* w, const float* w5, float* dx, const float* dact_src,
                        int N, int Ci, int Hi, int Wi, int Co, int R, int S, int stride,
                        int crop_t, int crop_l, int Ho, int Wo,
                        int dact, float slope, void* ws, size_t ws_bytes, bn_stream_t stream);

int bn_convT2d_bwd_weight(const float* x, const float* dy, float* dw, float* db,
                          int N, int Ci, int Hi, int Wi, int Co, int R, int S, int stride,
                          int crop_t, int crop_l, int Ho, int Wo,
                          int accumulate, void* ws, size_t ws_bytes, bn_stream_t stream);

int bn_act_fwd(const float* x, float* y, size_t n, int act, float slope, bn_stream_t stream);
int bn_act_bwd(const float* dy, const float* y, float* dpre, size_t n,
               int act, float slope, bn_stream_t stream);

int bn_maxpool2d_fwd(const float* x, float* y, int* idx, int planes, int H, int W, int Ho, int Wo,
                     int k, int stride, int pad_t, int pad_l, bn_stream_t stream);
int bn_maxpool2d_bwd(const float* dy, const int* idx, float* dx, int planes, int H, int W,
                     int Ho, int Wo, int k, int stride, int pad_t, int pad_l, bn_stream_t stream);
int bn_conv2d_pool2_act_fwd(const float* x, const float* w, const float* b, float* y, int* idx,
                            int N, int C, int H, int W, int K, int R, int S, int stride,
                            int pad_t, int pad_l, int P, int Q, int act, float slope, bn_stream_t stream);
int bn_conv2d_pool2_act_ok(int N, int C, int H, int W, int K, int R, int S, int stride,
                           int pad_t, int pad_l, int P, int Q);
size_t bn_conv2d_pool2_bwd_weight_ws_bytes(int N, int C, int H, int W, int K, int R, int S, int stride,
                                           int pad_t, int pad_l, int P, int Q);
int bn_conv2d_pool2_bwd_weight(const float* x, const float* dy, const float* y, const int* idx, float* dw, float* db,
                               int N, int C, int H, int W, int K, int R, int S, int stride,
                               int pad_t, int pad_l, int P, int Q, int act, float slope, int accumulate,
                               void* ws, size_t ws_bytes, bn_stream_t stream);
int bn_maxpool2d_act_fwd(const float* x, float* y, int* idx, int planes, int H, int W, int act, float slope,
                         bn_stream_t stream);
int bn_maxpool2d_act_bwd(const float* dy, const float* y, const int* idx, float* dx, int planes, int H, int W,
                         int act, float slope, bn_stream_t stream);
int bn_maxunpool2d_fwd(const float* x, const int* idx, float* y, int planes, int in_plane,
                       int out_plane, bn_stream_t stream);
int bn_maxunpool2d_fwd_k2(const float* x, const int* idx, float* y, int planes, int Hi, int Wi, bn_stream_t stream);
int bn_maxunpool2d_bwd(const float* dy, const int* idx, float* dx, int planes, int in_plane,
                       int out_plane, bn_stream_t stream);

size_t bn_batchnorm_ws_bytes(int N, int C);
int bn_batchnorm_stats(const float* x, float* mean, float* var, int N, int C, int HW,
                       void* ws, size_t ws_bytes, bn_stream_t stream);
int bn_batchnorm_finalize(const float* mean, const float* var, float* invstd,
                          float* running_mean, float* running_var, int C, float eps,
                          float momentum, float unbias, bn_stream_t stream);
int bn_batchnorm_act_fwd(const float* x, const float* mean, const float* invstd,
                         const float* gamma, const float* beta, float* y, int N, int C, int HW,
                         int act, float slope, bn_stream_t stream);
int bn_batchnorm_act_bwd(const float* x, const float* y, const float* dy, const float* mean,
                         const float* invstd, const float* gamma, float* dx, float* dgamma,
                         float* dbeta, int accumulate, int batch_stats, int N, int C, int HW,
                         int act, float slope, void* ws, size_t ws_bytes, bn_stream_t stream);

int bn_batchnorm_train_fwd_chunks(const float* x, const float* gamma, const float* beta,
                                  float* running_mean, float* running_var,
                                  long long* num_batches_tracked, float* y, float* mean,
                                  float* invstd, const int* bounds, const float* factors,
                                  int n_chunks, int C, int HW, float eps, int act, float slope,
                                  void* ws, size_t ws_bytes, bn_stream_t stream);
int bn_batchnorm_act_bwd_chunks(const float* x, const float* y, const float* dy, const float* mean,
                                const float* invstd, const float* gamma, const float* beta,
                                float* dx, float* dgamma, float* dbeta, int accumulate,
                                const int* bounds, int n_chunks, int C, int HW, int act, float slope,
                                void* ws, size_t ws_bytes, bn_stream_t stream);

int bn_batchnorm_moment(const float* x, const float* center, float* sums, int N, int C, int HW,
                        void* ws, size_t ws_bytes, bn_stream_t stream);
int bn_batchnorm_bwd_reduce(const float* x, const float* y, const float* dy, const float* mean,
                            const float* invstd, float* sum_dz, float* sum_dzx, int N, int C,
                            int HW, int act, float slope, void* ws, size_t ws_bytes,
                            bn_stream_t stream);
int bn_batchnorm_bwd_apply(const float* x, const float* y, const float* dy, const float* mean,
                           const float* invstd, const float* gamma, const float* sum_dz,
                           const float* sum_dzx, float* dx, int N, int C, int HW, float inv_count,
                           int act, float slope, bn_stream_t stream);

size_t bn_linear_ws_bytes(int M, int K, int N);
int bn_linear_fwd(const float* x, const float* w, const float* b, float* y,
                  int M, int K, int N, void* ws, size_t ws_bytes, bn_stream_t stream);
int bn_linear_bwd(const float* x, const float* w, const float* dy,
                  float* dx, const float* dact_src, int dact, float slope,
                  float* dw, float* db, int accumulate,
                  int M, int K, int N, void* ws, size_t ws_bytes, bn_stream_t stream);

int bn_sqerr_frame_sums(const float* pred, const float* target, const float* mask,
                        float* frame_sums, int N, size_t D, bn_stream_t stream);
int bn_sqerr_bwd(const float* pred, const float* target, const float* mask, float* dpred,
                 size_t n, float scale, const float* gscale, bn_stream_t stream);
int bn_reduce_sum(const float* in, float* out, size_t n, float scale, bn_stream_t stream);

int bn_reparam_fwd(const float* mu, const float* logvar, const float* eps, float* z,
                   size_t n, bn_stream_t stream);
int bn_kl_rows(const float* mu, const float* logvar, float* kl_rows, int N, int D,
               bn_stream_t stream);
int bn_reparam_bwd(const float* dz, const float* z, const float* mu, float* dlogvar, size_t n,
                   bn_stream_t stream);
int bn_kl_bwd(const float* mu, const float* logvar, float* dmu, float* dlogvar, size_t n,
              float scale, const float* gscale, bn_stream_t stream);

int bn_decomposed_kl_fwd(const float* z, const float* mu, const float* logvar, float* out3,
                         float* log_qz, float* lse, float* terms, int N, int D,
                         bn_stream_t stream);
int bn_decomposed_kl_bwd(const float* z, const float* mu, const float* logvar,
                         const float* log_qz, const float* lse, const float* g3, float* dz,
                         float* dmu, float* dlogvar, int N, int D, bn_stream_t stream);

int bn_psvae_head_fwd(const float* y, const float* w, const float* logvar, const float* eps,
                      const float* Dw, const float* Db, const float* labels, const float* lmask,
                      float* z, float* z_u, float* lv_u, float* yhat, float* row_sq,
                      float* row_kl, int N, int L, int U, bn_stream_t stream);
int bn_psvae_head_combine(const float* row_sq, const float* row_kl, const float* dkl3,
                          const int* bounds, int n_chunks, float alpha, float kl, float beta,
                          int L, float* T, float* cols5, bn_stream_t stream);
int bn_psvae_head_bwd(const float* dz, const float* gT, const int* bounds, int n_chunks,
                      const float* y, const float* logvar, const float* eps, const float* yhat,
                      const float* labels, const float* lmask, const float* Dw, const float* gz_u,
                      const float* gmu_u, const float* glv_u, float alpha, float* dy, float* dw,
                      float* dlogvar, float* dDw, float* dDb, int accumulate, int N, int L, int U,
                      bn_stream_t stream);

int bn_convT2d_fwd_sqerr_parts(int N, int Ci, int Hi, int Wi, int Co, int R, int S, int stride,
                               int crop_t, int crop_l, int Ho, int Wo);
size_t bn_convT2d_fwd_sqerr_ws_bytes(int N, int Ci, int Hi, int Wi, int Co, int R, int S,
                                     int stride, int crop_t, int crop_l, int Ho, int Wo,
                                     int with_xhat);
int bn_convT2d_fwd_sqerr(const float* x, const float* w, const float* b, const float* target,
                         const float* mask, float* xhat, float* dpre, float* part,
                         int N, int Ci, int Hi, int Wi, int Co, int R, int S, int stride,
                         int crop_t, int crop_l, int Ho, int Wo, int act, float slope,
                         void* ws, size_t ws_bytes, bn_stream_t stream);
int bn_scale_frames(float* t, const float* frame_scale, const float* group_scale,
                    const int* group_of_frame, int N, size_t D, bn_stream_t stream);

int bn_adam_amsgrad_step(float* p, const float* g, float* m, float* v, float* vmax, size_t n,
                         float lr, float beta1, float beta2, float eps, float weight_decay,
                         int step, bn_stream_t stream);

size_t bn_conv2d_fwd_u8_ws_bytes(int N, int C, int H, int W, int K, int R, int S, int stride,
                                 int pad_t, int pad_l, int P, int Q, int act);
int bn_conv2d_fwd_u8(const unsigned char* x, const float* w, const float* b, float* y,
                     int N, int C, int H, int W, int K, int R, int S, int stride,
                     int pad_t, int pad_l, int P, int Q, int act, float slope,
                     void* ws, size_t ws_bytes, bn_stream_t stream);

int bn_conv2d_first_bf16_ok(int N, int C, int H, int W, int K, int R, int S, int stride,
                            int pad_t, int pad_l, int P, int Q);
int bn_conv2d_bf16_ok(int N, int C, int H, int W, int K, int R, int S, int stride,
                      int pad_t, int pad_l, int P, int Q);
size_t bn_conv_pack_w_bf16_bytes(int K, int C, int R, int S);
int bn_conv_pack_w_bf16(const float* w, void* wp, int K, int C, int R, int S, bn_stream_t stream);
int bn_conv2d_first_bf16(const void* x, int x_is_u8, const float* w, const float* b, void* y,
                         int N, int C, int H, int W, int K, int R, int S, int stride,
                         int pad_t, int pad_l, int P, int Q, int act, float slope, bn_stream_t stream);
int bn_conv2d_fwd_bf16(const void* x, const void* wp, const float* b, void* y, int out_f32,
                       int N, int C, int H, int W, int K, int R, int S, int stride,
                       int pad_t, int pad_l, int P, int Q, int act, float slope, bn_stream_t stream);

int bn_convT2d_bf16_ok(int N, int Ci, int Hi, int Wi, int Co, int R, int S, int stride,
                       int off_t, int off_l, int Ho, int Wo);
int bn_convT2d_last_bf16_ok(int N, int Ci, int Hi, int Wi, int Co, int R, int S, int stride,
                            int off_t, int off_l, int Ho, int Wo);
size_t bn_convT_pack_w_bf16_bytes(int Ci, int Co, int R, int S);
int bn_convT_pack_w_bf16(const float* w, void* wp, int Ci, int Co, int R, int S, bn_stream_t stream);
int bn_to_nhwc_bf16(const float* x, void* y, int N, int C, int H, int W, bn_stream_t stream);
int bn_convT2d_fwd_bf16(const void* x, const void* wp, const float* b, void* y, int out_f32,
                        int N, int Ci, int Hi, int Wi, int Co, int R, int S, int stride,
                        int off_t, int off_l, int Ho, int Wo, int act, float slope, bn_stream_t stream);
int bn_convT2d_last_bf16(const void* x, const float* w, const float* b, float* y,
                         int N, int Ci, int Hi, int Wi, int Co, int R, int S, int stride,
                         int off_t, int off_l, int Ho, int Wo, int act, float slope, bn_stream_t stream);

size_t bn_convT2d_last_bf16_sqerr_ws_bytes(int N, int Ci, int Hi, int Wi, int Co, int R, int S,
// ... 70 lines not shown
```

Baseline: 58920 frames/s.

## Fuse split-K linear combine via tickets, batch chunk reductions, fold encoder activation grad

Split-K linear GEMMs now take a device ticket buffer, so the last-arriving block combines the partial slices in the same kernel instead of launching a separate combine kernel. Per-chunk reduce_sum calls in the loss and conv paths become one chunked-reduction launch. The conv edge weight-gradient path merges the bias and first weight partial sums into one launch. The encoder's last activation gradient moves into the linear backward through dact_src. These changes target launch overhead but add atomic and fence synchronisation, plus a ticket buffer that must be reset correctly.

After: 59150 frames/s (median of 6 runs). Within noise of the previous version (+0.4%).

```diff
diff --git a/behavenet_amd/_hip.py b/behavenet_amd/_hip.py
--- a/behavenet_amd/_hip.py
+++ b/behavenet_amd/_hip.py
@@ -75,10 +75,10 @@
     'bn_act_fwd': (_c_int, [_c_void_p] * 2 + [_c_size_t, _c_int, _c_float, _c_void_p]),
     'bn_act_bwd': (_c_int, [_c_void_p] * 3 + [_c_size_t, _c_int, _c_float, _c_void_p]),
     'bn_linear_ws_bytes': (_c_size_t, [_c_int] * 3),
-    'bn_linear_fwd': (_c_int, [_c_void_p] * 4 + [_c_int] * 3 + [_c_void_p, _c_size_t, _c_void_p]),
+    'bn_linear_fwd': (_c_int, [_c_void_p] * 4 + [_c_int] * 3 + [_c_void_p, _c_size_t, _c_void_p, _c_void_p]),
     'bn_linear_bwd': (
         _c_int, [_c_void_p] * 5 + [_c_int, _c_float, _c_void_p, _c_void_p, _c_int] +
-        [_c_int] * 3 + [_c_void_p, _c_size_t, _c_void_p]),
+        [_c_int] * 3 + [_c_void_p, _c_size_t, _c_void_p, _c_void_p]),
     'bn_sqerr_frame_sums': (_c_int, [_c_void_p] * 4 + [_c_int, _c_size_t, _c_void_p]),
     'bn_sqerr_bwd': (_c_int, [_c_void_p] * 4 + [_c_size_t, _c_float, _c_void_p, _c_void_p]),
     'bn_convT2d_fwd_sqerr_parts': (_c_int, _CONV_GEOM),
@@ -87,6 +87,7 @@
         _c_int, [_c_void_p] * 8 + _CONV_GEOM + [_c_int, _c_float, _c_void_p, _c_size_t, _c_void_p]),
     'bn_scale_frames': (_c_int, [_c_void_p] * 4 + [_c_int, _c_size_t, _c_void_p]),
     'bn_reduce_sum': (_c_int, [_c_void_p] * 2 + [_c_size_t, _c_float, _c_void_p]),
+    'bn_reduce_sum_chunks': (_c_int, [_c_void_p] * 5 + [_c_int, _c_void_p]),
     'bn_reparam_fwd': (_c_int, [_c_void_p] * 4 + [_c_size_t, _c_void_p]),
     'bn_kl_rows': (_c_int, [_c_void_p] * 3 + [_c_int, _c_int, _c_void_p]),
     'bn_reparam_bwd': (_c_int, [_c_void_p] * 4 + [_c_size_t, _c_void_p]),
@@ -224,6 +225,27 @@
     return buf.data_ptr()
 
 
+TICKET_WORDS = 4096
+_ticket_cache = {}
+
+
+def _tickets(device):
+    if torch.cuda.is_current_stream_capturing():
+        return torch.zeros(TICKET_WORDS, dtype=torch.int32, device=device)
+    device = torch.device(device)
+    key = (device, torch.cuda.current_stream(device).cuda_stream)
+    buf = _ticket_cache.get(key)
+    if buf is None:
+        with torch.cuda.stream(torch.cuda.current_stream(device)):
+            buf = torch.zeros(TICKET_WORDS, dtype=torch.int32, device=device)
+        _ticket_cache[key] = buf
+    return buf
+
+
+def _drop_tickets(device):
+    _ticket_cache.pop((torch.device(device), torch.cuda.current_stream(device).cuda_stream), None)
+
+
 def _workspace(op, geom, device):
     if torch.device(device).type != 'cuda':
         raise HipLibraryError(
@@ -751,27 +773,39 @@
     return _arena(device, nbytes, 'linear'), nbytes
 
 
-def linear_fwd(x, w, b):
+def linear_fwd(x, w, b, second_pass=False):
     M, K = x.shape
     N = w.shape[0]
     y = torch.empty((M, N), dtype=torch.float32, device=x.device)
+    split = load().bn_linear_ws_bytes(M, K, N) > 0
+    tk = _tickets(x.device) if split and not second_pass else None
     ws, nb = _linear_ws(M, K, N, x.device)
-    _check(load().bn_linear_fwd(
-        _ptr(x, 'x'), _ptr(w, 'w'), _ptr(b, 'b', allow_none=True), _ptr(y, 'y'), M, K, N,
-        ws, nb, _stream()), 'bn_linear_fwd')
+    try:
+        _check(load().bn_linear_fwd(
+            _ptr(x, 'x'), _ptr(w, 'w'), _ptr(b, 'b', allow_none=True), _ptr(y, 'y'), M, K, N,
+            ws, nb, _stream(), _ptr(tk, 'tickets', torch.int32, allow_none=True)), 'bn_linear_fwd')
+    except HipLibraryError:
+        _drop_tickets(x.device)
+        raise
     return y
 
 
-def linear_bwd(x, w, dy, need_dx, dact_src, dact, slope, dw, db, accumulate):
+def linear_bwd(x, w, dy, need_dx, dact_src, dact, slope, dw, db, accumulate, second_pass=False):
     M, N = dy.shape
     K = w.shape[1]
     dx = torch.empty((M, K), dtype=torch.float32, device=dy.device) if need_dx else None
+    split = need_dx and load().bn_linear_ws_bytes(M, K, N) > 0
+    tk = _tickets(dy.device) if split and not second_pass else None
     ws, nb = _linear_ws(M, K, N, dy.device) if need_dx else (None, 0)
-    _check(load().bn_linear_bwd(
-        _ptr(x, 'x', allow_none=True), _ptr(w, 'w'), _ptr(dy, 'dy'),
-        _ptr(dx, 'dx', allow_none=True), _ptr(dact_src, 'dact_src', allow_none=True), dact, slope,
-        _ptr(dw, 'dw', allow_none=True), _ptr(db, 'db', allow_none=True), int(accumulate),
-        M, K, N, ws, nb, _stream()), 'bn_linear_bwd')
+    try:
+        _check(load().bn_linear_bwd(
+            _ptr(x, 'x', allow_none=True), _ptr(w, 'w'), _ptr(dy, 'dy'),
+            _ptr(dx, 'dx', allow_none=True), _ptr(dact_src, 'dact_src', allow_none=True), dact, slope,
+            _ptr(dw, 'dw', allow_none=True), _ptr(db, 'db', allow_none=True), int(accumulate),
+            M, K, N, ws, nb, _stream(), _ptr(tk, 'tickets', torch.int32, allow_none=True)), 'bn_linear_bwd')
+    except HipLibraryError:
+        _drop_tickets(dy.device)
+        raise
     return dx
 
 
@@ -831,6 +865,23 @@
         out = torch.empty((), dtype=torch.float32, device=t.device)
     _check(load().bn_reduce_sum(_ptr(t, 'in'), _ptr(out, 'out'), t.numel(), float(scale),
                                 _stream()), 'bn_reduce_sum')
+    return out
+
+
+REDUCE_MAX_CHUNKS = 16
+
+
+def reduce_sum_chunks(t, bounds, scales, out):
+    row = t[0].numel() if t.shape[0] else 0
+    ptr_in, ptr_out = _ptr(t, 'in'), _ptr(out, 'out')
+    for c0 in range(0, len(bounds), REDUCE_MAX_CHUNKS):
+        grp = list(zip(bounds, scales))[c0:c0 + REDUCE_MAX_CHUNKS]
+        k = len(grp)
+        beg = (ctypes.c_longlong * k)(*[int(b) * row for (b, _e), _s in grp])
+        cnt = (ctypes.c_longlong * k)(*[(int(e) - int(b)) * row for (b, e), _s in grp])
+        sc = (ctypes.c_float * k)(*[float(s) for _b, s in grp])
+        _check(load().bn_reduce_sum_chunks(ptr_in, ptr_out + 4 * c0, beg, cnt, sc, k, _stream()),
+               'bn_reduce_sum_chunks')
     return out
 
 
diff --git a/behavenet_amd/csrc/bn_launch.h b/behavenet_amd/csrc/bn_launch.h
--- a/behavenet_amd/csrc/bn_launch.h
+++ b/behavenet_amd/csrc/bn_launch.h
@@ -12,6 +12,8 @@
     int accumulate;
     float* part;
     int kslice;
+    unsigned* tickets;
+    int nslices;
 };
 
 int bn_launch_down_generic(const float* big, const float* w, const float* bias, float* out,
@@ -30,7 +32,8 @@
 size_t bn_gemm_ws_bytes(int M, int N, int K);
 int bn_launch_col_sum(const float* dy, float* db, int M, int N, int accumulate, hipStream_t st);
 int bn_launch_linear_jobs(const GemmArgs* g0, const GemmArgs* g1, const float* dy, float* db, int M,
-                          int N, int accumulate, void* ws, size_t ws_bytes, hipStream_t st);
+                          int N, int accumulate, void* ws, size_t ws_bytes, unsigned* tickets,
+                          hipStream_t st);
 size_t bn_linear_jobs_ws_bytes(int M, int N, int K);
 
 int bn_launch_act_fwd(const float* x, float* y, size_t n, int act, float slope, hipStream_t st);
@@ -43,6 +46,8 @@
 int bn_launch_scale_frames(float* t, const float* frame_scale, const float* group_scale,
                            const int* group_of_frame, int N, size_t D, hipStream_t st);
 int bn_launch_reduce_sum(const float* in, float* out, size_t n, float scale, hipStream_t st);
+struct BnReduceChunks { size_t beg[BN_REDUCE_MAX_CHUNKS], n[BN_REDUCE_MAX_CHUNKS]; float scale[BN_REDUCE_MAX_CHUNKS]; };
+int bn_launch_reduce_sum_chunks(const float* in, float* out, const BnReduceChunks& ch, int n_chunks, hipStream_t st);
 int bn_launch_reparam_fwd(const float* mu, const float* logvar, const float* eps, float* z,
                           size_t n, hipStream_t st);
 int bn_launch_kl_rows(const float* mu, const float* logvar, float* kl_rows, int N, int D,
diff --git a/behavenet_amd/csrc/bn_reduce.h b/behavenet_amd/csrc/bn_reduce.h
--- a/behavenet_amd/csrc/bn_reduce.h
+++ b/behavenet_amd/csrc/bn_reduce.h
@@ -22,12 +22,35 @@
     return e == hipSuccess ? 0 : (int)e;
 }
 
+static inline int bn_sum_partials_threads(int total, int splits) {
+    return (splits >= 128 && total <= 16384) ? 1024 : 256;
+}
+
 static inline int bn_launch_sum_partials(const float* part, float* out, int total, int splits,
                                          int accumulate, int ab_elems, int ntap, hipStream_t st,
                                          int row_len = 0, int row_stride = 0) {
-    const int threads = (splits >= 128 && total <= 16384) ? 1024 : 256;
+    const int threads = bn_sum_partials_threads(total, splits);
     hipLaunchKernelGGL(k_sum_partials, dim3((total + 63) / 64), dim3(threads), 0, st, part, out, total,
                        splits, accumulate, ab_elems, ntap, row_len, row_stride);
     hipError_t e = hipGetLastError();
     return e == hipSuccess ? 0 : (int)e;
 }
+
+struct BnSumJob { const float* part; float* out; int total, ab_elems, ntap, row_len, row_stride; };
+__global__ __launch_bounds__(1024) void k_sum_partials_two(BnSumJob a, BnSumJob b, int splits, int accumulate,
+                                                           int blocks_a);
+static inline int bn_launch_sum_partials_two(const BnSumJob& a, const BnSumJob& b, int splits, int accumulate,
+                                             hipStream_t st) {
+    const int threads = bn_sum_partials_threads(a.total, splits);
+    if (threads != bn_sum_partials_threads(b.total, splits)) {
+        const int rc = bn_launch_sum_partials(a.part, a.out, a.total, splits, accumulate, a.ab_elems, a.ntap, st,
+                                              a.row_len, a.row_stride);
+        return rc ? rc : bn_launch_sum_partials(b.part, b.out, b.total, splits, accumulate, b.ab_elems, b.ntap, st,
+                                                b.row_len, b.row_stride);
+    }
+    const int blocks_a = (a.total + 63) / 64, blocks_b = (b.total + 63) / 64;
+    hipLaunchKernelGGL(k_sum_partials_two, dim3(blocks_a + blocks_b), dim3(threads), 0, st, a, b, splits, accumulate,
+                       blocks_a);
+    hipError_t e = hipGetLastError();
+    return e == hipSuccess ? 0 : (int)e;
+}
diff --git a/behavenet_amd/csrc/bn_ticket.h b/behavenet_amd/csrc/bn_ticket.h
--- /dev/null
+++ b/behavenet_amd/csrc/bn_ticket.h
@@ -0,0 +1,23 @@
+#pragma once
+#include "bn_common.h"
+
+__device__ __forceinline__ bool bn_ticket_arrive(unsigned* ticket, unsigned total, unsigned* flag) {
+    asm volatile("s_waitcnt vmcnt(0)" ::: "memory");
+    __syncthreads();
+    if (threadIdx.x == 0) {
+        __builtin_amdgcn_fence(__ATOMIC_RELEASE, "agent");
+        asm volatile("s_waitcnt vmcnt(0)" ::: "memory");
+        const unsigned old = __hip_atomic_fetch_add(ticket, 1u, __ATOMIC_RELAXED, __HIP_MEMORY_SCOPE_AGENT);
+        if (old == total - 1) {
+            __builtin_amdgcn_fence(__ATOMIC_ACQUIRE, "agent");
+            asm volatile("s_waitcnt vmcnt(0)" ::: "memory");
+        }
+        *flag = old;
+    }
+    __syncthreads();
+    return *flag == total - 1;
+}
+
+__device__ __forceinline__ void bn_ticket_reset(unsigned* ticket) {
+    __hip_atomic_store(ticket, 0u, __ATOMIC_RELAXED, __HIP_MEMORY_SCOPE_AGENT);
+}
diff --git a/behavenet_amd/csrc/capi.hip b/behavenet_amd/csrc/capi.hip
--- a/behavenet_amd/csrc/capi.hip
+++ b/behavenet_amd/csrc/capi.hip
@@ -1448,7 +1448,8 @@
 }
 
 extern "C" int bn_linear_fwd(const float* x, const float* w, const float* b, float* y, int M,
-                             int K, int N, void* ws, size_t ws_bytes, bn_stream_t stream) {
+                             int K, int N, void* ws, size_t ws_bytes, bn_stream_t stream,
+                             unsigned* tickets) {
     if (!x || !w || !y || M <= 0 || K <= 0 || N <= 0) return BN_E_BADARG;
     GemmArgs a;
     a.A = x; a.sai = K; a.sak = 1;
@@ -1457,13 +1458,14 @@
     a.M = M; a.N = N; a.K = K;
     a.bias_j = b; a.dact_src = nullptr; a.dact = BN_ACT_NONE; a.slope = 0.f; a.accumulate = 0;
     BnProfScope prof(BN_PROF_LINEAR_FWD, K, N, "k_linear_jobs", (hipStream_t)stream);
-    return bn_launch_linear_jobs(&a, nullptr, nullptr, nullptr, 0, 0, 0, ws, ws_bytes, (hipStream_t)stream);
+    return bn_launch_linear_jobs(&a, nullptr, nullptr, nullptr, 0, 0, 0, ws, ws_bytes, tickets,
+                                 (hipStream_t)stream);
 }
 
 extern "C" int bn_linear_bwd(const float* x, const float* w, const float* dy, float* dx,
                              const float* dact_src, int dact, float slope, float* dw, float* db,
                              int accumulate, int M, int K, int N, void* ws, size_t ws_bytes,
-                             bn_stream_t stream) {
+                             bn_stream_t stream, unsigned* tickets) {
     if (!dy || M <= 0 || K <= 0 || N <= 0) return BN_E_BADARG;
     hipStream_t st = (hipStream_t)stream;
     BnProfScope prof(BN_PROF_LINEAR_BWD, K, N, "k_linear_jobs (dx, dW, db)", st);
@@ -1489,7 +1491,7 @@
         a.accumulate = accumulate; a.part = nullptr; a.kslice = 0;
     }
     return bn_launch_linear_jobs(dx ? &gx : nullptr, dw ? &gw : nullptr, dy, db, M, N, accumulate, ws,
-                                 ws_bytes, st);
+                                 ws_bytes, tickets, st);
 }
 
 extern "C" int bn_sqerr_frame_sums(const float* pred, const float* target, const float* mask,
@@ -1574,6 +1576,19 @@
     return bn_launch_reduce_sum(in, out, n, scale, (hipStream_t)stream);
 }
 
+extern "C" int bn_reduce_sum_chunks(const float* in, float* out, const long long* beg, const long long* count,
+                                    const float* scale, int n_chunks, bn_stream_t stream) {
+    if (!in || !out || !beg || !count || !scale || n_chunks <= 0 || n_chunks > BN_REDUCE_MAX_CHUNKS)
+        return BN_E_BADARG;
+    BnReduceChunks ch;
+    memset(&ch, 0, sizeof(ch));
+    for (int c = 0; c < n_chunks; ++c) {
+        if (beg[c] < 0 || count[c] <= 0) return BN_E_BADARG;
+        ch.beg[c] = (size_t)beg[c]; ch.n[c] = (size_t)count[c]; ch.scale[c] = scale[c];
+    }
+    return bn_launch_reduce_sum_chunks(in, out, ch, n_chunks, (hipStream_t)stream);
+}
+
 extern "C" int bn_reparam_fwd(const float* mu, const float* logvar, const float* eps, float* z,
                               size_t n, bn_stream_t stream) {
     if (!mu || !logvar || !eps || !z) return BN_E_BADARG;
diff --git a/behavenet_amd/csrc/conv_edge.hip b/behavenet_amd/csrc/conv_edge.hip
--- a/behavenet_amd/csrc/conv_edge.hip
+++ b/behavenet_amd/csrc/conv_edge.hip
@@ -542,11 +542,13 @@
     }
     BN_LAUNCH_CHECK();
     if (bias_part) {
-        const int rc = bn_launch_sum_partials(bias_part, db, g.Cs, plan.d, accumulate, 0, 0, st);
+        const BnSumJob jw = {(const float*)ws, dw, g.Cs * 25, 0, 0, 25, g.Cb * 25};
+        const BnSumJob jb = {bias_part, db, g.Cs, 0, 0, 0, 0};
+        const int rc = bn_launch_sum_partials_two(jw, jb, plan.d, accumulate, st);
         if (rc) return rc;
         if (bias_done) *bias_done = true;
     }
-    for (int b = 0; b < g.Cb; ++b) {
+    for (int b = bias_part ? 1 : 0; b < g.Cb; ++b) {
         const int rc = bn_launch_sum_partials(
             (const float*)ws + (size_t)b * plan.d * g.Cs * 25, dw + b * 25, g.Cs * 25, plan.d,
             accumulate, 0, 0, st, 25, g.Cb * 25);
diff --git a/behavenet_amd/csrc/conv_generic.hip b/behavenet_amd/csrc/conv_generic.hip
--- a/behavenet_amd/csrc/conv_generic.hip
+++ b/behavenet_amd/csrc/conv_generic.hip
@@ -273,14 +273,13 @@
 }
 
 #include "bn_reduce.h"
-__global__ __launch_bounds__(1024) void k_sum_partials(const float* __restrict__ part,
-                                                       float* __restrict__ out, int total,
-                                                       int splits, int accumulate, int ab_elems,
-                                                       int ntap, int row_len, int row_stride) {
-    __shared__ float red[16][64];
+__device__ __forceinline__ void sum_partials_block(const float* __restrict__ part, float* __restrict__ out,
+                                                   const int total, const int splits, const int accumulate,
+                                                   const int ab_elems, const int ntap, const int row_len,
+                                                   const int row_stride, const int block, float (*red)[64]) {
     const int il = threadIdx.x & 63, zl = threadIdx.x >> 6;
     const int nz = blockDim.x >> 6;
-    const int i = blockIdx.x * 64 + il;
+    const int i = block * 64 + il;
     float s0 = 0.f, s1 = 0.f, s2 = 0.f, s3 = 0.f;
     if (i < total) {
         int z = zl;
@@ -309,6 +308,23 @@
         }
         out[o] = accumulate ? out[o] + v : v;
     }
+}
+
+__global__ __launch_bounds__(1024) void k_sum_partials(const float* __restrict__ part,
+                                                       float* __restrict__ out, int total,
+                                                       int splits, int accumulate, int ab_elems,
+                                                       int ntap, int row_len, int row_stride) {
+    __shared__ float red[16][64];
+    sum_partials_block(part, out, total, splits, accumulate, ab_elems, ntap, row_len, row_stride, blockIdx.x, red);
+}
+
+__global__ __launch_bounds__(1024) void k_sum_partials_two(BnSumJob a, BnSumJob b, int splits, int accumulate,
+                                                           int blocks_a) {
+    __shared__ float red[16][64];
+    const bool job_b = (int)blockIdx.x >= blocks_a;
+    const BnSumJob& j = job_b ? b : a;
+    sum_partials_block(j.part, j.out, j.total, splits, accumulate, j.ab_elems, j.ntap, j.row_len, j.row_stride,
+                       job_b ? (int)blockIdx.x - blocks_a : (int)blockIdx.x, red);
 }
 
 __global__ __launch_bounds__(256) void k_sum_partials_pair(
diff --git a/behavenet_amd/csrc/elementwise.hip b/behavenet_amd/csrc/elementwise.hip
--- a/behavenet_amd/csrc/elementwise.hip
+++ b/behavenet_amd/csrc/elementwise.hip
@@ -107,9 +107,8 @@
     }
 }
 
-__global__ __launch_bounds__(EW_THREADS) void k_reduce_sum(
-    const float* __restrict__ in, float* __restrict__ out, size_t n, float scale) {
-    __shared__ float red[EW_THREADS / BN_WAVE];
+__device__ __forceinline__ void reduce_sum_block(const float* __restrict__ in, float* __restrict__ out, size_t n,
+                                                 float scale, float* red) {
     float acc = 0.f;
     for (size_t i = threadIdx.x; i < n; i += EW_THREADS) acc += in[i];
 #pragma unroll
@@ -117,6 +116,19 @@
     if ((threadIdx.x & 63) == 0) red[threadIdx.x >> 6] = acc;
     __syncthreads();
     if (threadIdx.x == 0) out[0] = ((red[0] + red[1]) + (red[2] + red[3])) * scale;
+}
+
+__global__ __launch_bounds__(EW_THREADS) void k_reduce_sum(
+    const float* __restrict__ in, float* __restrict__ out, size_t n, float scale) {
+    __shared__ float red[EW_THREADS / BN_WAVE];
+    reduce_sum_block(in, out, n, scale, red);
+}
+
+__global__ __launch_bounds__(EW_THREADS) void k_reduce_sum_chunks(const float* __restrict__ in, float* __restrict__ out,
+                                                                  BnReduceChunks ch) {
+    __shared__ float red[EW_THREADS / BN_WAVE];
+    const int c = blockIdx.x;
+    reduce_sum_block(in + ch.beg[c], out + c, ch.n[c], ch.scale[c], red);
 }
 
 __global__ __launch_bounds__(EW_THREADS) void k_reparam_fwd(
@@ -309,6 +321,12 @@
     return 0;
 }
 
+int bn_launch_reduce_sum_chunks(const float* in, float* out, const BnReduceChunks& ch, int n_chunks, hipStream_t st) {
+    hipLaunchKernelGGL(k_reduce_sum_chunks, dim3(n_chunks), dim3(EW_THREADS), 0, st, in, out, ch);
+    BN_LAUNCH_CHECK();
+    return 0;
+}
+
 int bn_launch_reduce_sum(const float* in, float* out, size_t n, float scale, hipStream_t st) {
     hipLaunchKernelGGL(k_reduce_sum, dim3(1), dim3(EW_THREADS), 0, st, in, out, n, scale);
     BN_LAUNCH_CHECK();
diff --git a/behavenet_amd/csrc/gemm.hip b/behavenet_amd/csrc/gemm.hip
--- a/behavenet_amd/csrc/gemm.hip
+++ b/behavenet_amd/csrc/gemm.hip
@@ -1,9 +1,28 @@
 #include <string.h>
 #include "bn_common.h"
 #include "bn_launch.h"
+#include "bn_ticket.h"
 
 typedef float floatx16 __attribute__((ext_vector_type(16)));
 
+
+__device__ __forceinline__ void gemm_combine_one(const GemmArgs& a, const int slices, const int i, const int j) {
+    float v = 0.f;
+    const size_t zs = (size_t)a.M * a.N;
+    const float* p0 = a.part + (size_t)i * a.N + j;
+    for (int z0 = 0; z0 < slices; z0 += 16) {
+        float t[16];
+#pragma unroll
+        for (int u = 0; u < 16; ++u) t[u] = p0[(size_t)(z0 + u < slices ? z0 + u : z0) * zs];
+#pragma unroll
+        for (int u = 0; u < 16; ++u)
+            if (z0 + u < slices) v += t[u];
+    }
+    if (a.bias_j) v += a.bias_j[j];
+    const long off = (long)i * a.sci + (long)j * a.scj;
+    if (a.dact_src) v *= bn_act_grad_from_output(a.dact_src[off], a.dact, a.slope);
+    a.C[off] = a.accumulate ? a.C[off] + v : v;
+}
 
 __device__ __forceinline__ void gemm_tile(const GemmArgs& a, const int bx, const int by, const int bz,
                                           const int nw, const int ws, float* red,
@@ -101,16 +120,34 @@
 #pragma unroll
         for (int t = 0; t < 16; ++t) red[(ws * 16 + t) * 64 + lane] = acc[t];
         __syncthreads();
-        if (ws != 0) return;
-#pragma unroll
-        for (int t = 0; t < 16; ++t) {
-            float s = red[t * 64 + lane];
-            for (int w2 = 1; w2 < nw; ++w2) s += red[(w2 * 16 + t) * 64 + lane];
-            acc[t] = s;
+        if (ws != 0 && !a.tickets) return;
+        if (ws == 0) {
+#pragma unroll
+            for (int t = 0; t < 16; ++t) {
+                float s = red[t * 64 + lane];
+                for (int w2 = 1; w2 < nw; ++w2) s += red[(w2 * 16 + t) * 64 + lane];
+                acc[t] = s;
+            }
         }
     }
 
     const int j = j0 + (lane & 31);
+    if (a.tickets) {
+        if (ws == 0 && j < a.N) {
+#pragma unroll
+            for (int t = 0; t < 16; ++t) {
+                const int i = i0 + (t & 3) + 8 * (t >> 2) + 4 * (lane >> 5);
+                if (i < a.M) a.part[((size_t)bz * a.M + i) * a.N + j] = acc[t];
+            }
+        }
+        unsigned* ticket = a.tickets + by * ((a.N + 31) / 32) + bx;
+        if (!bn_ticket_arrive(ticket, (unsigned)a.nslices, reinterpret_cast<unsigned*>(red))) return;
+        const int rows = min(32, a.M - i0), cols = min(32, a.N - j0);
+        for (int e = threadIdx.x; e < rows * cols; e += nw * 64)
+            gemm_combine_one(a, a.nslices, i0 + e / cols, j0 + e % cols);
+        if (threadIdx.x == 0) bn_ticket_reset(ticket);
+        return;
+    }
     if (j >= a.N || !live) return;
     if (a.part) {
 #pragma unroll
@@ -200,7 +237,7 @@
     return s < 1 ? 1 : s;
 }
 
-static void gemm_job(GemmJob* j, const GemmArgs& a, float* part) {
+static void gemm_job(GemmJob* j, const GemmArgs& a, float* part, unsigned* tickets) {
     j->a = a;
     j->tiles_x = (a.N + 31) / 32;
     j->tiles = j->tiles_x * ((a.M + 31) / 32);
@@ -211,6 +248,8 @@
     j->nw = kw >= 4 ? 4 : kw >= 2 ? 2 : 1;
     const int upb = GJ_WAVES / j->nw, units = j->tiles * j->slices;
     j->blocks = (units + upb - 1) / upb;
+    j->a.nslices = j->slices;
+    j->a.tickets = (j->slices > 1 && upb == 1 && j->tiles <= BN_TICKET_WORDS / 2) ? tickets : nullptr;
 }
 
 size_t bn_linear_jobs_ws_bytes(int M, int N, int K) {
@@ -219,7 +258,8 @@
 }
 
 int bn_launch_linear_jobs(const GemmArgs* g0, const GemmArgs* g1, const float* dy, float* db, int M,
-                          int N, int accumulate, void* ws, size_t ws_bytes, hipStream_t st) {
+                          int N, int accumulate, void* ws, size_t ws_bytes, unsigned* tickets,
+                          hipStream_t st) {
     LinearJobs p;
     memset(&p, 0, sizeof(p));
     int blocks = 0;
@@ -230,7 +270,8 @@
             const size_t need = bn_linear_jobs_ws_bytes(gs[q]->M, gs[q]->N, gs[q]->K);
             float* part = nullptr;
             if (need && wp && ws_bytes >= need) { part = (float*)wp; wp += need; ws_bytes -= need; }
-            gemm_job(&p.g[q], *gs[q], part);
+            gemm_job(&p.g[q], *gs[q], part, tickets);
+            if (p.g[q].a.tickets) tickets += p.g[q].tiles;
             blocks += p.g[q].blocks;
         }
     if (db) {
@@ -241,7 +282,7 @@
     if (blocks == 0) return 0;
     BN_LAUNCH_MAIN(k_linear_jobs, dim3(blocks), dim3(64 * GJ_WAVES), 0, st, p);
     for (int q = 0; q < 2; ++q)
-        if (gs[q] && p.g[q].slices > 1)
+        if (gs[q] && p.g[q].slices > 1 && !p.g[q].a.tickets)
             hipLaunchKernelGGL(k_gemm_combine, dim3((gs[q]->M * gs[q]->N + 255) / 256), dim3(256), 0, st,
                                p.g[q].a, p.g[q].slices);
     BN_LAUNCH_CHECK();
@@ -356,22 +397,8 @@
 __global__ __launch_bounds__(256) void k_gemm_combine(GemmArgs a, int slices) {
     const int idx = blockIdx.x * 256 + threadIdx.x;
     if (idx >= a.M * a.N) return;
-    const int i = idx / a.N, j = idx - i * a.N;
-    float v = 0.f;
-    const size_t zs = (size_t)a.M * a.N;
-    const float* p0 = a.part + (size_t)i * a.N + j;
-    for (int z0 = 0; z0 < slices; z0 += 16) {
-        float t[16];
-#pragma unroll
-        for (int u = 0; u < 16; ++u) t[u] = p0[(size_t)(z0 + u < slices ? z0 + u : z0) * zs];
-#pragma unroll
-        for (int u = 0; u < 16; ++u)
-            if (z0 + u < slices) v += t[u];
-    }
-    if (a.bias_j) v += a.bias_j[j];
-    const long off = (long)i * a.sci + (long)j * a.scj;
-    if (a.dact_src) v *= bn_act_grad_from_output(a.dact_src[off], a.dact, a.slope);
-    a.C[off] = a.accumulate ? a.C[off] + v : v;
+    const int i = idx / a.N;
+    gemm_combine_one(a, slices, i, idx - i * a.N);
 }
 
 __global__ __launch_bounds__(64) void k_col_sum(const float* __restrict__ dy,
@@ -417,6 +444,7 @@
 }
 int bn_launch_gemm(const GemmArgs& a0, hipStream_t st, void* ws, size_t ws_bytes) {
     GemmArgs a = a0;
+    a.tickets = nullptr; a.nslices = 0;
     int ta = 0, tb = 0;
     if (gemm_tiled_ok(a, &ta, &tb)) {
         int slices = gemm_tiled_slices(a.M, a.N, a.K);
@@ -436,6 +464,7 @@
         }
     }
     a = a0;
+    a.tickets = nullptr; a.nslices = 0;
     int slices = gemm_slices(a.M, a.N, a.K);
     if (slices > 1 && (!ws || ws_bytes < (size_t)slices * a.M * a.N * sizeof(float))) slices = 1;
     a.kslice = ((a.K + slices - 1) / slices + 15) & ~15;
diff --git a/behavenet_amd/hip_functions.py b/behavenet_amd/hip_functions.py
--- a/behavenet_amd/hip_functions.py
+++ b/behavenet_amd/hip_functions.py
@@ -408,6 +408,14 @@
         else:
             dpre = dout
         dx, grads = _stack_backward(ctx, dpre, first_param=3)
+        return (None, dx, None) + tuple(grads)
+
+
+class ConvStackPreGradFn(ConvStackFn):
+
+    @staticmethod
+    def backward(ctx, dpre):
+        dx, grads = _stack_backward(ctx, dpre.contiguous(), first_param=3)
         return (None, dx, None) + tuple(grads)
 
 
@@ -468,7 +476,9 @@
     return (dpre if ctx.need_dx else None), grads
 
 
-def conv_stack(plan, x, params, h1=None):
+def conv_stack(plan, x, params, h1=None, grad_is_pre=False):
+    if grad_is_pre and plan[-1].act != _hip.ACT_NONE:
+        return ConvStackPreGradFn.apply(plan, x, h1, *params)
     return ConvStackFn.apply(plan, x, h1, *params)
 
 
@@ -712,8 +722,7 @@
         for i in range(len(plan) - 1):
             _note_signs(plan, i, acts[i + 1])
         out = torch.empty((len(bounds),), dtype=torch.float32, device=x.device)
-        for c, ((beg, end), sc) in enumerate(zip(bounds, scales)):
-            _hip.reduce_sum(part[beg:end], float(sc), out=out[c:c + 1])
+        _hip.reduce_sum_chunks(part, bounds, scales, out)
         ctx.plan = plan
         ctx.taps = taps
         ctx.need_dx = x.requires_grad
@@ -964,9 +973,10 @@
 class LinearFn(torch.autograd.Function):
 
     @staticmethod
-    def forward(ctx, x, w, b):
+    def forward(ctx, x, w, b, x_act=_hip.ACT_NONE):
         x = x.contiguous()
         ctx.save_for_backward(x, w)
+        ctx.x_act = x_act
         ctx.has_bias = b is not None
         ctx.param_refs = (w, b)
         _note_use((w, b), ctx.needs_input_grad[1])
@@ -988,8 +998,10 @@
             dw = torch.empty_like(w) if need_dw else None
             db = torch.empty((w.shape[0],), dtype=w.dtype, device=w.device) if need_db else None
         wc = w.contiguous()
+        dsrc, dact, slope = (x, ctx.x_act, LRELU_SLOPE) if ctx.x_act != _hip.ACT_NONE \
+            else (None, _hip.ACT_NONE, 0.0)
         if direct and _use_side_stream:
-            dx = _hip.linear_bwd(x, wc, dy, need_dx, None, _hip.ACT_NONE, 0.0, None, None, False) \
+            dx = _hip.linear_bwd(x, wc, dy, need_dx, dsrc, dact, slope, None, None, False) \
                 if need_dx else None
             side = _side_stream(w.device)
             ev = torch.cuda.Event()
@@ -1000,16 +1012,16 @@
             dy.record_stream(side)
             x.record_stream(side)
             _report_ready(ctx.param_refs)
-            return dx, None, None
-        dx = _hip.linear_bwd(x, wc, dy, need_dx, None, _hip.ACT_NONE, 0.0, dw, db, direct)
+            return dx, None, None, None
+        dx = _hip.linear_bwd(x, wc, dy, need_dx, dsrc, dact, slope, dw, db, direct)
         if direct:
             _report_ready(ctx.param_refs)
-            return dx, None, None
-        return dx, dw, db
-
-
-def linear(x, w, b=None):
-    return LinearFn.apply(x, w, b)
+            return dx, None, None, None
+        return dx, dw, db, None
+
+
+def linear(x, w, b=None, x_act=_hip.ACT_NONE):
+    return LinearFn.apply(x, w, b, x_act)
 
 
 class SqErrFn(torch.autograd.Function):
@@ -1049,8 +1061,7 @@
         ctx.bounds, ctx.scales = list(bounds), [float(s) for s in scales]
         sums = _hip.sqerr_frame_sums(a, b, mask)
         out = torch.empty((len(ctx.bounds),), dtype=torch.float32, device=a.device)
-        for i, ((beg, end), s) in enumerate(zip(ctx.bounds, ctx.scales)):
-            _hip.reduce_sum(sums[beg:end], s, out=out[i:i + 1])
+        _hip.reduce_sum_chunks(sums, ctx.bounds, ctx.scales, out)
         return out
 
     @staticmethod
diff --git a/behavenet_amd/models/aes.py b/behavenet_amd/models/aes.py
--- a/behavenet_amd/models/aes.py
+++ b/behavenet_amd/models/aes.py
@@ -183,9 +183,10 @@
             params += [mod.weight, mod.bias]
         return params
 
-    def _features(self, x, dataset=None):
+    def _features(self, x, dataset=None, one_linear_consumer=False):
         hp = self.hparams
         self._pool_state = ([], [])
+        self._features_act = _hip.ACT_NONE
         if encode_dtype() == 'bf16' and self._bf16_eligible(x):
             h = conv_stack_bf16(self._plan, x, self._stack_params(dataset))
             return h.view(h.size(0), -1)
@@ -196,7 +197,9 @@
                               _bn_modules(self.encoder, self._layer_names))
         else:
             h = conv_stack(self._plan, x, self._stack_params(dataset),
-                           h1=self._first_layer_slice(x, dataset))
+                           h1=self._first_layer_slice(x, dataset), grad_is_pre=one_linear_consumer)
+            if one_linear_consumer:
+                self._features_act = self._plan[-1].act
         return h.view(h.size(0), -1)
 
     def _bf16_eligible(self, x):
@@ -281,12 +284,13 @@
         return h1[beg:beg + x.shape[0]]
 
     def forward(self, x, dataset=None):
-        x1 = self._features(x, dataset)
+        variational = self.hparams.get('variational', False)
+        x1 = self._features(x, dataset, one_linear_consumer=not variational)
         pool_idx, sizes = self._pool_out()
-        if self.hparams.get('variational', False):
+        if variational:
             return (linear(x1, self.FF.weight, self.FF.bias),
                     linear(x1, self.logvar.weight, self.logvar.bias), pool_idx, sizes)
-        return linear(x1, self.FF.weight, self.FF.bias), pool_idx, sizes
+        return linear(x1, self.FF.weight, self.FF.bias, x_act=self._features_act), pool_idx, sizes
 
 
 class ConvAEDecoder(BaseModule):
diff --git a/include/behavenet_hip.h b/include/behavenet_hip.h
--- a/include/behavenet_hip.h
+++ b/include/behavenet_hip.h
@@ -131,19 +131,25 @@
                            const float* sum_dzx, float* dx, int N, int C, int HW, float inv_count,
                            int act, float slope, bn_stream_t stream);
 
+#define BN_TICKET_WORDS 4096
 size_t bn_linear_ws_bytes(int M, int K, int N);
 int bn_linear_fwd(const float* x, const float* w, const float* b, float* y,
-                  int M, int K, int N, void* ws, size_t ws_bytes, bn_stream_t stream);
+                  int M, int K, int N, void* ws, size_t ws_bytes, bn_stream_t stream,
+                  unsigned* tickets);
 int bn_linear_bwd(const float* x, const float* w, const float* dy,
                   float* dx, const float* dact_src, int dact, float slope,
                   float* dw, float* db, int accumulate,
-                  int M, int K, int N, void* ws, size_t ws_bytes, bn_stream_t stream);
+                  int M, int K, int N, void* ws, size_t ws_bytes, bn_stream_t stream,
+                  unsigned* tickets);
 
 int bn_sqerr_frame_sums(const float* pred, const float* target, const float* mask,
                         float* frame_sums, int N, size_t D, bn_stream_t stream);
 int bn_sqerr_bwd(const float* pred, const float* target, const float* mask, float* dpred,
                  size_t n, float scale, const float* gscale, bn_stream_t stream);
 int bn_reduce_sum(const float* in, float* out, size_t n, float scale, bn_stream_t stream);
+#define BN_REDUCE_MAX_CHUNKS 16
+int bn_reduce_sum_chunks(const float* in, float* out, const long long* beg, const long long* count,
+                         const float* scale, int n_chunks, bn_stream_t stream);
 
 int bn_reparam_fwd(const float* mu, const float* logvar, const float* eps, float* z,
                    size_t n, bn_stream_t stream);
```
